# open-mmlab/Amphion

Measured on AMD Instinct MI355X. Metric: audio samples/sec (HiFi-GAN V1 22.05 kHz generator, mel->wav), higher is better.
Workload: dtype f32 (split-f16 MFMA: 3 x v_mfma_f32_32x32x16_f16 per term, f32 accumulate)

## Files before the change

amphion_amd/_lib.py:

```python
from __future__ import annotations

import ctypes
import os
import weakref
from ctypes import POINTER, c_char_p, c_float, c_int, c_int32, c_int64, c_size_t, c_void_p

_HERE = os.path.dirname(os.path.abspath(__file__))
LIB_PATH = os.environ.get("AMP_LIB_PATH") or os.path.join(_HERE, "lib", "libamphion_hip.so")

AMP_MAX_STAGES = 8
AMP_MAX_KERNELS = 8
AMP_MAX_DILATIONS = 8

AMP_ARCH_HIFIGAN, AMP_ARCH_BIGVGAN, AMP_ARCH_HIFIGAN_VITS = 0, 1, 2
AMP_ACT_LRELU, AMP_ACT_SNAKE, AMP_ACT_SNAKEBETA = 0, 1, 2
AMP_PRECISION_F32, AMP_PRECISION_F16X3 = 0, 1
AMP_CONV_OPT_PAD_REFLECT, AMP_CONV_OPT_TANH = 1, 2
AMP_PAD_REPLICATE, AMP_PAD_ZEROS, AMP_PAD_REFLECT = 0, 1, 2
AMP_PW_BIAS, AMP_PW_BIAS_GELU, AMP_PW_SCALE_RES = 0, 1, 2
PRECISIONS = {"f32": AMP_PRECISION_F32, "fp32": AMP_PRECISION_F32, "f16x3": AMP_PRECISION_F16X3}


class AmpError(RuntimeError):

    def __init__(self, status, message):
        super().__init__(f"libamphion_hip error {status}: {message}")
        self.status = status


class amp_gen_desc(ctypes.Structure):
    _fields_ = [
        ("arch", c_int32),
        ("n_in", c_int32),
        ("upsample_initial_channel", c_int32),
        ("n_stages", c_int32),
        ("upsample_rates", c_int32 * AMP_MAX_STAGES),
        ("upsample_kernel_sizes", c_int32 * AMP_MAX_STAGES),
        ("n_kernels", c_int32),
        ("resblock_kernel_sizes", c_int32 * AMP_MAX_KERNELS),
        ("n_dilations", c_int32 * AMP_MAX_KERNELS),
        ("resblock_dilation_sizes", (c_int32 * AMP_MAX_DILATIONS) * AMP_MAX_KERNELS),
        ("resblock_type", c_int32),
        ("activation", c_int32),
        ("snake_logscale", c_int32),
        ("gin_channels", c_int32),
    ]


class amp_mel_desc(ctypes.Structure):
    _fields_ = [
        ("struct_size", ctypes.c_uint32),
        ("n_fft", c_int32),
        ("win_size", c_int32),
        ("hop_size", c_int32),
        ("n_mel", c_int32),
        ("pad_mode", c_int32),
        ("mag_eps", c_float),
        ("log_clip", c_float),
        ("mel_bands_dev", c_void_p),
        ("range_dev", c_void_p),
        ("range_host", c_void_p),
        ("range_reset_dev", c_void_p),
        ("range_seq", c_int32),
    ]

    def __init__(self, *args, **kw):
        super().__init__(ctypes.sizeof(type(self)), *args, **kw)


class amp_dw_desc(ctypes.Structure):
    _fields_ = [
        ("residual_channels", c_int32),
        ("residual_layers", c_int32),
        ("dilation_cycle_length", c_int32),
        ("n_mel", c_int32),
        ("upsample0", c_int32),
        ("upsample1", c_int32),
        ("max_steps", c_int32),
    ]


_SIGNATURES = {
    "amp_version": (c_int, []),
    "amp_last_error": (c_char_p, []),
    "amp_device_count": (c_int, []),
    "amp_set_precision": (c_int, [c_int]),
    "amp_get_precision": (c_int, []),
    "amp_gen_create": (c_int, [POINTER(amp_gen_desc), POINTER(c_void_p)]),
    "amp_gen_set_weight": (c_int, [c_void_p, c_char_p, c_void_p, POINTER(c_int64), c_int]),
    "amp_gen_finalize": (c_int, [c_void_p]),
    "amp_gen_hop": (c_int, [c_void_p]),
    "amp_gen_workspace_bytes": (c_size_t, [c_void_p, c_int, c_int]),
    "amp_set_group_mb": (c_int, [c_int]),
    "amp_set_pair_strips": (c_int, [c_int]),
    "amp_range_check": (c_int, [c_void_p]),
    "amp_gen_range_check": (c_int, [c_void_p, c_void_p]),
    "amp_gen_forward": (c_int, [c_void_p, c_void_p, c_void_p, c_int, c_int, c_void_p, c_void_p, c_size_t, c_void_p]),
    "amp_gen_forward_ragged": (c_int, [c_void_p, c_void_p, c_void_p, c_void_p, c_int, c_int, c_void_p, c_void_p, c_size_t, c_void_p]),
    "amp_gen_set_profiling": (c_int, [c_void_p, c_int]),
    "amp_gen_last_timing_ms": (c_int, [c_void_p, c_int, POINTER(c_float)]),
    "amp_gen_timing_ms": (c_int, [c_void_p, c_int, c_int, POINTER(c_float)]),
    "amp_gen_kernel_name": (c_int, [c_void_p, c_int, c_int, c_char_p, c_size_t]),
    "amp_gen_destroy": (None, [c_void_p]),
    "amp_conv_create": (c_int, [c_int, c_int, c_int, c_int, c_int, c_int, c_int, c_void_p, c_void_p, POINTER(c_void_p)]),
    "amp_conv_out_len": (c_int, [c_void_p, c_int]),
    "amp_conv_forward": (c_int, [c_void_p, c_void_p, c_int, c_int, c_float, c_void_p, c_float, c_void_p, c_void_p]),
    "amp_conv_forward_strided": (c_int, [c_void_p, c_void_p, ctypes.c_longlong, c_int, c_int, c_float, c_void_p, c_float, c_void_p, c_void_p]),
    "amp_conv_forward_ragged": (c_int, [c_void_p, c_void_p, ctypes.c_longlong, c_int, c_int, c_void_p, c_float, c_void_p, c_float, c_void_p, c_void_p]),
    "amp_conv_forward_mrf": (c_int, [c_void_p, c_void_p, c_int, c_int, c_float, c_void_p, c_void_p, c_int, c_float, c_void_p]),
    "amp_apnet_polar": (c_int, [c_void_p, c_void_p, c_void_p, c_size_t, c_void_p, c_void_p, c_void_p, c_void_p]),
    "amp_istft_same": (c_int, [POINTER(amp_mel_desc), c_void_p, c_void_p, c_int, c_int, c_void_p, c_void_p, c_void_p, c_void_p, c_void_p]),
    "amp_istft_same_polar": (c_int, [POINTER(amp_mel_desc), c_void_p, ctypes.c_longlong, c_int, c_int, c_float, c_void_p, c_void_p, c_void_p,
                                     c_void_p, c_void_p]),
    "amp_pw_create": (c_int, [c_int, c_int, c_void_p, c_void_p, POINTER(c_void_p)]),
    "amp_pw_forward": (c_int, [c_void_p, c_void_p, ctypes.c_longlong, c_int, c_int, c_int, c_void_p, c_void_p, c_void_p, c_void_p]),
    "amp_pw_precision": (c_int, [c_void_p]),
    "amp_pw_destroy": (None, [c_void_p]),
    "amp_dw_create": (c_int, [POINTER(amp_dw_desc), POINTER(c_void_p)]),
    "amp_dw_set_weight": (c_int, [c_void_p, c_char_p, c_void_p, ctypes.c_longlong]),
    "amp_dw_finalize": (c_int, [c_void_p]),
    "amp_dw_precision": (c_int, [c_void_p]),
    "amp_dw_set_precision": (c_int, [c_void_p, c_int]),
    "amp_dw_workspace_bytes": (c_size_t, [c_void_p, c_int, c_int]),
    "amp_dw_condition": (c_int, [c_void_p, c_void_p, c_int, c_int, c_void_p, c_void_p, c_size_t, c_void_p]),
    "amp_dw_embed": (c_int, [c_void_p, c_void_p, c_int, c_void_p, c_void_p]),
    "amp_dw_input": (c_int, [c_void_p, c_void_p, c_int, c_int, c_void_p, c_void_p]),
    "amp_dw_layer": (c_int, [c_void_p, c_int, c_void_p, c_void_p, c_void_p, ctypes.c_longlong, c_void_p, c_void_p, c_void_p, c_int, c_int, c_void_p]),
    "amp_dw_tail": (c_int, [c_void_p, c_void_p, c_int, c_int, c_void_p, c_void_p]),
    "amp_dw_forward": (c_int, [c_void_p, c_void_p, c_int, c_void_p, c_int, c_void_p, c_int, c_int, c_void_p, c_void_p, c_size_t, c_void_p]),
    "amp_dw_sample_step": (c_int, [c_void_p, c_void_p, c_int, c_float, c_float, c_float, c_float, c_void_p, c_void_p, c_int, c_int, c_void_p,
                                   c_size_t, c_void_p]),
    "amp_dw_destroy": (None, [c_void_p]),
    "amp_fvq_create": (c_int, [c_int, c_int, c_int, c_int, c_int, POINTER(c_void_p), POINTER(c_void_p), POINTER(c_void_p), POINTER(c_void_p),
                               POINTER(c_void_p), POINTER(c_void_p)]),
    "amp_fvq_encode": (c_int, [c_void_p, c_void_p, c_int, c_int, c_int, c_void_p, c_void_p, c_void_p, c_void_p]),
    "amp_fvq_decode": (c_int, [c_void_p, c_void_p, c_int, c_int, c_int, c_void_p, c_void_p]),
    "amp_fvq_check": (c_int, [c_void_p, c_void_p]),
    "amp_fvq_encode_ex": (c_int, [c_void_p, c_void_p, ctypes.c_longlong, c_void_p, c_int, c_int, c_int, c_void_p, c_void_p, c_void_p, c_void_p,
                                  c_void_p]),
    "amp_fvq_decode_add": (c_int, [c_void_p, c_void_p, c_int, c_int, c_int, c_void_p, c_void_p, c_void_p]),
    "amp_semantic_prepare": (c_int, [c_void_p, c_void_p, c_void_p, c_int, c_int, c_int, c_int, c_void_p, c_void_p]),
    "amp_fvq_destroy": (None, [c_void_p]),
    "amp_codec_unit_create": (c_int, [c_int, c_int, c_void_p, c_void_p, c_void_p, c_void_p, c_void_p, c_void_p, POINTER(c_void_p)]),
    "amp_codec_unit_fused": (c_int, [c_void_p]),
    "amp_set_codec_unit_fusion": (c_int, [c_int]),
    "amp_codec_unit_workspace_bytes": (c_size_t, [c_void_p, c_int, c_int]),
    "amp_codec_unit_forward": (c_int, [c_void_p, c_void_p, c_int, c_int, c_void_p, c_void_p, c_size_t, c_void_p]),
    "amp_codec_unit_destroy": (None, [c_void_p]),
    "amp_aa_unit_create": (c_int, [c_int, c_int, c_void_p, c_void_p, c_void_p, c_void_p, c_void_p, c_void_p, c_void_p, c_void_p, c_int, c_void_p,
                                   c_void_p, POINTER(c_void_p)]),
    "amp_aa_unit_fused": (c_int, [c_void_p]),
    "amp_set_aa_unit_fusion": (c_int, [c_int]),
    "amp_aa_unit_workspace_bytes": (c_size_t, [c_void_p, c_int, c_int]),
    "amp_aa_unit_forward": (c_int, [c_void_p, c_void_p, c_int, c_int, c_void_p, c_void_p, c_size_t, c_void_p]),
    "amp_aa_unit_destroy": (None, [c_void_p]),
    "amp_sconv_create": (c_int, [c_int, c_int, c_int, c_int, c_void_p, c_void_p, POINTER(c_void_p)]),
    "amp_sconv_out_len": (c_int, [c_void_p, c_int]),
    "amp_sconv_workspace_bytes": (c_size_t, [c_void_p, c_int, c_int]),
    "amp_sconv_forward": (c_int, [c_void_p, c_void_p, c_int, c_int, c_void_p, c_void_p, c_size_t, c_void_p, c_void_p]),
    "amp_sconv_destroy": (None, [c_void_p]),
    "amp_tconv_create": (c_int, [c_int, c_int, c_int, c_int, c_int, c_void_p, c_void_p, POINTER(c_void_p)]),
    "amp_tconv_out_len": (c_int, [c_void_p, c_int]),
    "amp_tconv_fused": (c_int, [c_void_p]),
    "amp_set_tconv_fusion": (c_int, [c_int]),
    "amp_tconv_workspace_bytes": (c_size_t, [c_void_p, c_int, c_int]),
    "amp_tconv_forward": (c_int, [c_void_p, c_void_p, c_int, c_int, c_void_p, c_void_p, c_size_t, c_void_p, c_void_p]),
    "amp_tconv_destroy": (None, [c_void_p]),
    "amp_elu_pad": (c_int, [c_void_p, c_int, c_int, c_int, c_int, c_int, c_int, c_float, c_void_p, c_void_p]),
    "amp_lstm_create": (c_int, [c_int, c_int, c_int, c_int, c_int, POINTER(c_void_p), POINTER(c_void_p), POINTER(c_void_p), POINTER(c_void_p),
                                POINTER(c_void_p)]),
    "amp_lstm_workspace_bytes": (c_size_t, [c_void_p, c_int, c_int]),
    "amp_lstm_out_channels": (c_int, [c_void_p]),
    "amp_lstm_forward": (c_int, [c_void_p, c_void_p, c_int, c_int, c_void_p, c_void_p, c_size_t, c_void_p]),
    "amp_lstm_recur": (c_int, [c_void_p, c_int, c_void_p, c_int, c_int, c_void_p, c_void_p, c_void_p, c_void_p]),
    "amp_lstm_destroy": (None, [c_void_p]),
    "amp_evq_create": (c_int, [c_int, c_int, c_int, POINTER(c_void_p), POINTER(c_void_p)]),
    "amp_evq_encode": (c_int, [c_void_p, c_void_p, c_int, c_int, c_int, c_int, c_void_p, c_void_p, c_void_p, c_void_p]),
    "amp_evq_decode": (c_int, [c_void_p, c_void_p, c_int, c_int, c_int, c_int, c_void_p, c_void_p]),
    "amp_evq_check": (c_int, [c_void_p, c_void_p]),
    "amp_evq_destroy": (None, [c_void_p]),
    "amp_dsconv_create": (c_int, [c_int, c_int, c_void_p, c_void_p, POINTER(c_void_p)]),
    "amp_dsconv_out_len": (c_int, [c_void_p, c_int]),
    "amp_dsconv_workspace_bytes": (c_size_t, [c_void_p, c_int, c_int]),
    "amp_dsconv_forward": (c_int, [c_void_p, c_void_p, c_int, c_int, c_int, c_void_p, c_size_t, c_void_p, c_void_p]),
    "amp_dsconv_destroy": (None, [c_void_p]),
    "amp_gelu": (c_int, [c_void_p, ctypes.c_longlong, c_void_p, c_void_p]),
    "amp_layer_norm_c": (c_int, [c_void_p, c_void_p, c_void_p, c_void_p, c_void_p, c_int, c_int, c_int, c_float, c_int, c_void_p, c_void_p]),
    "amp_add_channel_bias": (c_int, [c_void_p, c_void_p, c_int, c_int, c_int, c_void_p]),
    "amp_layer_norm_c_ragged": (c_int, [c_void_p, c_void_p, c_void_p, c_void_p, c_void_p, c_void_p, c_int, c_int, c_int, c_float, c_int, c_void_p, c_void_p]),
    "amp_dds_seam": (c_int, [c_void_p, c_void_p, c_void_p, c_void_p, c_float, c_void_p, c_void_p, c_int, c_int, c_void_p, c_void_p, c_float,
                             c_void_p, c_int, c_int, c_int, c_void_p, c_void_p, c_void_p]),
    "amp_dwconv_layer_norm_c": (c_int, [c_void_p, c_void_p, c_void_p, c_int, c_int, c_void_p, c_void_p, c_void_p, c_int, c_int, c_int, c_float, c_int, c_void_p, c_void_p]),
    "amp_dwconv_layer_norm_c_causal": (c_int, [c_void_p, c_void_p, c_void_p, c_int, c_int, c_void_p, c_void_p, c_void_p, c_int, c_int, c_int, c_float, c_int,
                                               c_void_p, c_void_p]),
    "amp_rel_attention_strided": (c_int, [c_void_p, c_void_p, c_void_p, ctypes.c_longlong, c_void_p, c_void_p, c_void_p, c_int, c_int, c_int, c_int, c_int, c_void_p, c_void_p]),
    "amp_set_rel_attention_tiled": (c_int, [c_int]),
    "amp_set_resblock_streams": (c_int, [c_int]),
    "amp_gen_prepare_streams": (c_int, [c_void_p]),
    "amp_rel_attention": (c_int, [c_void_p, c_void_p, c_void_p, c_void_p, c_void_p, c_void_p, c_int, c_int, c_int, c_int, c_int, c_void_p, c_void_p]),
    "amp_dwconv": (c_int, [c_void_p, c_void_p, c_void_p, c_void_p, c_int, c_int, c_int, c_int, c_int, c_void_p, c_void_p]),
    "amp_spline_flow": (c_int, [c_void_p, c_void_p, c_void_p, c_int, c_int, c_int, c_int, c_float, c_int, c_int, c_int, c_void_p, c_void_p]),
    "amp_spline_flow_proj": (c_int, [c_void_p, c_void_p, c_void_p, c_void_p, c_void_p, c_int, c_int, c_int, c_int, c_int, c_float, c_int, c_int, c_int, c_void_p, c_void_p]),
    "amp_affine_reverse": (c_int, [c_void_p, c_void_p, c_void_p, c_void_p, c_int, c_int, c_int, c_void_p, c_void_p]),
    "amp_embed_tokens": (c_int, [c_void_p, c_void_p, c_void_p, c_int, c_int, c_int, c_int, c_float, c_void_p, c_void_p]),
    "amp_durations": (c_int, [c_void_p, c_void_p, c_int, c_int, c_float, c_void_p, c_void_p, c_void_p, c_void_p]),
    "amp_expand_path": (c_int, [c_void_p, c_void_p, c_void_p, c_void_p, c_int, c_int, c_int, c_int, c_void_p, c_void_p, c_void_p]),
    "amp_expand_path_strided": (c_int, [c_void_p, ctypes.c_longlong, c_void_p, c_void_p, c_void_p, c_int, c_int, c_int, c_int, c_void_p, c_void_p, c_void_p]),
    "amp_gauss_sample": (c_int, [c_void_p, c_void_p, c_void_p, c_size_t, c_float, c_void_p, c_void_p]),
    "amp_snake": (c_int, [c_void_p, c_int, c_int, c_int, c_void_p, c_void_p, c_int, c_void_p, c_void_p]),
    "amp_fir_upsample": (c_int, [c_void_p, c_int, c_int, c_int, c_void_p, c_int, c_int, c_void_p, c_void_p]),
    "amp_fir_filter": (c_int, [c_void_p, c_int, c_int, c_int, c_void_p, c_int, c_int, c_int, c_int, c_int, c_void_p, c_void_p]),
    "amp_wav_to_pcm16": (c_int, [c_void_p, c_int, c_int, ctypes.c_longlong, c_void_p, c_void_p, ctypes.c_longlong, c_void_p]),
    "amp_conv_set_option": (c_int, [c_void_p, c_int, c_int]),
    "amp_pair_forward": (c_int, [c_void_p, c_void_p, c_void_p, c_int, c_int, c_float, c_void_p, c_void_p]),
    "amp_resblock_forward": (c_int, [POINTER(c_void_p), POINTER(c_void_p), c_int, c_void_p, c_int, c_int, c_float, c_void_p, c_void_p]),
    "amp_set_resblock_fusion": (c_int, [c_int]),
    "amp_conv_destroy": (None, [c_void_p]),
    "amp_set_small_conv": (c_int, [c_int]),
    "amp_set_conv_blk": (c_int, [c_int]),
    "amp_set_conv_rg_fast": (c_int, [c_int]),
    "amp_set_pingpong": (c_int, [c_int]),
    "amp_set_conv_blk_narrow": (c_int, [c_int]),
    "amp_ampblock_forward": (c_int, [POINTER(c_void_p), POINTER(c_void_p), c_int, c_void_p, c_void_p, c_int, c_void_p, c_void_p,
                                     c_void_p, c_int, c_int, c_void_p, c_int, c_float, c_void_p]),
    "amp_set_ampblock_fusion": (c_int, [c_int]),
    "amp_conv_create_gated": (c_int, [c_int, c_int, c_int, c_int, c_void_p, c_void_p, POINTER(c_void_p)]),
    "amp_wn_forward": (c_int, [POINTER(c_void_p), POINTER(c_void_p), c_int, c_void_p, c_void_p, ctypes.c_longlong, c_void_p, c_int, c_int,
                               c_void_p, c_void_p, c_void_p]),
    "amp_wn_gate": (c_int, [c_void_p, c_void_p, ctypes.c_longlong, c_void_p, c_int, c_int, c_int, c_void_p]),
    "amp_wn_accumulate": (c_int, [c_void_p, c_void_p, c_void_p, c_void_p, c_int, c_int, c_int, c_int, c_int, c_void_p]),
    "amp_sequence_mask": (c_int, [c_void_p, c_void_p, c_int, c_int, c_int, c_void_p]),
    "amp_coupling_apply": (c_int, [c_void_p, c_void_p, c_void_p, c_int, c_int, c_int, c_int, c_void_p]),
    "amp_flip_channels": (c_int, [c_void_p, c_void_p, c_int, c_int, c_int, c_void_p]),
    "amp_posterior_sample": (c_int, [c_void_p, c_void_p, c_void_p, c_void_p, c_int, c_int, c_int, c_void_p]),
    "amp_antialias_snake": (c_int, [c_void_p, c_int, c_int, c_int, c_void_p, c_void_p, c_int, c_void_p, c_void_p, c_void_p, c_void_p]),
    "amp_istft_forward": (c_int, [POINTER(amp_mel_desc), c_void_p, c_void_p, c_int, c_int, c_void_p, c_void_p, c_void_p, c_void_p, c_void_p]),
    "amp_mel_num_frames": (c_int, [POINTER(amp_mel_desc), c_int]),
    "amp_mel_init": (c_int, []),
    "amp_mel_forward_ragged": (c_int, [POINTER(amp_mel_desc), c_void_p, c_void_p, c_int, c_int, c_void_p, c_void_p, c_void_p, c_void_p, c_void_p, c_void_p, c_void_p]),
    "amp_mel_backward": (c_int, [POINTER(amp_mel_desc), c_void_p, c_int, c_int] + [c_void_p] * 11),
    "amp_mel_forward": (c_int, [POINTER(amp_mel_desc), c_void_p, c_int, c_int, c_void_p, c_void_p, c_void_p, c_void_p, c_void_p, c_void_p, c_void_p]),
}

EXPORTED_SYMBOLS = tuple(_SIGNATURES)

_lib = None


def lib():
    global _lib
    if _lib is None:
        if not os.path.exists(LIB_PATH):
            raise RuntimeError(
                f"{LIB_PATH} not found: build it with `python -m amphion_amd.build` "
                "(the HIP path has no CPU fallback)"
            )
        import torch

        L = ctypes.CDLL(LIB_PATH)
        for name, (res, args) in _SIGNATURES.items():
            fn = getattr(L, name)
            fn.restype = res
            fn.argtypes = args
        _lib = L
    return _lib


def set_precision(name):
    if name not in PRECISIONS:
        raise ValueError(f"precision must be one of {sorted(PRECISIONS)}, got {name!r}")
    check(lib().amp_set_precision(PRECISIONS[name]))


def get_precision():
    return "f32" if lib().amp_get_precision() == AMP_PRECISION_F32 else "f16x3"


def check(status):
    if status < 0:
        raise AmpError(status, lib().amp_last_error().decode("utf-8", "replace"))
    return status


def ptr(t):
    return c_void_p(t.data_ptr()) if t is not None else None


def _destroy(name, address):
    try:
        getattr(lib(), name)(c_void_p(address))
    except Exception:
        pass


def finalizer(owner, destroy, handle):
    return weakref.finalize(owner, _destroy, destroy, handle.value)


AMP_ERR_INVALID = -1
AMP_ERR_UNSUPPORTED = -4
AMP_ERR_RANGE = -6


def range_check(device=None):
    import torch

    dev = torch.device("cuda", torch.cuda.current_device()) if device is None else torch.device(device)
    with torch.cuda.device(dev):
        check(lib().amp_range_check(current_stream_ptr(dev)))


def require_device_tensor(t, name="tensor"):
    import torch

    if not isinstance(t, torch.Tensor):
        raise TypeError(f"{name} must be a torch.Tensor")
    if not t.is_cuda:
        raise RuntimeError(
            f"{name} is on {t.device}: the amphion_amd kernels run on a ROCm (MI355X) device only; "
            "there is no CPU fallback (move the model and its input to 'cuda')"
        )
    if t.dtype != torch.float32:
        raise TypeError(f"{name} must be float32, got {t.dtype}")
    return t.contiguous()


class _NullCtx:
    def __enter__(self):
        return None

    def __exit__(self, *a):
        return False


_NULL_CTX = _NullCtx()


def on_device(device):
    import torch

    idx = device.index if isinstance(device, torch.device) else torch.device(device).index
    if idx is None or idx == torch._C._cuda_getDevice():
        return _NULL_CTX
    return torch.cuda.device(device)


def current_stream_ptr(device):
    import torch

    raw = getattr(torch._C, "_cuda_getCurrentRawStream", None)
    if raw is not None:
        idx = device.index if isinstance(device, torch.device) else torch.device(device).index
        return c_void_p(raw(torch.cuda.current_device() if idx is None else idx))
    return c_void_p(torch.cuda.current_stream(device).cuda_stream)
```

amphion_amd/csrc/amp_host.h:

```cpp
#pragma once
#include <math.h>

#include <vector>

#include "amp_internal.h"

#define AMP_HIP(expr)                                                                  \
    do {                                                                               \
        hipError_t e__ = (expr);                                                       \
        if (e__ != hipSuccess) {                                                       \
            set_error("%s failed: %s (%s:%d)", #expr, hipGetErrorString(e__), __FILE__, __LINE__); \
            return AMP_ERR_HIP;                                                        \
        }                                                                              \
    } while (0)

#define AMP_RC(expr) do { int rc__ = (expr); if (rc__ != AMP_OK) return rc__; } while (0)

struct amp_conv {
    int transposed = 0, cin = 0, cout = 0, k = 0, stride = 1, dilation = 1, padding = 0;
    int M = 0, ntaps = 0, KT = 0, off0 = 0, dstep = 0, halo_left = 0, halo_right = 0, up = 1, up_pad = 0;
    int nchunks = 0;
    int precision = amp::PREC_F32;
    int pad_reflect = 0, tanh_out = 0;
    int out_pad = 0;
    int gated_H = 0;
    int Mpad = 0;
    float wscale = 1.f;
    amp::ConvPlan plan{};
    void* wp_dev = nullptr;
    float* bias_dev = nullptr;
    ~amp_conv() {
        if (wp_dev) (void)hipFree(wp_dev);
        if (bias_dev) (void)hipFree(bias_dev);
    }
};

namespace amp {

int device_upload(const void* host, size_t bytes, void** out);

struct DeviceAllocs {
    std::vector<void*> owned;
    DeviceAllocs() = default;
    DeviceAllocs(const DeviceAllocs&) = delete;
    DeviceAllocs& operator=(const DeviceAllocs&) = delete;
    ~DeviceAllocs() {
        for (void* p : owned) (void)hipFree(p);
    }
    int upload(const void* host, size_t bytes, void** out) {
        if (int rc = device_upload(host, bytes, out); rc != AMP_OK) return rc;
        owned.push_back(*out);
        return AMP_OK;
    }
    template <class T, class P>
    int upload(const std::vector<T>& v, P** out) { return upload(v.data(), v.size() * sizeof(T), (void**)out); }
};

int default_precision();

constexpr int kConvBlkDefault = 3;
constexpr int kConvRgFastDefault = 1;
constexpr int kPingPongDefault = 1;
struct Config {
    int pair_strips = -1;
    int rb_fusion = 1;
    int ampb_fusion = 1;
    int conv_blk = kConvBlkDefault;
    size_t group_bytes = 0;
    int small_conv = 1;
    int conv_rg_fast = 1;
    int pingpong = 1;
    int narrow_blk = 1;
    int rb_streams = -1;
    Config();
};
Config& cfg();

struct RangeGuard {
    unsigned* dev = nullptr;
    unsigned* host = nullptr;
    hipEvent_t ev = nullptr;
    bool pending = false;
};
bool guard_init(RangeGuard& g);
void guard_free(RangeGuard& g);
int range_poll(RangeGuard* g, hipStream_t st);
int range_publish(RangeGuard* g, hipStream_t st);
int range_check_sync(RangeGuard* g, hipStream_t st, const char* who);
struct RangeFlagScope {
    explicit RangeFlagScope(unsigned* word);
    ~RangeFlagScope();
    RangeFlagScope(const RangeFlagScope&) = delete;
    RangeFlagScope& operator=(const RangeFlagScope&) = delete;
};

inline float pow2_weight_scale(float wmax) {
    int e2 = 0;
    if (wmax > 0.f) { (void)frexpf(wmax, &e2); if (ldexpf(1.f, e2 - 1) == wmax) e2 -= 1; }
    return wmax > 0.f ? ldexpf(1.f, 13 - e2) : 1.f;
}

template <class View>
std::vector<_Float16> pack_a_f16x3(int row_blocks, int k16, int taps, size_t pad_entries, float wscale, View view) {
    std::vector<_Float16> wp(((size_t)row_blocks * k16 * taps * 2 + pad_entries) * 64 * 8, (_Float16)0.f);
    for (int mb = 0; mb < row_blocks; ++mb)
        for (int c = 0; c < k16; ++c)
            for (int g = 0; g < taps; ++g)
                for (int lane = 0; lane < 64; ++lane)
                    for (int e = 0; e < 8; ++e) {
                        const float v = view(mb * 32 + (lane & 31), c * 16 + 8 * (lane >> 5) + e, g) * wscale;
                        const _Float16 hi = (_Float16)v;
                        const _Float16 lo = (_Float16)(v - (float)hi);
                        const size_t ent = (((size_t)mb * k16 + c) * taps + g) * 2;
                        wp[((ent + 0) * 64 + lane) * 8 + e] = hi;
                        wp[((ent + 1) * 64 + lane) * 8 + e] = lo;
                    }
    return wp;
}

template <class View>
int pack_matrix_f16x3(const char* who, int rows, int cols, int row_blocks, int k16, View W, std::vector<_Float16>* wp, float* inv_scale) {
    float wmax = 0.f;
    for (int m = 0; m < rows; ++m)
        for (int i = 0; i < cols; ++i) {
            const float w = fabsf(W(m, i));
            if (!(w < 1e30f)) { set_error("%s: non-finite weight", who); return AMP_ERR_INVALID; }
            wmax = fmaxf(wmax, w);
        }
    const float wscale = pow2_weight_scale(wmax);
    *inv_scale = 1.f / (16.f * wscale);
    *wp = pack_a_f16x3(row_blocks, k16, 1, 0, wscale, [&](int m, int i, int) { return (m < rows && i < cols) ? W(m, i) : 0.f; });
    return AMP_OK;
}

int conv_build(amp_conv* c, const float* w, const float* bias);
int conv_run(const amp_conv* c, const float* x, int B, int T, float slope_in, const float* res, float slope_out, float* y, int mode, float div,
             hipStream_t stream, long long xbs = 0, const int* lens = nullptr, int len_mul = 1, ConvArgs* plan_small = nullptr,
             int* plan_ni = nullptr);
int next_rev(const int* lens);

bool pair_supported(const amp_conv* c1, const amp_conv* c2);
int pair_run(const amp_conv* c1, const amp_conv* c2, const float* x, int B, int T, float slope, float* y, int mode, float div,
             hipStream_t stream, const int* lens = nullptr, int len_mul = 1);
bool pair_tile_args(const amp_conv* c1, const amp_conv* c2, const float* x, int B, int T, float slope, float* y, int mode, float div,
                    const int* lens, int len_mul, PairArgs* out);

bool rb_supported(const amp_conv* const* c1, const amp_conv* const* c2, int np, int B, int T);
int rb_split(const amp_conv* const* c1, int np, int B, int T);
int rb_run(const amp_conv* const* c1, const amp_conv* const* c2, int np, const float* x, int B, int T, float slope, float* y, int mode,
           float div, hipStream_t stream, const int* lens = nullptr, int len_mul = 1, int first = 0, int count = -1);

struct ActParams {
    float* a_dev = nullptr;
    float* invb_dev = nullptr;
    float* fu_dev = nullptr;
    float* fd_dev = nullptr;
    float* fu2_dev = nullptr;
};
int act_params_upload(const float* alpha_dev, const float* beta_dev, int C, int logscale, const float* filt_up_host,
                      const float* filt_down_host, float** out);
bool ampb_supported(const amp_conv* const* c1, const amp_conv* const* c2, int np, const ActParams* acts, size_t nacts, int B, int T);
int ampb_run(const amp_conv* const* c1, const amp_conv* const* c2, int np, const ActParams* acts, const float* x, int B, int T, float* y,
             int mode, float div, hipStream_t stream, const int* lens = nullptr, int len_mul = 1);

}
```

amphion_amd/csrc/amp_internal.h:

```cpp
#pragma once
#include <hip/hip_runtime.h>
#include <stdarg.h>
#include <stdint.h>
#include <stdio.h>

#include <atomic>
#include <mutex>
#include <string>
#include <vector>

#include "amphion_hip.h"

namespace amp {

constexpr int KC = 8;
constexpr int KC16 = 16;

enum { PREC_F32 = 0, PREC_F16X3 = 1 };

struct ConvArgs {
    const float* x;
    const void* wp;
    const float* bias;
    const float* res;
    float* y;
    int B, Cin, Tin;
    long long xbs;
    int nchunks;
    int M;
    int Tq;
    int tiles_per_item;
    int rev;
    int row_groups;
    int off0, dstep;
    int halo_left;
    int wd;
    int Cout, Tout;
    int up, up_pad;
    float slope_in, slope_out;
    int mode;
    float div;
    float acc_scale, inv_scale;
    const int* lens;
    int len_mul;
    unsigned* range_flag;
    int pad_reflect;
    int tanh_out;
    int Mpad;
    const float* gate_cond;
    long long gate_cond_bs;
    int wn_H;
    float* wn_x;
    float* wn_out;
    int wn_first, wn_last;
};

struct PairArgs {
    const float* x;
    float* y;
    const void* wp1;
    const float* bias1;
    const void* wp2;
    const float* bias2;
    int B, C, T;
    int tiles_per_item;
    int strip_len;
    int strips_per_item;
    int wide;
    int rev;
    int dil;
    float slope;
    float sc1, isc1, sc2, isc2;
    int mode;
    float div;
    const int* lens;
    int len_mul;
    unsigned* range_flag;
};

struct ConvSmall3Args {
    ConvArgs a[3];
    int nx[3], ny[3];
};
hipError_t launch_conv_small3(const ConvSmall3Args& p, const int ni[3], hipStream_t stream);

struct Pair3Args {
    PairArgs a[3];
    int n[3];
};
hipError_t launch_pair3(const Pair3Args& p, hipStream_t stream);

constexpr int AMP_RB_MAX_PAIRS = 3;
struct RbArgs {
    const float* x;
    float* y;
    const void* wp1[AMP_RB_MAX_PAIRS];
    const float* bias1[AMP_RB_MAX_PAIRS];
    const void* wp2[AMP_RB_MAX_PAIRS];
    const float* bias2[AMP_RB_MAX_PAIRS];
    float sc1[AMP_RB_MAX_PAIRS], isc1[AMP_RB_MAX_PAIRS], sc2[AMP_RB_MAX_PAIRS], isc2[AMP_RB_MAX_PAIRS];
    int dil[AMP_RB_MAX_PAIRS];
    int np;
    int rh;
    int B, C, T;
    int tiles_per_item;
    int rev;
    float slope;
    int mode;
    float div;
    const int* lens;
    int len_mul;
    unsigned* range_flag;
};

constexpr int AMP_AMPB_MAX_STEPS = 6;
struct AmpbArgs {
    const float* x;
    float* y;
    const void* wp[AMP_AMPB_MAX_STEPS];
    const float* bias[AMP_AMPB_MAX_STEPS];
    float sc[AMP_AMPB_MAX_STEPS], isc[AMP_AMPB_MAX_STEPS];
    int dil[AMP_AMPB_MAX_STEPS];
    const float* act_a[AMP_AMPB_MAX_STEPS];
    const float* act_invb[AMP_AMPB_MAX_STEPS];
    const float* act_fu[AMP_AMPB_MAX_STEPS];
    const float* act_fd[AMP_AMPB_MAX_STEPS];
    int ns;
    int rh;
    int B, C, T;
    int tiles_per_item;
    int rev;
    int mode;
    float div;
    const int* lens;
    int len_mul;
    unsigned* range_flag;
};

constexpr int DW_TN = 64;
struct DwLayerArgs {
    const float* x;
    const float* cond;
    const float* dconst;
    long long dconst_bs;
    const float* skip_in;
    float* x_out;
    float* skip_out;
    const uint4* wp1;
    const uint4* wp2;
    const float* w1f;
    const float* w2f;
    const float* bias1;
    const float* bias2;
    int C, n_mel, L, d;
    int K16;
    int tiles_per_item;
    float inv1, inv2;
    unsigned* range_flag;
};
size_t dw_layer_lds_bytes(int C, int n_mel, bool f32);
hipError_t launch_dw_layer(DwLayerArgs a, int B, bool f32, hipStream_t stream);

constexpr int CU_TN = 64;
struct CodecUnitArgs {
    const float* x;
    float* y;
    const uint4* wp1;
    const uint4* wp2;
    const float* bias1;
    const float* bias2;
    const float *alpha1, *invb1, *alpha2, *invb2;
    int C, T, d;
    int tiles_per_item;
    float inv1, inv2;
    unsigned* range_flag;
};
size_t codec_unit_lds_bytes(int C, int d);
hipError_t launch_codec_unit(CodecUnitArgs a, int B, hipStream_t stream);

constexpr int AA_N1 = 64;
constexpr int AA_TN = 54;
struct AaUnitArgs {
    const float* x;
    float* y;
    const uint4* wp1;
    const uint4* wp2;
    const float* bias1;
    const float* bias2;
    const float *a1, *invb1, *a2, *invb2;
    const float* filt;
    int C, T, d;
    int tiles_per_item;
    float inv1, inv2;
    unsigned* range_flag;
};
size_t aa_unit_lds_bytes(int C, int d);
hipError_t launch_aa_unit(AaUnitArgs a, int B, hipStream_t stream);

constexpr int TC_TN = 64;
struct TconvArgs {
    const float* x;
    float* y;
    const uint4* wp;
    const float* bias;
    const float* alpha;
    int cin, cout, s, p;
    int T, Tout;
    int M, NRB;
    int q_first;
    int tiles_per_item;
    float inv;
    unsigned* range_flag;
};
size_t tconv_lds_bytes(int cin);
hipError_t launch_tconv(TconvArgs a, int B, hipStream_t stream);

struct ConvPlan {
    int KT;
    int WM, WN;
    int NI;
    int HALO;
    int NT() const { return 32 * NI * WN; }
    int Mgroup() const { return 32 * WM; }
};

bool choose_plan(int ntaps, int M, int halo_total, int Tq, ConvPlan* plan);

template <int KT> hipError_t launch_conv(const ConvPlan& plan, const ConvArgs& a, hipStream_t stream);
template <int KT> hipError_t launch_conv_f16x3(const ConvPlan& plan, const ConvArgs& a, hipStream_t stream);
template <int KT> int conv_blk_nt(int cm, int halo_total);
template <int KT> hipError_t launch_conv_blk(int cm, int wn, const ConvArgs& a, hipStream_t stream);
constexpr int kSmallConvMaxChunks = 16;
template <int KT> hipError_t launch_conv_small(int ni, int epi, const ConvArgs& a, hipStream_t stream);
template <int KT> int pair_tile(int C, int dil);
template <int KT> hipError_t launch_pair(const PairArgs& a, hipStream_t stream);
template <int KT> int strip_step(int C, int dil, int wide, int* wg_per_cu);
template <int KT> hipError_t launch_strip(const PairArgs& a, hipStream_t stream);
template <int KT> int rb_tile(int C, int max_dil, int wide);
template <int KT> hipError_t launch_rb(const RbArgs& a, int wide, hipStream_t stream);
template <int KT> int ampb_tile(int C, int max_dil, int wide);
template <int KT> hipError_t launch_ampb(const AmpbArgs& a, int wide, hipStream_t stream);

hipError_t launch_conv_post(const float* x, const float* w_dev , const float* bias_dev ,
                            float* y, int B, int Cin, int T, int K, float slope_in, int apply_tanh,
                            const int* lens, int len_mul, hipStream_t stream);

hipError_t launch_act1d(const float* x, float* y, int B, int C, int T, const float* a_dev, const float* invb_dev,
                        const float* filt_up12, const float* filt_dn12, const int* lens, int len_mul,
                        hipStream_t stream, int rev = 0 );

hipError_t launch_add_channel_bias(float* y, const float* cb, int B, int C, int T, hipStream_t stream);
constexpr int AMP_MRF_MAX_PARTS = 3;
struct MrfSumArgs {
    float* y;
    const float* p[AMP_MRF_MAX_PARTS];
    int n;
    float div;
    size_t count;
};
hipError_t launch_mrf_sum(const MrfSumArgs& a, hipStream_t stream);

hipError_t launch_wn_gate(const float* a, const float* cond, long long cond_bs, float* out, int B, int H, int T,
                          hipStream_t stream);
hipError_t launch_wn_accumulate(float* x, float* out, const float* rs, const int* lens, int B, int H, int T, int last,
                                int first, hipStream_t stream);
hipError_t launch_mask(float* x, const int* lens, int B, int C, int T, hipStream_t stream);
hipError_t launch_coupling(float* x, const float* m, const int* lens, int B, int h, int T, int reverse,
                           hipStream_t stream);
hipError_t launch_flip_channels(const float* x, float* y, int B, int C, int T, hipStream_t stream);
hipError_t launch_posterior_sample(const float* stats, const float* eps, const int* lens, float* z, int B, int C, int T,
                                   hipStream_t stream);

hipError_t launch_fir_up(const float* x, float* y, int rows, int T, const float* taps_host, int K, int ratio, int pad,
                         int pad_left, hipStream_t stream);
hipError_t launch_fir_filter(const float* x, float* y, int rows, int T, int Tout, const float* taps_host, int K,
                             int stride, int pad_left, int mode, hipStream_t stream);
hipError_t launch_snake(const float* x, float* y, int B, int C, int T, const float* alpha, const float* beta, int logscale,
                        hipStream_t stream);
hipError_t launch_pcm16(const float* x, short* y, int B, int L, long long x_stride, long long y_stride, const int* lens,
                        hipStream_t stream);
hipError_t launch_apnet_polar(const float* logamp, const float* R, const float* I, size_t n, float* pha, float* rea,
                              float* imag, hipStream_t stream);

hipError_t launch_mel(const amp_mel_desc& d, const float* wav, const int* lens, int B, int L, int F, const float* window,
                      const float* melbasis, float* mel, float* mag, float* re, float* im, hipStream_t stream);

void set_error(const char* fmt, ...);

template <auto Kernel>
inline hipError_t ensure_dynamic_lds(size_t bytes) {
    if (bytes <= 64 * 1024) return hipSuccess;
    static std::atomic<unsigned long long> done{0};
    static std::mutex mu;
    int dev = 0;
    if (hipGetDevice(&dev) != hipSuccess || dev < 0) dev = 0;
    if (dev < 64 && ((done.load(std::memory_order_acquire) >> dev) & 1ull)) return hipSuccess;
    std::lock_guard<std::mutex> lock(mu);
    if (dev < 64 && ((done.load(std::memory_order_acquire) >> dev) & 1ull)) return hipSuccess;
    const hipError_t e = hipFuncSetAttribute(reinterpret_cast<const void*>(Kernel), hipFuncAttributeMaxDynamicSharedMemorySize, (int)bytes);
    if (e != hipSuccess) return e;
    if (dev < 64) done.fetch_or(1ull << dev, std::memory_order_release);
    return hipSuccess;
}

template <auto Kernel, class Args>
inline hipError_t launch_dynamic_lds(unsigned grid, size_t lds, hipStream_t stream, const Args& a) {
    if (hipError_t e = ensure_dynamic_lds<Kernel>(lds); e != hipSuccess) return e;
    hipLaunchKernelGGL(Kernel, dim3(grid), dim3(256), lds, stream, a);
    return hipGetLastError();
}

extern __thread std::string* tl_kernel_log;
bool manifest_on();
void manifest_add(const char* name, unsigned long long workgroups, double gflop, double mb, const char* what);
extern __thread char tl_last_kernel[160];
template <typename... A>
inline void note_kernel(const char* base, A... args) {
    if (!tl_kernel_log && !manifest_on()) return;
    char* buf = tl_last_kernel;
    constexpr int cap = (int)sizeof(tl_last_kernel);
    const int v[] = {static_cast<int>(args)...};
    int n = snprintf(buf, cap, "%s<", base);
    for (size_t i = 0; i < sizeof...(args) && n < cap - 16; ++i)
        n += snprintf(buf + n, cap - n, i ? ", %d" : "%d", v[i]);
    snprintf(buf + n, cap - n, ">");
    if (!tl_kernel_log) return;
    if (tl_kernel_log->find(buf) != std::string::npos) return;
    if (!tl_kernel_log->empty()) *tl_kernel_log += " | ";
    *tl_kernel_log += buf;
}
inline void note_work(unsigned long long workgroups, double gflop, double mb, const char* fmt, ...) __attribute__((format(printf, 4, 5)));
inline void note_work(unsigned long long workgroups, double gflop, double mb, const char* fmt, ...) {
    if (!manifest_on()) return;
    char what[160];
    va_list ap;
    va_start(ap, fmt);
    vsnprintf(what, sizeof(what), fmt, ap);
    va_end(ap);
    manifest_add(tl_last_kernel, workgroups, gflop, mb, what);
}
extern __thread int tl_conv_transposed;
inline void note_conv_work(const ConvArgs& a, int KT, dim3 grid) {
    const bool convt = tl_conv_transposed != 0;
    tl_conv_transposed = 0;
    if (!manifest_on()) return;
    const double gf = 2.0 * a.M * a.Cin * KT * (double)a.Tq * a.B / 1e9;
    const double mb = 4.0 * a.B * ((double)a.Cin * a.Tin + (double)a.Cout * a.Tout * (1 + (a.res ? 1 : 0) + (a.mode ? 1 : 0))) / 1e6;
    note_work((unsigned long long)grid.x * grid.y, gf, mb, "%s %d->%d k=%d d=%d T=%d->%d B=%d%s%s grid=%ux%u", convt ? "ConvT" : "conv", a.Cin,
              a.Cout, a.up > 1 ? KT * a.up : KT, a.dstep, a.Tin, a.Tout, a.B, a.res ? " +res" : "", a.mode ? " +sum" : "", grid.x, grid.y);
}

unsigned* range_flag_for_current_device();

}
```

amphion_amd/csrc/conv_host.hip:

```cpp
#include <string.h>

#include <memory>
#include <type_traits>
#include <vector>

#include "amp_host.h"

namespace amp {

template <int... K> struct Taps { static constexpr int list[] = {K...}; };
using ConvTaps = Taps<1, 2, 3, 5, 7, 11>;
using BlkTaps = Taps<2, 3, 7, 11>;
using SmallTaps = Taps<1, 3, 5, 7, 11>;
using PairTaps = Taps<3, 5, 7, 11>;
using RbTaps = Taps<3, 5, 7, 11>;
using AmpbTaps = Taps<3, 5, 7, 11>;

template <int... K, typename R, typename F>
static R with_taps(Taps<K...>, int k, R dflt, F&& f) {
    R r = dflt;
    (void)((k == K && (r = f(std::integral_constant<int, K>{}), true)) || ...);
    return r;
}

static hipError_t launch_conv(const ConvPlan& p, const ConvArgs& a, hipStream_t s) {
    return with_taps(ConvTaps{}, p.KT, hipErrorInvalidValue, [&](auto K) { return launch_conv<K>(p, a, s); });
}
static hipError_t launch_conv_f16x3(const ConvPlan& p, const ConvArgs& a, hipStream_t s) {
    return with_taps(ConvTaps{}, p.KT, hipErrorInvalidValue, [&](auto K) { return launch_conv_f16x3<K>(p, a, s); });
}
static int conv_blk_nt(int k, int cm, int halo) { return with_taps(BlkTaps{}, k, 0, [&](auto K) { return conv_blk_nt<K>(cm, halo); }); }
static hipError_t launch_conv_blk(int k, int cm, int wn, const ConvArgs& a, hipStream_t s) {
    return with_taps(BlkTaps{}, k, hipErrorInvalidValue, [&](auto K) { return launch_conv_blk<K>(cm, wn, a, s); });
}
static hipError_t launch_conv_small(int k, int ni, int epi, const ConvArgs& a, hipStream_t s) {
    return with_taps(SmallTaps{}, k, hipErrorInvalidValue, [&](auto K) { return launch_conv_small<K>(ni, epi, a, s); });
}
static int pair_tile(int k, int C, int dil) { return with_taps(PairTaps{}, k, 0, [&](auto K) { return pair_tile<K>(C, dil); }); }
static hipError_t launch_pair(int k, const PairArgs& a, hipStream_t s) {
    return with_taps(PairTaps{}, k, hipErrorInvalidValue, [&](auto K) { return launch_pair<K>(a, s); });
}
static int strip_step(int k, int C, int dil, int wide, int* wg) {
    return with_taps(PairTaps{}, k, 0, [&](auto K) { return strip_step<K>(C, dil, wide, wg); });
}
static hipError_t launch_strip(int k, const PairArgs& a, hipStream_t s) {
    return with_taps(PairTaps{}, k, hipErrorInvalidValue, [&](auto K) { return launch_strip<K>(a, s); });
}
static int rb_tile(int k, int C, int max_dil, int wide) { return with_taps(RbTaps{}, k, 0, [&](auto K) { return rb_tile<K>(C, max_dil, wide); }); }
static hipError_t launch_rb(int k, const RbArgs& a, int wide, hipStream_t s) {
    return with_taps(RbTaps{}, k, hipErrorInvalidValue, [&](auto K) { return launch_rb<K>(a, wide, s); });
}
static int ampb_tile(int k, int C, int max_dil, int wide) {
    return with_taps(AmpbTaps{}, k, 0, [&](auto K) { return ampb_tile<K>(C, max_dil, wide); });
}
static hipError_t launch_ampb(int k, const AmpbArgs& a, int wide, hipStream_t s) {
    return with_taps(AmpbTaps{}, k, hipErrorInvalidValue, [&](auto K) { return launch_ampb<K>(a, wide, s); });
}

static int round_up_taps(int ntaps) {
    for (int kt : ConvTaps::list)
        if (kt >= ntaps) return kt;
    return -1;
}

bool choose_plan(int KT, int M, int halo_total, int , ConvPlan* plan) {
    bool ok = false;
    for (int kt : ConvTaps::list) ok |= (kt == KT);
    if (!ok || halo_total > 128) return false;
    plan->KT = KT;
    plan->HALO = halo_total <= 64 ? 64 : 128;
    if (M > 64) { plan->WM = 4; plan->WN = 1; plan->NI = 8; }
    else if (M > 32) { plan->WM = 2; plan->WN = 2; plan->NI = 8; }
    else { plan->WM = 1; plan->WN = 4; plan->NI = 4; }
    return true;
}

struct StripChoice { bool use; int wide; int steps; };
static StripChoice strip_choice(int C, int k) {
    const int mode = cfg().pair_strips;
    if (mode == 0) return {false, 0, 0};
    if (C == 128 && (k == 7 || k == 11)) return {true, 3, 1};
    return {false, 0, 0};
}

static void strip_plan(int B, int T, int n1, int hb, int wg_per_cu, int* strip_len, int* spi_out) {
    const int slots = wg_per_cu * 256;
    long best = -1; int best_spi = 1;
    const int max_spi = (T + n1 - 1) / n1;
    for (int spi = 1; spi <= max_spi; ++spi) {
        const int L = (T + spi - 1) / spi;
        if ((long)(spi - 1) * L >= T) continue;
        const long steps = (L + hb + n1 - 1) / n1;
        const long rounds = ((long)B * spi + slots - 1) / slots;
        const long cost = rounds * (4 * steps + 1);
        if (best < 0 || cost < best) { best = cost; best_spi = spi; }
    }
    *spi_out = best_spi;
    *strip_len = (T + best_spi - 1) / best_spi;
}

static void strip_geometry(int B, int T, int n1, int hb, int wg_per_cu, int steps, bool ragged, int* strip_len, int* spi) {
    strip_plan(B, T, n1, hb, wg_per_cu, strip_len, spi);
    if (steps > 0 && steps * n1 - hb < T) { *strip_len = steps * n1 - hb; *spi = (T + *strip_len - 1) / *strip_len; }
    if (steps == 1 && !ragged && 4 * n1 - hb < T) {
        const int len4 = 4 * n1 - hb, spi4 = (T + len4 - 1) / len4;
        if ((long long)B * spi4 >= 1024) { *strip_len = len4; *spi = spi4; }
    }
}

constexpr long long kSmallGridWorkgroups = 384;

static bool small_conv_enabled() { return cfg().small_conv != 0; }

static int conv_blk_mode() { return cfg().conv_blk; }
static int narrow_blk_mode() { return cfg().narrow_blk; }
constexpr size_t kConvRgFastMaxWeightBytes = 3u << 20;
static bool conv_rg_fast() { return cfg().conv_rg_fast != 0; }
static thread_local unsigned g_launch_parity = 0;
int next_rev(const int* lens) {
    if (!cfg().pingpong || lens) return 0;
    return (int)(g_launch_parity++ & 1u);
}
constexpr long long kConvBlkMinWorkgroups = 512;

int conv_build(amp_conv* c, const float* w, const float* bias) {
    if (c->cin <= 0 || c->cout <= 0 || c->k <= 0 || c->stride <= 0 || c->dilation <= 0) {
        set_error("amp_conv: bad dimensions cin=%d cout=%d k=%d stride=%d dilation=%d", c->cin, c->cout, c->k, c->stride,
                  c->dilation);
        return AMP_ERR_INVALID;
    }
    if (!c->transposed) {
        if (c->stride != 1) { set_error("amp_conv: strided Conv1d is not on the vocoder path"); return AMP_ERR_UNSUPPORTED; }
        c->up = 1; c->up_pad = 0;
        c->M = c->cout;
        c->ntaps = c->k;
        c->off0 = -c->padding;
        c->dstep = c->dilation;
    } else if (c->stride == 1) {
        if (c->dilation != 1) { set_error("amp_conv: dilated ConvTranspose1d unsupported (dilation=%d)", c->dilation); return AMP_ERR_UNSUPPORTED; }
        c->up = 1; c->up_pad = 0;
        c->M = c->cout;
        c->ntaps = c->k;
        c->off0 = -(c->k - 1 - c->padding);
        c->dstep = 1;
    } else {
        if (c->dilation != 1) { set_error("amp_conv: dilated ConvTranspose1d unsupported (dilation=%d)", c->dilation); return AMP_ERR_UNSUPPORTED; }
        c->up = c->stride; c->up_pad = c->padding;
        c->M = c->cout * c->stride;
        c->ntaps = (c->k + c->stride - 1) / c->stride;
        c->off0 = 0;
        c->dstep = -1;
    }
    c->KT = round_up_taps(c->ntaps);
    if (c->KT < 0) { set_error("amp_conv: k=%d at stride=%d is %d taps, unsupported (max 11)", c->k, c->stride, c->ntaps); return AMP_ERR_UNSUPPORTED; }
    const int omin = c->dstep >= 0 ? c->off0 : c->off0 + (c->KT - 1) * c->dstep;
    const int omax = c->dstep >= 0 ? c->off0 + (c->KT - 1) * c->dstep : c->off0;
    c->halo_left = omin < 0 ? -omin : 0;
    c->halo_right = omax > 0 ? omax : 0;
    if (!choose_plan(c->KT, c->M, c->halo_left + c->halo_right, 0, &c->plan)) {
        set_error("amp_conv: receptive field (k=%d, dilation=%d, padding=%d: %d columns) exceeds the 128-column staged halo", c->k, c->dilation,
                  c->padding, c->halo_left + c->halo_right);
        return AMP_ERR_UNSUPPORTED;
    }
    c->precision = default_precision();
    if (c->precision == PREC_F16X3) c->plan.NI = 4;
    const int Mg = c->plan.Mgroup();
    const int Mpad = ((c->M + Mg - 1) / Mg) * Mg;
    c->Mpad = Mpad;
    const int nmb = Mpad / 32;
    const int cin = c->cin, cout = c->cout, k = c->k, up = c->up;
    auto wview = [&](int m, int i, int g) -> float {
        if (m >= c->M || i >= cin || g >= c->ntaps) return 0.f;
        if (!c->transposed) return w[((size_t)m * cin + i) * k + g];
        if (up == 1) return w[((size_t)i * cout + m) * k + (k - 1 - g)];
        const int o = m / up, r = m - o * up;
        const int j = r + g * up;
        return j < k ? w[((size_t)i * cout + o) * k + j] : 0.f;
    };
    if (c->precision == PREC_F32) {
        c->nchunks = (c->cin + KC - 1) / KC;
        const size_t n = ((size_t)nmb * c->nchunks + 1) * c->KT * 64 * 4;
        std::vector<float> wp(n, 0.f);
        for (int mb = 0; mb < nmb; ++mb)
            for (int ch = 0; ch < c->nchunks; ++ch)
                for (int g = 0; g < c->KT; ++g)
                    for (int lane = 0; lane < 64; ++lane)
                        for (int p = 0; p < 4; ++p)
                            wp[((((size_t)mb * c->nchunks + ch) * c->KT + g) * 64 + lane) * 4 + p] =
                                wview(mb * 32 + (lane & 31), ch * KC + 2 * p + (lane >> 5), g);
        AMP_RC(device_upload(wp.data(), n * sizeof(float), &c->wp_dev));
    } else {
        c->nchunks = (c->cin + KC16 - 1) / KC16;
        float wmax = 0.f;
        const size_t nw = (size_t)cin * cout * k;
        for (size_t i = 0; i < nw; ++i) wmax = fmaxf(wmax, fabsf(w[i]));
        if (!(wmax < 1e30f)) { set_error("amp_conv: non-finite weight"); return AMP_ERR_INVALID; }
        c->wscale = pow2_weight_scale(wmax);
        const std::vector<_Float16> wp = pack_a_f16x3(nmb, c->nchunks, c->KT, (size_t)2 * c->KT * 2, c->wscale, wview);
        AMP_RC(device_upload(wp.data(), wp.size() * sizeof(_Float16), &c->wp_dev));
    }
    if (bias) AMP_RC(device_upload(bias, (size_t)cout * sizeof(float), (void**)&c->bias_dev));
    return AMP_OK;
}

static size_t conv_weight_bytes(const amp_conv* c) { return (size_t)c->Mpad * c->nchunks * KC16 * c->KT * 4; }

static int conv_out_len(const amp_conv* c, int T) {
    if (!c->transposed) return T + 2 * c->padding - c->dilation * (c->k - 1);
    return (T - 1) * c->stride - 2 * c->padding + c->k + c->out_pad;
}

static bool small_conv_static_ok(const amp_conv* c) {
    return c->precision == PREC_F16X3 && !c->transposed && !c->pad_reflect && c->plan.WM == 4 &&
           (c->KT == 1 || c->KT == 3 || c->KT == 5 || c->KT == 7 || c->KT == 11) && c->KT == c->ntaps &&
           c->nchunks <= kSmallConvMaxChunks && c->halo_left + c->halo_right <= 64;
}
static bool small_conv_covers(const amp_conv* c) { return small_conv_enabled() && small_conv_static_ok(c); }
static int small_conv_ni(const amp_conv* c) { return (c->halo_left + c->halo_right <= 32) ? 1 : 2; }

int conv_run(const amp_conv* c, const float* x, int B, int T, float slope_in, const float* res, float slope_out,
             float* y, int mode, float div, hipStream_t stream, long long xbs, const int* lens, int len_mul,
             ConvArgs* plan_small, int* plan_ni) {
    if (B <= 0 || T <= 0) { set_error("amp_conv_forward: B=%d T=%d", B, T); return AMP_ERR_INVALID; }
    const int Tout = conv_out_len(c, T);
    if (Tout <= 0) { set_error("amp_conv_forward: input too short (T=%d gives T_out=%d)", T, Tout); return AMP_ERR_INVALID; }
    ConvArgs a{};
    a.x = x; a.wp = c->wp_dev; a.bias = c->bias_dev; a.res = res; a.y = y;
    a.B = B; a.Cin = c->cin; a.Tin = T; a.xbs = xbs > 0 ? xbs : (long long)c->cin * T; a.nchunks = c->nchunks; a.M = c->M;
    a.Tq = c->up > 1 ? T + c->ntaps - 1 : Tout;
    ConvPlan plan = c->plan;
    if (c->precision == PREC_F16X3) {
        const long long wgs = (long long)B * ((a.Tq + plan.NT() - 1) / plan.NT()) * ((c->M + plan.Mgroup() - 1) / plan.Mgroup());
        if (wgs < kSmallGridWorkgroups) plan.NI = 2;
    }
    const int NT = plan.NT();
    a.tiles_per_item = (a.Tq + NT - 1) / NT;
    a.off0 = c->off0; a.dstep = c->dstep; a.halo_left = c->halo_left;
    a.wd = NT + c->halo_left + c->halo_right;
    a.Cout = c->cout; a.Tout = Tout; a.up = c->up; a.up_pad = c->up_pad;
    a.slope_in = slope_in; a.slope_out = slope_out; a.mode = mode; a.div = div;
    a.lens = lens; a.len_mul = len_mul;
    a.pad_reflect = c->pad_reflect; a.tanh_out = c->tanh_out;
    a.range_flag = c->precision == PREC_F16X3 ? range_flag_for_current_device() : nullptr;
    a.rev = c->precision == PREC_F16X3 ? next_rev(lens) : 0;
    if (c->pad_reflect && (c->halo_left >= T || c->halo_right >= T)) {
        set_error("amp_conv_forward: reflection padding %d needs more than %d input samples", c->halo_left > c->halo_right ? c->halo_left : c->halo_right, T);
        return AMP_ERR_INVALID;
    }
    if (c->gated_H) { set_error("amp_conv_forward: a gated conv (amp_conv_create_gated) only runs inside amp_wn_forward"); return AMP_ERR_STATE; }
    if (c->precision == PREC_F16X3 && slope_in > 1.f) {
        set_error("amp_conv_forward: leaky_relu slope %g > 1 on the input is outside the f16x3 kernels (use AMP_PRECISION_F32)", (double)slope_in);
        return AMP_ERR_UNSUPPORTED;
    }
    tl_conv_transposed = c->transposed;
    if (c->precision == PREC_F32) {
        if (plan_small) return AMP_ERR_UNSUPPORTED;
        a.acc_scale = a.inv_scale = 1.f;
        AMP_HIP(launch_conv(plan, a, stream));
    } else {
        a.acc_scale = 16.f * c->wscale;
        a.inv_scale = 1.f / a.acc_scale;
        const long long wgs_half = (long long)B * ((a.Tq + 63) / 64) * ((c->M + plan.Mgroup() - 1) / plan.Mgroup());
        int blk_cm = 0, blk_nt = 0, blk_wn = 1;
        const bool blk_kt = c->KT == 2 || c->KT == 3 || (conv_blk_mode() == 3 && (c->KT == 7 || c->KT == 11));
        if (c->M % 256 == 0) blk_wn = 1;
        else if (c->M % 128 == 0 && c->KT != 2 && (narrow_blk_mode() >= 2 || (narrow_blk_mode() == 1 && c->KT >= 7))) blk_wn = 2;
        else blk_wn = 0;
        if (conv_blk_mode() > 0 && plan.NI == 4 && blk_wn > 0 && blk_kt && !c->tanh_out && !c->pad_reflect) {
            int cm = (conv_blk_mode() >= 2 && c->KT == 2 && c->nchunks % 2 == 0) ? 2 : 1;
            const int halo = c->halo_left + c->halo_right;
            const int nt = blk_wn * conv_blk_nt(c->KT, cm, halo);
            if (nt > 0 && (long long)B * ((a.Tq + nt - 1) / nt) * (c->M / (256 / blk_wn)) >= kConvBlkMinWorkgroups) { blk_cm = cm; blk_nt = nt; }
        }
        if (plan_small && !(blk_cm == 0 && plan.NI == 2 && small_conv_covers(c) && (c->KT <= 5 || wgs_half <= 128))) return AMP_ERR_UNSUPPORTED;
        if (blk_cm > 0) {
            const int rows = 256 / blk_wn;
            a.tiles_per_item = (a.Tq + blk_nt - 1) / blk_nt;
            a.wd = blk_nt + c->halo_left + c->halo_right;
            a.row_groups = (conv_rg_fast() && c->M / rows > 1 && conv_weight_bytes(c) <= kConvRgFastMaxWeightBytes) ? c->M / rows : 0;
            AMP_HIP(launch_conv_blk(c->KT, blk_cm, blk_wn, a, stream));
        } else if (plan.NI == 2 && small_conv_covers(c) && (c->KT <= 5 || wgs_half <= 128)) {
            const int ni = small_conv_ni(c);
            a.Mpad = c->Mpad;
            a.tiles_per_item = (a.Tq + 32 * ni - 1) / (32 * ni);
            a.wd = 32 * ni + c->halo_left + c->halo_right;
            if (plan_small) { *plan_small = a; *plan_ni = ni; return AMP_OK; }
            AMP_HIP(launch_conv_small(c->KT, ni, 0, a, stream));
        } else {
            const int nrg = (c->M + plan.Mgroup() - 1) / plan.Mgroup();
            a.row_groups = (conv_rg_fast() && nrg > 1 && conv_weight_bytes(c) <= kConvRgFastMaxWeightBytes) ? nrg : 0;
            AMP_HIP(launch_conv_f16x3(plan, a, stream));
        }
    }
    return AMP_OK;
}

bool pair_supported(const amp_conv* c1, const amp_conv* c2) {
    if (c1->precision != PREC_F16X3 || c2->precision != PREC_F16X3) return false;
    if (c1->pad_reflect || c2->pad_reflect || c1->tanh_out || c2->tanh_out) return false;
    if (c1->transposed || c2->transposed || c1->cin != c1->cout || c2->cin != c2->cout || c1->cin != c2->cin) return false;
    if (c1->k != c2->k || c2->dilation != 1 || c1->k != c1->KT) return false;
    if (c1->padding != (c1->k - 1) / 2 * c1->dilation || c2->padding != (c2->k - 1) / 2) return false;
    if (!c1->bias_dev || !c2->bias_dev) return false;
    const StripChoice sc = strip_choice(c1->cin, c1->k);
    if (sc.use && strip_step(c1->k, c1->cin, c1->dilation, sc.wide, nullptr) > 0) return true;
    return pair_tile(c1->k, c1->cin, c1->dilation) > 0;
}

int pair_run(const amp_conv* c1, const amp_conv* c2, const float* x, int B, int T, float slope, float* y,
                    int mode, float div, hipStream_t stream, const int* lens, int len_mul) {
    if (x == y) { set_error("pair_run: x and y must not alias"); return AMP_ERR_INVALID; }
    if (slope > 1.f) { set_error("pair_run: leaky_relu slope %g > 1 is outside the fused pair kernels", (double)slope); return AMP_ERR_UNSUPPORTED; }
    PairArgs a{};
    a.x = x; a.y = y;
    a.wp1 = c1->wp_dev; a.bias1 = c1->bias_dev; a.wp2 = c2->wp_dev; a.bias2 = c2->bias_dev;
    a.B = B; a.C = c1->cin; a.T = T;
    a.dil = c1->dilation;
    a.slope = slope;
    a.sc1 = 16.f * c1->wscale; a.isc1 = 1.f / a.sc1;
    a.sc2 = 16.f * c2->wscale; a.isc2 = 1.f / a.sc2;
    a.mode = mode; a.div = div;
    a.lens = lens; a.len_mul = len_mul;
    a.range_flag = range_flag_for_current_device();
    a.rev = next_rev(lens);
    int wg = 2;
    const StripChoice sc = strip_choice(c1->cin, c1->k);
    const int n1 = sc.use ? strip_step(c1->k, c1->cin, c1->dilation, sc.wide, &wg) : 0;
    if (n1 > 0) {
        a.wide = sc.wide;
        strip_geometry(B, T, n1, c1->k - 1, wg, sc.steps, lens != nullptr, &a.strip_len, &a.strips_per_item);
        if (cfg().pair_strips == -1 && sc.wide >= 2 && (long long)B * a.strips_per_item < 512 && pair_tile(c1->k, c1->cin, c1->dilation) > 0) {
            const int NT = pair_tile(c1->k, c1->cin, c1->dilation);
            a.tiles_per_item = (T + NT - 1) / NT;
            AMP_HIP(launch_pair(c1->k, a, stream));
            return AMP_OK;
        }
        AMP_HIP(launch_strip(c1->k, a, stream));
        return AMP_OK;
    }
    const int NT = pair_tile(c1->k, c1->cin, c1->dilation);
    a.tiles_per_item = (T + NT - 1) / NT;
    AMP_HIP(launch_pair(c1->k, a, stream));
    return AMP_OK;
}

bool pair_tile_args(const amp_conv* c1, const amp_conv* c2, const float* x, int B, int T, float slope, float* y, int mode,
                           float div, const int* lens, int len_mul, PairArgs* out) {
    if (x == y || slope > 1.f || !pair_supported(c1, c2)) return false;
    PairArgs a{};
    a.x = x; a.y = y;
    a.wp1 = c1->wp_dev; a.bias1 = c1->bias_dev; a.wp2 = c2->wp_dev; a.bias2 = c2->bias_dev;
    a.B = B; a.C = c1->cin; a.T = T;
    a.dil = c1->dilation;
    a.slope = slope;
    a.sc1 = 16.f * c1->wscale; a.isc1 = 1.f / a.sc1;
    a.sc2 = 16.f * c2->wscale; a.isc2 = 1.f / a.sc2;
    a.mode = mode; a.div = div;
    a.lens = lens; a.len_mul = len_mul;
    a.range_flag = range_flag_for_current_device();
    a.rev = 0;
    int wg = 2;
    const StripChoice sc = strip_choice(c1->cin, c1->k);
    const int n1 = sc.use ? strip_step(c1->k, c1->cin, c1->dilation, sc.wide, &wg) : 0;
    if (n1 > 0) {
        int strip_len = 0, strips_per_item = 0;
        strip_geometry(B, T, n1, c1->k - 1, wg, sc.steps, lens != nullptr, &strip_len, &strips_per_item);
        if (!(cfg().pair_strips == -1 && sc.wide >= 2 && (long long)B * strips_per_item < 512)) return false;
    }
    const int NT = pair_tile(c1->k, c1->cin, c1->dilation);
    if (NT <= 0) return false;
    a.tiles_per_item = (T + NT - 1) / NT;
    *out = a;
    return true;
}

static int rb_fusion_mode() { return cfg().rb_fusion; }
static int rb_form(int C, int k) {
    const int m = rb_fusion_mode();
    if (m == 0) return -1;
    if (m == 3) return (C == 32 || (C == 64 && k <= 5)) ? 0 : 1;
    if (m == 2) return 1;
    if (C == 32) return k >= 11 ? 1 : 0;
    if (C == 64) return k <= 5 ? 0 : 1;
    if (C == 128) return 1;
    return -1;
}
constexpr long long kRbMinWorkgroups = 256;

bool rb_supported(const amp_conv* const* c1, const amp_conv* const* c2, int np, int B, int T) {
    if (np < 1 || np > AMP_RB_MAX_PAIRS) return false;
    int max_dil = 1, rh = 0;
    for (int p = 0; p < np; ++p) {
        if (!c1[p] || !c2[p] || !pair_supported(c1[p], c2[p])) return false;
        if (c1[p]->cin != c1[0]->cin || c1[p]->k != c1[0]->k) return false;
        max_dil = c1[p]->dilation > max_dil ? c1[p]->dilation : max_dil;
        rh += (c1[p]->k - 1) / 2 * (c1[p]->dilation + 1);
    }
    const int form = rb_form(c1[0]->cin, c1[0]->k);
    if (form < 0) return false;
    const int W = rb_tile(c1[0]->k, c1[0]->cin, max_dil, form);
    if (W <= 0 || W - 2 * rh < W / 2) return false;
    const int NT = W - 2 * rh;
    if (rb_fusion_mode() == 1 && (long long)B * ((T + NT - 1) / NT) < kRbMinWorkgroups) return false;
    return true;
}

int rb_split(const amp_conv* const* c1, int np, int B, int T) {
    if (np != 3 || rb_fusion_mode() != 1) return 0;
    int max_dil = 1, rh = 0;
    for (int p = 0; p < np; ++p) {
        max_dil = c1[p]->dilation > max_dil ? c1[p]->dilation : max_dil;
        rh += (c1[p]->k - 1) / 2 * (c1[p]->dilation + 1);
    }
    const int W = rb_tile(c1[0]->k, c1[0]->cin, max_dil, rb_form(c1[0]->cin, c1[0]->k));
    const int NT = W - 2 * rh;
    if (W <= 0 || 5 * NT >= 4 * W) return 0;
    if ((long long)B * ((T + NT - 1) / NT) < 1024) return 0;
    return 2;
}

int rb_run(const amp_conv* const* c1, const amp_conv* const* c2, int np, const float* x, int B, int T, float slope, float* y, int mode,
           float div, hipStream_t stream, const int* lens, int len_mul, int first, int count) {
    if (x == y) { set_error("rb_run: x and y must not alias"); return AMP_ERR_INVALID; }
    if (slope > 1.f) { set_error("rb_run: leaky_relu slope %g > 1 is outside the fused kernels", (double)slope); return AMP_ERR_UNSUPPORTED; }
    RbArgs a{};
    a.x = x; a.y = y;
    a.np = count < 0 ? np - first : count;
    c1 += first;
    c2 += first;
    int max_dil = 1;
    for (int p = 0; p < a.np; ++p) {
        a.wp1[p] = c1[p]->wp_dev; a.bias1[p] = c1[p]->bias_dev; a.wp2[p] = c2[p]->wp_dev; a.bias2[p] = c2[p]->bias_dev;
        a.sc1[p] = 16.f * c1[p]->wscale; a.isc1[p] = 1.f / a.sc1[p];
        a.sc2[p] = 16.f * c2[p]->wscale; a.isc2[p] = 1.f / a.sc2[p];
        a.dil[p] = c1[p]->dilation;
        a.rh += (c1[p]->k - 1) / 2 * (c1[p]->dilation + 1);
        max_dil = c1[p]->dilation > max_dil ? c1[p]->dilation : max_dil;
    }
    for (int p = a.np; p < AMP_RB_MAX_PAIRS; ++p) {
        a.wp1[p] = a.wp1[0]; a.bias1[p] = a.bias1[0]; a.wp2[p] = a.wp2[0]; a.bias2[p] = a.bias2[0]; a.dil[p] = 1;
    }
    a.B = B; a.C = c1[0]->cin; a.T = T;
    const int form = rb_form(a.C, c1[0]->k);
    const int W = rb_tile(c1[0]->k, a.C, max_dil, form);
    const int NT = W - 2 * a.rh;
    a.tiles_per_item = (T + NT - 1) / NT;
    a.slope = slope; a.mode = mode; a.div = div;
    a.lens = lens; a.len_mul = len_mul;
    a.range_flag = range_flag_for_current_device();
    a.rev = next_rev(lens);
    AMP_HIP(launch_rb(c1[0]->k, a, form, stream));
    return AMP_OK;
}

static int ampb_fusion_mode() { return cfg().ampb_fusion; }
static int ampb_form(int C, int k) {
    const int m = ampb_fusion_mode();
    if (m == 0) return -1;
    if (m == 3) return C == 32 ? 0 : 1;
    if (m == 2) return 1;
    if (C == 32) return k >= 11 ? 1 : 0;
    if (C == 64) return k <= 3 ? 1 : -1;
    return -1;
}
constexpr long long kAmpbMinWorkgroups = 256;

static int ampb_halo(const amp_conv* const* c1, int np) {
    int rh = 0;
    for (int p = 0; p < np; ++p) rh += 10 + (c1[p]->k - 1) / 2 * (c1[p]->dilation + 1);
    return (rh + 3) & ~3;
}

bool ampb_supported(const amp_conv* const* c1, const amp_conv* const* c2, int np, const ActParams* acts, size_t nacts, int B, int T) {
    if (np < 1 || 2 * np > AMP_AMPB_MAX_STEPS || nacts != (size_t)(2 * np)) return false;
    for (size_t i = 0; i < nacts; ++i)
        if (!acts[i].fu2_dev) return false;
    if ((T & 3) != 0) return false;
    int max_dil = 1;
    for (int p = 0; p < np; ++p) {
        const amp_conv *a = c1[p], *b = c2[p];
        if (!a || !b || a->precision != PREC_F16X3 || b->precision != PREC_F16X3) return false;
        if (a->pad_reflect || b->pad_reflect || a->tanh_out || b->tanh_out || a->transposed || b->transposed) return false;
        if (a->cin != a->cout || b->cin != b->cout || a->cin != b->cin || a->cin != c1[0]->cin) return false;
        if (a->k != c1[0]->k || b->k != a->k || b->dilation != 1 || a->k != a->KT) return false;
        if (a->padding != (a->k - 1) / 2 * a->dilation || b->padding != (b->k - 1) / 2) return false;
        if (!a->bias_dev || !b->bias_dev) return false;
        max_dil = a->dilation > max_dil ? a->dilation : max_dil;
    }
    const int form = ampb_form(c1[0]->cin, c1[0]->k);
    if (form < 0) return false;
    const int W = ampb_tile(c1[0]->k, c1[0]->cin, max_dil, form);
    const int rh = ampb_halo(c1, np);
    if (W <= 0 || W - 2 * rh < W / 2) return false;
    const int NT = W - 2 * rh;
    if (ampb_fusion_mode() == 1 && (long long)B * ((T + NT - 1) / NT) < kAmpbMinWorkgroups) return false;
    return true;
}

int ampb_run(const amp_conv* const* c1, const amp_conv* const* c2, int np, const ActParams* acts, const float* x, int B, int T,
                    float* y, int mode, float div, hipStream_t stream, const int* lens, int len_mul) {
    if (x == y) { set_error("ampb_run: x and y must not alias"); return AMP_ERR_INVALID; }
    AmpbArgs a{};
    a.x = x; a.y = y;
    a.ns = 2 * np;
    int max_dil = 1;
    for (int s = 0; s < AMP_AMPB_MAX_STEPS; ++s) {
        const int sv = s < a.ns ? s : 0;
        const amp_conv* c = (sv & 1) ? c2[sv >> 1] : c1[sv >> 1];
        a.wp[s] = c->wp_dev; a.bias[s] = c->bias_dev;
        a.sc[s] = 16.f * c->wscale; a.isc[s] = 1.f / a.sc[s];
        a.dil[s] = c->dilation;
        a.act_a[s] = acts[sv].a_dev; a.act_invb[s] = acts[sv].invb_dev; a.act_fu[s] = acts[sv].fu2_dev; a.act_fd[s] = acts[sv].fd_dev;
        max_dil = c->dilation > max_dil ? c->dilation : max_dil;
    }
    a.rh = ampb_halo(c1, np);
    a.B = B; a.C = c1[0]->cin; a.T = T;
    const int form = ampb_form(a.C, c1[0]->k);
    const int W = ampb_tile(c1[0]->k, a.C, max_dil, form);
    const int NT = W - 2 * a.rh;
    a.tiles_per_item = (T + NT - 1) / NT;
    a.mode = mode; a.div = div;
    a.lens = lens; a.len_mul = len_mul;
    a.range_flag = range_flag_for_current_device();
    a.rev = next_rev(lens);
    AMP_HIP(launch_ampb(c1[0]->k, a, form, stream));
    return AMP_OK;
}

int act_params_upload(const float* alpha_dev, const float* beta_dev, int C, int logscale, const float* filt_up_host,
                             const float* filt_down_host, float** out) {
    std::vector<float> al(C), be(C), a(C), ib(C);
    AMP_HIP(hipMemcpy(al.data(), alpha_dev, C * sizeof(float), hipMemcpyDeviceToHost));
    if (beta_dev) AMP_HIP(hipMemcpy(be.data(), beta_dev, C * sizeof(float), hipMemcpyDeviceToHost));
    for (int i = 0; i < C; ++i) {
        float av = al[i], bv = beta_dev ? be[i] : al[i];
        if (logscale) { av = expf(av); bv = expf(bv); }
        a[i] = av;
        ib[i] = 1.0f / (bv + 0.000000001f);
    }
    float* scratch = nullptr;
    AMP_HIP(hipMalloc((void**)&scratch, (2 * (size_t)C + 36) * sizeof(float)));
    float fu2[12];
    for (int i = 0; i < 12; ++i) fu2[i] = 2.f * filt_up_host[i];
    hipError_t e = hipMemcpy(scratch, a.data(), C * sizeof(float), hipMemcpyHostToDevice);
    if (e == hipSuccess) e = hipMemcpy(scratch + C, ib.data(), C * sizeof(float), hipMemcpyHostToDevice);
    if (e == hipSuccess) e = hipMemcpy(scratch + 2 * C, filt_up_host, 12 * sizeof(float), hipMemcpyHostToDevice);
    if (e == hipSuccess) e = hipMemcpy(scratch + 2 * C + 12, filt_down_host, 12 * sizeof(float), hipMemcpyHostToDevice);
    if (e == hipSuccess) e = hipMemcpy(scratch + 2 * C + 24, fu2, 12 * sizeof(float), hipMemcpyHostToDevice);
    if (e != hipSuccess) { (void)hipFree(scratch); set_error("act_params_upload: %s", hipGetErrorString(e)); return AMP_ERR_HIP; }
    *out = scratch;
    return AMP_OK;
}

}

using namespace amp;

extern "C" {

int amp_conv_create(int transposed, int cin, int cout, int k, int stride, int dilation, int padding,
                    const float* weight_host, const float* bias_host, amp_conv** out) {
    if (!weight_host || !out) { set_error("amp_conv_create: null argument"); return AMP_ERR_INVALID; }
    if (amp_device_count() <= 0) { set_error("amp_conv_create: no HIP device visible (the HIP path has no CPU fallback)"); return AMP_ERR_HIP; }
    auto c = std::make_unique<amp_conv>();
    c->transposed = transposed; c->cin = cin; c->cout = cout; c->k = k; c->stride = stride; c->dilation = dilation; c->padding = padding;
    int rc = conv_build(c.get(), weight_host, bias_host);
    if (rc != AMP_OK) return rc;
    *out = c.release();
    return AMP_OK;
}

int amp_conv_create_gated(int hidden, int k, int dilation, int padding, const float* weight_host, const float* bias_host,
                          amp_conv** out) {
    if (!weight_host || !out) { set_error("amp_conv_create_gated: null argument"); return AMP_ERR_INVALID; }
    if (amp_device_count() <= 0) { set_error("amp_conv_create_gated: no HIP device visible (the HIP path has no CPU fallback)"); return AMP_ERR_HIP; }
    if (hidden <= 0 || hidden % 32 != 0) { set_error("amp_conv_create_gated: hidden=%d must be a multiple of 32", hidden); return AMP_ERR_UNSUPPORTED; }
    if (default_precision() != PREC_F16X3) { set_error("amp_conv_create_gated: the fused WN layer exists for the f16x3 arithmetic only"); return AMP_ERR_UNSUPPORTED; }
    const int H = hidden, M = 2 * H;
    const size_t rowlen = (size_t)H * k;
    std::vector<float> wperm((size_t)M * rowlen), bperm((size_t)M, 0.f);
    for (int p = 0; p < M; ++p) {
        const int mb = p >> 5, rho = p & 31;
        const int i = rho & 3, hi = (rho >> 2) & 1, jj = rho >> 3, s = jj & 1, u = jj >> 1;
        const int orow = s * H + 16 * mb + i + 4 * hi + 8 * u;
        memcpy(&wperm[(size_t)p * rowlen], &weight_host[(size_t)orow * rowlen], rowlen * sizeof(float));
        if (bias_host) bperm[p] = bias_host[orow];
    }
    auto c = std::make_unique<amp_conv>();
    c->transposed = 0; c->cin = H; c->cout = M; c->k = k; c->stride = 1; c->dilation = dilation; c->padding = padding;
    int rc = conv_build(c.get(), wperm.data(), bperm.data());
    if (rc != AMP_OK) return rc;
    if (!small_conv_static_ok(c.get()) || conv_out_len(c.get(), 64) != 64) {
        set_error("amp_conv_create_gated: H=%d k=%d dilation=%d padding=%d is outside the fused WN kernel (k in {1,3,5}, H <= 256, 'same' padding, (k-1)*dilation <= 64)", H, k, dilation, padding);
        return AMP_ERR_UNSUPPORTED;
    }
    c->gated_H = H;
    *out = c.release();
    return AMP_OK;
}

static void small_args(const amp_conv* c, const float* x, int B, int T, const int* lens, int ni, ConvArgs* a) {
    *a = ConvArgs{};
    a->x = x; a->wp = c->wp_dev; a->bias = c->bias_dev;
    a->B = B; a->Cin = c->cin; a->Tin = T; a->xbs = (long long)c->cin * T; a->nchunks = c->nchunks; a->M = c->M; a->Mpad = c->Mpad;
    a->Tq = T; a->tiles_per_item = (T + 32 * ni - 1) / (32 * ni);
    a->off0 = c->off0; a->dstep = c->dstep; a->halo_left = c->halo_left; a->wd = 32 * ni + c->halo_left + c->halo_right;
    a->Cout = c->cout; a->Tout = T; a->up = 1; a->up_pad = 0;
    a->slope_in = 1.f; a->slope_out = 1.f; a->mode = 0; a->div = 1.f;
    a->lens = lens; a->len_mul = 1;
    a->acc_scale = 16.f * c->wscale; a->inv_scale = 1.f / a->acc_scale;
    a->range_flag = range_flag_for_current_device();
}

int amp_wn_forward(const amp_conv* const* in_layers, const amp_conv* const* res_skip_layers, int n_layers, float* x_dev,
                   const float* cond_dev, long long cond_batch_stride, const int32_t* lens_dev, int B, int T,
                   float* acts_ws_dev, float* out_dev, void* stream_) {
    if (!in_layers || !res_skip_layers || n_layers <= 0 || !x_dev || !acts_ws_dev || !out_dev || B <= 0 || T <= 0) {
        set_error("amp_wn_forward: bad argument");
        return AMP_ERR_INVALID;
    }
    hipStream_t stream = (hipStream_t)stream_;
    const int H = in_layers[0] ? in_layers[0]->gated_H : 0;
    for (int i = 0; i < n_layers; ++i) {
        const amp_conv* ci = in_layers[i];
        const amp_conv* cr = res_skip_layers[i];
        if (!ci || !cr) { set_error("amp_wn_forward: null layer %d", i); return AMP_ERR_INVALID; }
        const int rs_out = i < n_layers - 1 ? 2 * H : H;
        if (!ci->gated_H || ci->gated_H != H || cr->k != 1 || cr->cin != H || cr->cout != rs_out || cr->gated_H ||
            !small_conv_static_ok(cr) || cr->tanh_out || ci->tanh_out || !cr->bias_dev || !ci->bias_dev) {
            set_error("amp_wn_forward: layer %d is not an (amp_conv_create_gated in-layer, 1x1 %d -> %d res_skip) pair", i, H, rs_out);
            return AMP_ERR_INVALID;
        }
    }
    for (int i = 0; i < n_layers; ++i) {
        ConvArgs a;
        const int ni_in = small_conv_ni(in_layers[i]), ni_rs = small_conv_ni(res_skip_layers[i]);
        small_args(in_layers[i], x_dev, B, T, lens_dev, ni_in, &a);
        a.y = acts_ws_dev; a.wn_H = H;
        a.gate_cond = cond_dev ? cond_dev + (size_t)i * 2 * H : nullptr;
        a.gate_cond_bs = cond_batch_stride;
        AMP_HIP(launch_conv_small(in_layers[i]->KT, ni_in, 1, a, stream));
        small_args(res_skip_layers[i], acts_ws_dev, B, T, nullptr, ni_rs, &a);
        a.lens = lens_dev;
        a.wn_H = H; a.wn_x = x_dev; a.wn_out = out_dev; a.wn_first = i == 0; a.wn_last = i == n_layers - 1;
        AMP_HIP(launch_conv_small(1, ni_rs, 2, a, stream));
    }
    return AMP_OK;
}

int amp_conv_out_len(const amp_conv* c, int T) { return c ? conv_out_len(c, T) : 0; }

int amp_conv_forward(const amp_conv* c, const float* x_dev, int B, int T, float slope_in, const float* res_dev,
                     float slope_out, float* y_dev, void* stream) {
    if (!c || !x_dev || !y_dev) { set_error("amp_conv_forward: null argument"); return AMP_ERR_INVALID; }
    if (x_dev == y_dev) { set_error("amp_conv_forward: x and y must not alias (the conv reads a halo)"); return AMP_ERR_INVALID; }
    return conv_run(c, x_dev, B, T, slope_in, res_dev, slope_out, y_dev, 0, 1.f, (hipStream_t)stream);
}

int amp_conv_forward_strided(const amp_conv* c, const float* x_dev, long long x_batch_stride, int B, int T,
                             float slope_in, const float* res_dev, float slope_out, float* y_dev, void* stream) {
    if (!c || !x_dev || !y_dev) { set_error("amp_conv_forward_strided: null argument"); return AMP_ERR_INVALID; }
    if (x_batch_stride < (long long)c->cin * T) { set_error("amp_conv_forward_strided: batch stride %lld < cin*T", x_batch_stride); return AMP_ERR_INVALID; }
    return conv_run(c, x_dev, B, T, slope_in, res_dev, slope_out, y_dev, 0, 1.f, (hipStream_t)stream, x_batch_stride);
}

int amp_conv_forward_ragged(const amp_conv* c, const float* x_dev, long long x_batch_stride, int B, int T, const int32_t* lens_dev,
                            float slope_in, const float* res_dev, float slope_out, float* y_dev, void* stream) {
    if (!c || !x_dev || !y_dev) { set_error("amp_conv_forward_ragged: null argument"); return AMP_ERR_INVALID; }
    if (x_dev == y_dev) { set_error("amp_conv_forward_ragged: x and y must not alias (the conv reads a halo)"); return AMP_ERR_INVALID; }
    if (x_batch_stride != 0 && x_batch_stride < (long long)c->cin * T) { set_error("amp_conv_forward_ragged: batch stride %lld < cin*T", x_batch_stride); return AMP_ERR_INVALID; }
    if (lens_dev && (c->transposed || c->pad_reflect || conv_out_len(c, T) != T)) {
        set_error("amp_conv_forward_ragged: valid lengths need a 'same' zero-padded Conv1d (output length == input length)");
        return AMP_ERR_UNSUPPORTED;
    }
    return conv_run(c, x_dev, B, T, slope_in, res_dev, slope_out, y_dev, 0, 1.f, (hipStream_t)stream, x_batch_stride, lens_dev);
}

int amp_pair_forward(const amp_conv* c1, const amp_conv* c2, const float* x_dev, int B, int T, float slope,
                     float* y_dev, void* stream) {
    if (!c1 || !c2 || !x_dev || !y_dev) { set_error("amp_pair_forward: null argument"); return AMP_ERR_INVALID; }
    if (B <= 0 || T <= 0) { set_error("amp_pair_forward: B=%d T=%d", B, T); return AMP_ERR_INVALID; }
    if (!pair_supported(c1, c2)) {
        set_error("amp_pair_forward: pair (C=%d k=%d dilation=%d) is not covered by the fused kernel", c1->cin, c1->k, c1->dilation);
        return AMP_ERR_UNSUPPORTED;
    }
    return pair_run(c1, c2, x_dev, B, T, slope, y_dev, 0, 1.f, (hipStream_t)stream);
}

int amp_resblock_forward(const amp_conv* const* c1, const amp_conv* const* c2, int n_pairs, const float* x_dev, int B, int T,
                         float slope, float* y_dev, void* stream) {
    if (!c1 || !c2 || !x_dev || !y_dev) { set_error("amp_resblock_forward: null argument"); return AMP_ERR_INVALID; }
    if (B <= 0 || T <= 0 || n_pairs < 1 || n_pairs > AMP_RB_MAX_PAIRS) { set_error("amp_resblock_forward: B=%d T=%d n_pairs=%d", B, T, n_pairs); return AMP_ERR_INVALID; }
    for (int p = 0; p < n_pairs; ++p) if (!c1[p] || !c2[p]) { set_error("amp_resblock_forward: null conv handle"); return AMP_ERR_INVALID; }
    if (!rb_supported(c1, c2, n_pairs, B, T)) {
        set_error("amp_resblock_forward: block (C=%d k=%d, %d pairs, B=%d T=%d) is not covered by the whole-resblock kernel under the "
                  "current amp_set_resblock_fusion mode", c1[0]->cin, c1[0]->k, n_pairs, B, T);
        return AMP_ERR_UNSUPPORTED;
    }
    return rb_run(c1, c2, n_pairs, x_dev, B, T, slope, y_dev, 0, 1.f, (hipStream_t)stream);
}

int amp_ampblock_forward(const amp_conv* const* c1, const amp_conv* const* c2, int n_pairs, const float* alpha_dev,
                         const float* beta_dev, int logscale, const float* filt_up_host, const float* filt_down_host,
                         const float* x_dev, int B, int T, float* y_dev, int mode, float div, void* stream) {
    if (!c1 || !c2 || !alpha_dev || !filt_up_host || !filt_down_host || !x_dev || !y_dev) { set_error("amp_ampblock_forward: null argument"); return AMP_ERR_INVALID; }
    if (B <= 0 || T <= 0 || n_pairs < 1 || 2 * n_pairs > AMP_AMPB_MAX_STEPS || mode < 0 || mode > 2) {
        set_error("amp_ampblock_forward: B=%d T=%d n_pairs=%d mode=%d", B, T, n_pairs, mode);
        return AMP_ERR_INVALID;
    }
    if (x_dev == y_dev) { set_error("amp_ampblock_forward: x and y must not alias (tiles read each other's halo)"); return AMP_ERR_INVALID; }
    for (int p = 0; p < n_pairs; ++p) if (!c1[p] || !c2[p]) { set_error("amp_ampblock_forward: null conv handle"); return AMP_ERR_INVALID; }
    const int C = c1[0]->cin, na = 2 * n_pairs;
    float* scratch[AMP_AMPB_MAX_STEPS] = {};
    ActParams acts[AMP_AMPB_MAX_STEPS];
    int rc = AMP_OK;
    for (int i = 0; i < na && rc == AMP_OK; ++i) {
        rc = act_params_upload(alpha_dev + (size_t)i * C, beta_dev ? beta_dev + (size_t)i * C : nullptr, C, logscale, filt_up_host, filt_down_host, &scratch[i]);
        if (rc == AMP_OK) { acts[i].a_dev = scratch[i]; acts[i].invb_dev = scratch[i] + C; acts[i].fu_dev = scratch[i] + 2 * C; acts[i].fd_dev = scratch[i] + 2 * C + 12; acts[i].fu2_dev = scratch[i] + 2 * C + 24; }
    }
    if (rc == AMP_OK && !ampb_supported(c1, c2, n_pairs, acts, (size_t)na, B, T)) {
        set_error("amp_ampblock_forward: block (C=%d k=%d, %d pairs, B=%d T=%d) is not covered by the whole-AMPBlock kernel under the "
                  "current amp_set_ampblock_fusion mode (run the convs and activations one by one: the same bits)", c1[0]->cin, c1[0]->k, n_pairs, B, T);
        rc = AMP_ERR_UNSUPPORTED;
    }
    if (rc == AMP_OK) rc = ampb_run(c1, c2, n_pairs, acts, x_dev, B, T, y_dev, mode, div, (hipStream_t)stream);
    hipError_t e = hipStreamSynchronize((hipStream_t)stream);
    for (int i = 0; i < na; ++i) if (scratch[i]) (void)hipFree(scratch[i]);
    if (rc == AMP_OK && e != hipSuccess) { set_error("amp_ampblock_forward: %s", hipGetErrorString(e)); return AMP_ERR_HIP; }
    return rc;
}

int amp_conv_forward_mrf(const amp_conv* c, const float* x_dev, int B, int T, float slope_in, const float* res_dev,
                         float* y_dev, int mode, float div, void* stream) {
    if (!c || !x_dev || !y_dev) { set_error("amp_conv_forward_mrf: null argument"); return AMP_ERR_INVALID; }
    if (x_dev == y_dev) { set_error("amp_conv_forward_mrf: x and y must not alias (the conv reads a halo)"); return AMP_ERR_INVALID; }
    if (mode < 0 || mode > 2 || (mode == 2 && !(div > 0.f))) { set_error("amp_conv_forward_mrf: mode=%d div=%g", mode, (double)div); return AMP_ERR_INVALID; }
    return conv_run(c, x_dev, B, T, slope_in, res_dev, 1.f, y_dev, mode, div, (hipStream_t)stream);
}

int amp_conv_set_option(amp_conv* c, int option, int value) {
    if (!c) { set_error("amp_conv_set_option: null handle"); return AMP_ERR_INVALID; }
    if (option == AMP_CONV_OPT_PAD_REFLECT) {
        if (value && c->transposed) { set_error("amp_conv_set_option: reflection padding on a transposed conv"); return AMP_ERR_UNSUPPORTED; }
        c->pad_reflect = value != 0;
    } else if (option == AMP_CONV_OPT_TANH) {
        if (value && c->transposed) { set_error("amp_conv_set_option: tanh on a transposed conv"); return AMP_ERR_UNSUPPORTED; }
        c->tanh_out = value != 0;
    } else {
        set_error("amp_conv_set_option: unknown option %d", option);
        return AMP_ERR_INVALID;
    }
    return AMP_OK;
}

void amp_conv_destroy(amp_conv* c) { delete c; }

}
```

amphion_amd/csrc/generator.hip:

```cpp
#include <math.h>
#include <stdio.h>

#include <map>
#include <memory>
#include <mutex>
#include <string>
#include <vector>

#include "amp_host.h"

using namespace amp;

struct HostTensor {
    std::vector<int64_t> shape;
    std::vector<float> data;
    size_t numel() const { size_t n = 1; for (auto s : shape) n *= (size_t)s; return n; }
};

struct ResBlock {
    int k = 0;
    std::vector<int> dil;
    std::vector<std::unique_ptr<amp_conv>> c1, c2;
    std::vector<ActParams> acts;
};
// ... 122 lines not shown

int amp_gen_set_weight(amp_gen* g, const char* ref_key, const float* data_host, const int64_t* shape, int ndim) {
    if (!g || !ref_key || !data_host || (!shape && ndim > 0)) { set_error("amp_gen_set_weight: null argument"); return AMP_ERR_INVALID; }
    if (g->finalized) { set_error("amp_gen_set_weight: handle already finalized"); return AMP_ERR_STATE; }
    std::string key(ref_key);
    if (key.rfind("module.", 0) == 0) key = key.substr(7);
    auto it = g->expected.find(key);
    if (it == g->expected.end()) { set_error("amp_gen_set_weight: unexpected key '%s'", ref_key); return AMP_ERR_INVALID; }
    HostTensor t;
    t.shape.assign(shape, shape + ndim);
    if (t.shape != it->second) {
        std::string got, want;
        for (auto s : t.shape) got += std::to_string(s) + ",";
        for (auto s : it->second) want += std::to_string(s) + ",";
        set_error("amp_gen_set_weight: '%s' has shape (%s) expected (%s)", ref_key, got.c_str(), want.c_str());
        return AMP_ERR_INVALID;
    }
    hipPointerAttribute_t attr{};
    const bool on_device = hipPointerGetAttributes(&attr, data_host) == hipSuccess && attr.type == hipMemoryTypeDevice;
    if (!on_device) (void)hipGetLastError();
    if (on_device) {
        t.data.resize(t.numel());
        AMP_HIP(hipMemcpy(t.data.data(), data_host, t.numel() * sizeof(float), hipMemcpyDeviceToHost));
    } else {
        t.data.assign(data_host, data_host + t.numel());
    }
    g->w[key] = std::move(t);
    return AMP_OK;
}

}

static bool get_folded(amp_gen* g, const std::string& p, std::vector<float>* wout, const float** bias, bool need_bias) {
    auto itw = g->w.find(p + ".weight");
    if (itw != g->w.end()) {
        *wout = itw->second.data;
    } else {
        auto ig = g->w.find(p + ".weight_g"), iv = g->w.find(p + ".weight_v");
        if (ig == g->w.end() || iv == g->w.end()) { set_error("amp_gen_finalize: missing weight for '%s'", p.c_str()); return false; }
        const HostTensor& V = iv->second;
        const size_t d0 = (size_t)V.shape[0], inner = V.numel() / d0;
        wout->resize(V.numel());
        for (size_t r = 0; r < d0; ++r) {
            double ss = 0.0;
            for (size_t i = 0; i < inner; ++i) { const double v = V.data[r * inner + i]; ss += v * v; }
            const float nrm = (float)sqrt(ss);
            const float sc = ig->second.data[r] / nrm;
            for (size_t i = 0; i < inner; ++i) (*wout)[r * inner + i] = V.data[r * inner + i] * sc;
        }
    }
    *bias = nullptr;
    auto ib = g->w.find(p + ".bias");
    if (ib != g->w.end()) *bias = ib->second.data.data();
    else if (need_bias) { set_error("amp_gen_finalize: missing '%s.bias'", p.c_str()); return false; }
    return true;
}

static int upload(amp_gen* g, const float* src, size_t n, float** dst) {
    AMP_RC(device_upload(src, n * sizeof(float), (void**)dst));
    g->dev_allocs.push_back(*dst);
    return AMP_OK;
}

static int build_act(amp_gen* g, const std::string& p, int c, ActParams* out) {
    auto ia = g->w.find(p + ".act.alpha");
    if (ia == g->w.end()) { set_error("amp_gen_finalize: missing '%s.act.alpha'", p.c_str()); return AMP_ERR_MISSING_WEIGHT; }
    const std::vector<float>* beta = nullptr;
    if (g->d.activation == AMP_ACT_SNAKEBETA) {
        auto ib = g->w.find(p + ".act.beta");
        if (ib == g->w.end()) { set_error("amp_gen_finalize: missing '%s.act.beta'", p.c_str()); return AMP_ERR_MISSING_WEIGHT; }
        beta = &ib->second.data;
    }
    auto iu = g->w.find(p + ".upsample.filter"), idn = g->w.find(p + ".downsample.lowpass.filter");
    if (iu == g->w.end() || idn == g->w.end()) { set_error("amp_gen_finalize: missing anti-aliasing filter buffers of '%s'", p.c_str()); return AMP_ERR_MISSING_WEIGHT; }
    std::vector<float> a(c), ib(c);
    for (int i = 0; i < c; ++i) {
        float al = ia->second.data[i];
        float be = beta ? (*beta)[i] : al;
        if (g->d.snake_logscale) { al = expf(al); be = expf(be); }
        a[i] = al;
        ib[i] = 1.0f / (be + 0.000000001f);
    }
    int rc;
    if ((rc = upload(g, a.data(), c, &out->a_dev)) != AMP_OK) return rc;
    if ((rc = upload(g, ib.data(), c, &out->invb_dev)) != AMP_OK) return rc;
    if ((rc = upload(g, iu->second.data.data(), 12, &out->fu_dev)) != AMP_OK) return rc;
    if ((rc = upload(g, idn->second.data.data(), 12, &out->fd_dev)) != AMP_OK) return rc;
    float fu2[12];
    for (int i = 0; i < 12; ++i) fu2[i] = 2.f * iu->second.data[i];
    if ((rc = upload(g, fu2, 12, &out->fu2_dev)) != AMP_OK) return rc;
    return AMP_OK;
}

static int make_conv(amp_gen* g, const std::string& p, bool transposed, int cin, int cout, int k, int stride, int dil,
                     int pad, bool need_bias, std::unique_ptr<amp_conv>* out) {
    std::vector<float> w;
    const float* bias = nullptr;
    if (!get_folded(g, p, &w, &bias, need_bias)) return AMP_ERR_MISSING_WEIGHT;
    auto c = std::make_unique<amp_conv>();
    c->transposed = transposed; c->cin = cin; c->cout = cout; c->k = k; c->stride = stride; c->dilation = dil; c->padding = pad;
    int rc = conv_build(c.get(), w.data(), bias);
    if (rc != AMP_OK) return rc;
    *out = std::move(c);
    return AMP_OK;
}

extern "C" {

int amp_gen_finalize(amp_gen* g) {
    if (!g) { set_error("amp_gen_finalize: null handle"); return AMP_ERR_INVALID; }
    if (g->finalized) return AMP_OK;
    if (amp_device_count() <= 0) { set_error("amp_gen_finalize: no HIP device visible (the HIP path has no CPU fallback)"); return AMP_ERR_HIP; }
    const amp_gen_desc& d = g->d;
    const bool vits = d.arch == AMP_ARCH_HIFIGAN_VITS;
    const int c0 = d.upsample_initial_channel;
    int rc;
    if ((rc = make_conv(g, "conv_pre", false, d.n_in, c0, 7, 1, 1, 3, true, &g->conv_pre)) != AMP_OK) return rc;
    if (vits && d.gin_channels > 0)
        if ((rc = make_conv(g, "cond", false, d.gin_channels, c0, 1, 1, 1, 0, true, &g->cond)) != AMP_OK) return rc;
    int ch = c0;
    for (int i = 0; i < d.n_stages; ++i) {
        const int u = d.upsample_rates[i], k = d.upsample_kernel_sizes[i];
        const int cin = c0 >> i, cout = c0 >> (i + 1);
        std::unique_ptr<amp_conv> up;
        if ((rc = make_conv(g, ups_key(g, i), true, cin, cout, k, u, 1, (k - u) / 2, true, &up)) != AMP_OK) return rc;
        g->ups.push_back(std::move(up));
        ch = cout;
        for (int j = 0; j < d.n_kernels; ++j) {
            ResBlock rb;
            rb.k = d.resblock_kernel_sizes[j];
            const std::string pre = "resblocks." + std::to_string(i * d.n_kernels + j);
            for (int p = 0; p < d.n_dilations[j]; ++p) {
                const int dl = d.resblock_dilation_sizes[j][p];
                rb.dil.push_back(dl);
                std::unique_ptr<amp_conv> a, b;
                const int pad1 = (rb.k * dl - dl) / 2;
                if (d.resblock_type == 1) {
                    if ((rc = make_conv(g, pre + ".convs1." + std::to_string(p), false, cout, cout, rb.k, 1, dl, pad1, true, &a)) != AMP_OK) return rc;
                    if ((rc = make_conv(g, pre + ".convs2." + std::to_string(p), false, cout, cout, rb.k, 1, 1, (rb.k - 1) / 2, true, &b)) != AMP_OK) return rc;
                    rb.c1.push_back(std::move(a));
                    rb.c2.push_back(std::move(b));
                } else {
                    if ((rc = make_conv(g, pre + ".convs." + std::to_string(p), false, cout, cout, rb.k, 1, dl, pad1, true, &a)) != AMP_OK) return rc;
                    rb.c1.push_back(std::move(a));
                }
            }
            if (d.arch == AMP_ARCH_BIGVGAN) {
                const int nact = d.resblock_type == 1 ? 2 * d.n_dilations[j] : d.n_dilations[j];
                rb.acts.resize(nact);
                for (int m = 0; m < nact; ++m)
                    if ((rc = build_act(g, pre + ".activations." + std::to_string(m), cout, &rb.acts[m])) != AMP_OK) return rc;
            }
            g->rbs.push_back(std::move(rb));
        }
    }
    if (d.arch == AMP_ARCH_BIGVGAN)
        if ((rc = build_act(g, "activation_post", ch, &g->act_post)) != AMP_OK) return rc;
    {
        std::vector<float> w;
        const float* bias = nullptr;
        if (!get_folded(g, "conv_post", &w, &bias, !vits)) return AMP_ERR_MISSING_WEIGHT;
        g->post_cin = ch;
        if ((rc = upload(g, w.data(), w.size(), &g->post_w_dev)) != AMP_OK) return rc;
        if (bias) if ((rc = upload(g, bias, 1, &g->post_b_dev)) != AMP_OK) return rc;
    }
    if (!guard_init(g->guard)) { set_error("amp_gen_finalize: cannot allocate the range-guard word"); return AMP_ERR_HIP; }
    g->w.clear();
    g->finalized = true;
    return AMP_OK;
}

int amp_gen_hop(const amp_gen* g) { return g ? g->hop : 0; }

static size_t gen_buf_elems(const amp_gen* g, int B, int T) {
    size_t mx = (size_t)B * g->d.upsample_initial_channel * T;
    int t = T;
    for (int i = 0; i < g->d.n_stages; ++i) {
        t *= g->d.upsample_rates[i];
        const size_t e = (size_t)B * g->ch[i] * t;
        if (e > mx) mx = e;
    }
    return (mx + 63) & ~(size_t)63;
}

static int gen_num_bufs(const amp_gen* g) { return g->d.arch == AMP_ARCH_BIGVGAN ? 6 : 5; }

constexpr long long kRbHorizontalMaxFrames = 1024;
constexpr long long kRbStreamsMaxFrames = 4096;
static int gen_side_bufs(const amp_gen* g) { return (g->d.n_kernels - 1) * (g->d.arch == AMP_ARCH_BIGVGAN ? 4 : 3); }
static bool gen_streams_wanted(const amp_gen* g, int B, int T) {
    if (g->d.n_kernels < 2) return false;
    const int m = cfg().rb_streams;
    return m == 1 || (m < 0 && (long long)B * T <= kRbStreamsMaxFrames);
}

static size_t group_target_bytes() { return cfg().group_bytes; }

static int gen_group_items(const amp_gen* g, int B, int T) {
    const size_t target = group_target_bytes();
    if (target == 0) return B;
    const size_t per_item = gen_buf_elems(g, 1, T) * sizeof(float) * (size_t)(gen_num_bufs(g) - 1);
    size_t n = target / (per_item ? per_item : 1);
    if (n < 1) n = 1;
    return n < (size_t)B ? (int)n : B;
}

size_t amp_gen_workspace_bytes(const amp_gen* g, int B, int T) {
    if (!g || B <= 0 || T <= 0) return 0;
    const int G = gen_group_items(g, B, T);
    const int nb = gen_num_bufs(g) + ((G == B && gen_streams_wanted(g, B, T)) ? gen_side_bufs(g) : 0);
    return gen_buf_elems(g, G, T) * sizeof(float) * nb + (size_t)G * g->d.upsample_initial_channel * sizeof(float) + 256;
}

int amp_gen_set_profiling(amp_gen* g, int slots) {
    if (!g || slots < 0 || slots > 4096) { set_error("amp_gen_set_profiling: bad argument"); return AMP_ERR_INVALID; }
    for (auto& p : g->prof) {
        if (p.ev_begin) (void)hipEventDestroy(p.ev_begin);
        if (p.ev_end) (void)hipEventDestroy(p.ev_end);
        for (auto e : p.ev_mrf) (void)hipEventDestroy(e);
        for (auto e : p.ev_rb) (void)hipEventDestroy(e);
    }
    g->prof.clear();
    g->prof.resize((size_t)slots);
    g->prof_count = 0;
    for (auto& p : g->prof) {
        AMP_HIP(hipEventCreate(&p.ev_begin));
        AMP_HIP(hipEventCreate(&p.ev_end));
    }
    return AMP_OK;
}

int amp_gen_timing_ms(amp_gen* g, int back, int which, float* ms_out) {
    if (!g || !ms_out) { set_error("amp_gen_timing_ms: null argument"); return AMP_ERR_INVALID; }
    if (g->prof.empty() || back < 0 || (size_t)back >= g->prof.size() || (size_t)back >= g->prof_count) {
        set_error("amp_gen_timing_ms: no profiled forward %d back (slots=%zu, recorded=%zu)", back, g->prof.size(), g->prof_count);
        return AMP_ERR_STATE;
    }
    const amp_gen::ProfSlot& p = g->prof[(g->prof_count - 1 - (size_t)back) % g->prof.size()];
    if (!p.valid) { set_error("amp_gen_timing_ms: slot not recorded"); return AMP_ERR_STATE; }
    AMP_HIP(hipEventSynchronize(p.ev_end));
    if (which == 0) {
        AMP_HIP(hipEventElapsedTime(ms_out, p.ev_begin, p.ev_end));
    } else if (which >= 1 && which < 2 + g->d.n_stages) {
        float tot = 0.f;
        for (int gi = 0; gi < p.ev_groups; ++gi)
            for (int i = 0; i < g->d.n_stages; ++i) {
                if (which >= 2 && i != which - 2) continue;
                float ms = 0.f;
                const size_t e = 2 * ((size_t)g->d.n_stages * gi + i);
                AMP_HIP(hipEventElapsedTime(&ms, p.ev_mrf[e], p.ev_mrf[e + 1]));
                tot += ms;
            }
        *ms_out = tot;
    } else if (which >= 100 && which < 100 + 16 * g->d.n_stages && (which - 100) % 16 < g->d.n_kernels) {
        const int i = (which - 100) / 16, j = (which - 100) % 16, nk = g->d.n_kernels;
        float tot = 0.f;
        for (int gi = 0; gi < p.ev_groups; ++gi) {
            float ms = 0.f;
            const size_t e = (size_t)g->d.n_stages * (nk + 1) * gi + (size_t)i * (nk + 1) + j;
            AMP_HIP(hipEventElapsedTime(&ms, p.ev_rb[e], p.ev_rb[e + 1]));
            tot += ms;
        }
        *ms_out = tot;
    } else {
        set_error("amp_gen_timing_ms: which=%d", which);
        return AMP_ERR_INVALID;
    }
    return AMP_OK;
}

int amp_gen_last_timing_ms(amp_gen* g, int which, float* ms_out) { return amp_gen_timing_ms(g, 0, which, ms_out); }

int amp_gen_kernel_name(amp_gen* g, int back, int which, char* buf, size_t n) {
    if (!g || !buf || n == 0) { set_error("amp_gen_kernel_name: null argument"); return AMP_ERR_INVALID; }
    if (g->prof.empty() || back < 0 || (size_t)back >= g->prof.size() || (size_t)back >= g->prof_count) {
        set_error("amp_gen_kernel_name: no profiled forward %d back (slots=%zu, recorded=%zu)", back, g->prof.size(), g->prof_count);
        return AMP_ERR_STATE;
    }
    const amp_gen::ProfSlot& p = g->prof[(g->prof_count - 1 - (size_t)back) % g->prof.size()];
    const int i = (which - 100) / 16, j = (which - 100) % 16;
    if (which < 100 || i >= g->d.n_stages || j >= g->d.n_kernels || (size_t)(i * g->d.n_kernels + j) >= p.rb_kernels.size()) {
        set_error("amp_gen_kernel_name: which=%d", which);
        return AMP_ERR_INVALID;
    }
    snprintf(buf, n, "%s", p.rb_kernels[(size_t)i * g->d.n_kernels + j].c_str());
    return AMP_OK;
}

constexpr float kLreluSlope = 0.1f;

struct Stage {
    amp_gen* g;
    int i;
    int B, t, C, lm;
    const int* lens;
    hipStream_t st;
    bool conc;
    const float* U;
    float* XS;
    float *R, *TMP, *ACT;
    float* SIDE;
    int side_per;
    size_t be;
    const ResBlock& rb(int j) const { return g->rbs[(size_t)i * g->d.n_kernels + j]; }
};

constexpr int kMaxFusedPairs = AMP_AMPB_MAX_STEPS / 2 > AMP_RB_MAX_PAIRS ? AMP_AMPB_MAX_STEPS / 2 : AMP_RB_MAX_PAIRS;
struct RbPtrs {
    const amp_conv *c1[kMaxFusedPairs], *c2[kMaxFusedPairs];
    int n = 0;
    explicit RbPtrs(const ResBlock& rb) {
        if (rb.c1.size() > (size_t)kMaxFusedPairs || rb.c2.size() != rb.c1.size()) return;
        n = (int)rb.c1.size();
        for (int p = 0; p < n; ++p) { c1[p] = rb.c1[p].get(); c2[p] = rb.c2[p].get(); }
    }
};

static int accumulate_mode(int j, int nk) { return j == 0 ? 0 : (j == nk - 1 ? 2 : 1); }

struct RbBufs { float *R, *TMP, *XS, *ACT; };
static RbBufs rb_bufs(const Stage& s, int j, bool own) {
    if (!own || j == 0) return {s.R, s.TMP, s.XS, s.ACT};
    float* SB = s.SIDE + (size_t)(j - 1) * s.side_per * s.be;
    return {SB, SB + s.be, SB + 2 * s.be, s.ACT ? SB + 3 * s.be : nullptr};
}

static int launch_stage_mrf_sum(const Stage& s, const hipEvent_t* evs) {
    const int nk = s.g->d.n_kernels;
    MrfSumArgs ma{};
    ma.y = s.XS; ma.n = nk - 1; ma.div = (float)nk; ma.count = (size_t)s.B * s.C * s.t;
    for (int j = 1; j < nk; ++j) {
        if (evs) AMP_HIP(hipStreamWaitEvent(s.st, evs[1 + j], 0));
        ma.p[j - 1] = rb_bufs(s, j, true).XS;
    }
    AMP_HIP(launch_mrf_sum(ma, s.st));
    return AMP_OK;
}

static bool horizontal_slots(const Stage& s, int slot_of[3]) {
    slot_of[0] = slot_of[1] = slot_of[2] = -1;
    for (int j = 0; j < 3; ++j) {
        const int k = s.rb(j).c1[0]->k;
        const int sl = k == 11 ? 0 : k == 7 ? 1 : k == 3 ? 2 : -1;
        if (sl < 0 || slot_of[sl] >= 0) return false;
        slot_of[sl] = j;
    }
    return true;
}

static int try_stage_pair3(const Stage& s, const int slot_of[3], bool* ran) {
    *ran = false;
    const int nk = s.g->d.n_kernels;
    const size_t nd = s.rb(0).dil.size();
    std::vector<Pair3Args> plan(nd);
    for (int sl = 0; sl < 3; ++sl) {
        const int j = slot_of[sl];
        const ResBlock& rb = s.rb(j);
        if (rb.dil.size() != nd) return AMP_OK;
        const RbBufs b = rb_bufs(s, j, true);
        const float* cur = s.U;
        for (size_t p = 0; p < nd; ++p) {
            float* dst = p + 1 == nd ? b.XS : (cur == b.R ? b.TMP : b.R);
            if (!pair_tile_args(rb.c1[p].get(), rb.c2[p].get(), cur, s.B, s.t, kLreluSlope, dst, 0, (float)nk, s.lens, s.lm, &plan[p].a[sl]))
                return AMP_OK;
            plan[p].n[sl] = s.B * plan[p].a[sl].tiles_per_item;
            cur = dst;
        }
    }
    for (const Pair3Args& p : plan) AMP_HIP(launch_pair3(p, s.st));
    AMP_RC(launch_stage_mrf_sum(s, nullptr));
    *ran = true;
    return AMP_OK;
}

static int try_stage_small3(const Stage& s, const int slot_of[3], bool* ran) {
    *ran = false;
    const int nk = s.g->d.n_kernels;
    for (int j = 0; j < 3; ++j)
        if (pair_supported(s.rb(j).c1[0].get(), s.rb(j).c2[0].get())) return AMP_OK;
    const size_t nd = s.rb(0).dil.size();
    struct Step { ConvSmall3Args p; int ni[3]; };
    std::vector<Step> steps;
    const float* cur[3] = {s.U, s.U, s.U};
    RbBufs b[3];
    for (int j = 0; j < 3; ++j) b[j] = rb_bufs(s, j, true);
    auto plan3 = [&](bool second, size_t p) -> bool {
        Step sp{};
        for (int sl = 0; sl < 3; ++sl) {
            const int j = slot_of[sl];
            const amp_conv* c = second ? s.rb(j).c2[p].get() : s.rb(j).c1[p].get();
            const int rc = second ? conv_run(c, b[j].TMP, s.B, s.t, 1.f, cur[j], 1.f, b[j].R, 0, 1.f, s.st, 0, s.lens, s.lm, &sp.p.a[sl], &sp.ni[sl])
                                  : conv_run(c, cur[j], s.B, s.t, kLreluSlope, nullptr, kLreluSlope, b[j].TMP, 0, 1.f, s.st, 0, s.lens, s.lm, &sp.p.a[sl], &sp.ni[sl]);
            if (rc != AMP_OK) return false;
            sp.p.nx[sl] = s.B * sp.p.a[sl].tiles_per_item;
            sp.p.ny[sl] = (sp.p.a[sl].M + 127) / 128;
        }
        if (sp.ni[1] != 1 || sp.ni[2] != 1) return false;
        steps.push_back(sp);
        return true;
    };
    bool ok = true;
    for (size_t p = 0; ok && p < nd; ++p) {
        for (int j = 0; j < 3 && ok; ++j) ok = s.rb(j).dil.size() == nd;
        ok = ok && plan3(false, p);
        if (ok && p + 1 < nd) {
            ok = plan3(true, p);
            for (int j = 0; j < 3; ++j) cur[j] = b[j].R;
        }
    }
    for (int j = 0; ok && j < 3; ++j) {
        ConvArgs unused_a; int unused_ni;
        ok = conv_run(s.rb(j).c2[nd - 1].get(), b[j].TMP, s.B, s.t, 1.f, cur[j], 1.f, s.XS, accumulate_mode(j, nk), (float)nk, s.st, 0, s.lens,
                      s.lm, &unused_a, &unused_ni) == AMP_OK;
    }
    if (!ok) return AMP_OK;
    for (const Step& sp : steps) AMP_HIP(launch_conv_small3(sp.p, sp.ni, s.st));
    for (int j = 0; j < 3; ++j)
        AMP_RC(conv_run(s.rb(j).c2[nd - 1].get(), b[j].TMP, s.B, s.t, 1.f, cur[j], 1.f, s.XS, accumulate_mode(j, nk), (float)nk, s.st, 0, s.lens, s.lm));
    *ran = true;
    return AMP_OK;
}

static int wait_before_last(hipEvent_t wait, hipStream_t sj) {
    if (wait) AMP_HIP(hipStreamWaitEvent(sj, wait, 0));
    return AMP_OK;
}

static int run_resblock1(const Stage& s, const ResBlock& rb, const RbBufs& b, int mode_last, hipEvent_t wait, hipStream_t sj) {
    const int B = s.B, t = s.t;
    const float nk = (float)s.g->d.n_kernels;
    const int nd = (int)rb.dil.size();
    RbPtrs q(rb);
    if (q.n && rb_supported(q.c1, q.c2, nd, B, t)) {
        const int sp = rb_split(q.c1, nd, B, t);
        if (sp > 0) AMP_RC(rb_run(q.c1, q.c2, nd, s.U, B, t, kLreluSlope, b.R, 0, 1.f, sj, s.lens, s.lm, 0, sp));
        AMP_RC(wait_before_last(wait, sj));
        return rb_run(q.c1, q.c2, nd, sp > 0 ? b.R : s.U, B, t, kLreluSlope, b.XS, mode_last, nk, sj, s.lens, s.lm, sp, -1);
    }
    const float* cur = s.U;
    for (int p = 0; p < nd; ++p) {
        const bool last = p == nd - 1;
        const amp_conv *c1 = rb.c1[p].get(), *c2 = rb.c2[p].get();
        if (pair_supported(c1, c2)) {
            float* dst = last ? b.XS : (cur == b.R ? b.TMP : b.R);
            if (last) AMP_RC(wait_before_last(wait, sj));
            AMP_RC(pair_run(c1, c2, cur, B, t, kLreluSlope, dst, last ? mode_last : 0, nk, sj, s.lens, s.lm));
            cur = dst;
            continue;
        }
        if (cur == b.TMP) {
            AMP_HIP(hipMemcpyAsync(b.R, b.TMP, (size_t)B * s.C * t * sizeof(float), hipMemcpyDeviceToDevice, sj));
            cur = b.R;
        }
        AMP_RC(conv_run(c1, cur, B, t, kLreluSlope, nullptr, kLreluSlope, b.TMP, 0, 1.f, sj, 0, s.lens, s.lm));
        if (!last) { AMP_RC(conv_run(c2, b.TMP, B, t, 1.f, cur, 1.f, b.R, 0, 1.f, sj, 0, s.lens, s.lm)); cur = b.R; }
        else { AMP_RC(wait_before_last(wait, sj)); AMP_RC(conv_run(c2, b.TMP, B, t, 1.f, cur, 1.f, b.XS, mode_last, nk, sj, 0, s.lens, s.lm)); }
    }
    return AMP_OK;
}

static int run_ampblock1(const Stage& s, const ResBlock& rb, const RbBufs& b, int mode_last, hipEvent_t wait, hipStream_t sj) {
    const int B = s.B, t = s.t, nd = (int)rb.dil.size();
    const float nk = (float)s.g->d.n_kernels;
    RbPtrs q(rb);
    if (q.n && ampb_supported(q.c1, q.c2, nd, rb.acts.data(), rb.acts.size(), B, t)) {
        AMP_RC(wait_before_last(wait, sj));
        return ampb_run(q.c1, q.c2, nd, rb.acts.data(), s.U, B, t, b.XS, mode_last, nk, sj, s.lens, s.lm);
    }
    const float* cur = s.U;
    for (int p = 0; p < nd; ++p) {
        const ActParams& a1 = rb.acts[2 * p];
        const ActParams& a2 = rb.acts[2 * p + 1];
        AMP_HIP(launch_act1d(cur, b.ACT, B, s.C, t, a1.a_dev, a1.invb_dev, a1.fu_dev, a1.fd_dev, s.lens, s.lm, sj, next_rev(s.lens)));
        AMP_RC(conv_run(rb.c1[p].get(), b.ACT, B, t, 1.f, nullptr, 1.f, b.TMP, 0, 1.f, sj, 0, s.lens, s.lm));
        AMP_HIP(launch_act1d(b.TMP, b.ACT, B, s.C, t, a2.a_dev, a2.invb_dev, a2.fu_dev, a2.fd_dev, s.lens, s.lm, sj, next_rev(s.lens)));
        if (p < nd - 1) { AMP_RC(conv_run(rb.c2[p].get(), b.ACT, B, t, 1.f, cur, 1.f, b.R, 0, 1.f, sj, 0, s.lens, s.lm)); cur = b.R; }
        else { AMP_RC(wait_before_last(wait, sj)); AMP_RC(conv_run(rb.c2[p].get(), b.ACT, B, t, 1.f, cur, 1.f, b.XS, mode_last, nk, sj, 0, s.lens, s.lm)); }
    }
    return AMP_OK;
}

static int run_resblock2(const Stage& s, const ResBlock& rb, const RbBufs& b, int mode_last, hipEvent_t wait, hipStream_t sj) {
    const bool big = s.g->d.arch == AMP_ARCH_BIGVGAN;
    const int B = s.B, t = s.t, nd = (int)rb.dil.size();
    const float* cur = s.U;
    for (int p = 0; p < nd; ++p) {
        const float* in = cur;
        float sl = kLreluSlope;
        if (big) {
            const ActParams& a1 = rb.acts[p];
            AMP_HIP(launch_act1d(cur, b.ACT, B, s.C, t, a1.a_dev, a1.invb_dev, a1.fu_dev, a1.fd_dev, s.lens, s.lm, sj, next_rev(s.lens)));
            in = b.ACT;
            sl = 1.f;
        }
        if (p < nd - 1) {
            float* dst = (in == cur && cur == b.R) ? b.TMP : b.R;
            AMP_RC(conv_run(rb.c1[p].get(), in, B, t, sl, cur, 1.f, dst, 0, 1.f, sj, 0, s.lens, s.lm));
            cur = dst;
        } else {
            AMP_RC(wait_before_last(wait, sj));
            AMP_RC(conv_run(rb.c1[p].get(), in, B, t, sl, cur, 1.f, b.XS, mode_last, (float)s.g->d.n_kernels, sj, 0, s.lens, s.lm));
        }
    }
    return AMP_OK;
}

static bool stage_sums_separately(const Stage& s) {
    const amp_gen_desc& d = s.g->d;
    if (!s.conc || d.resblock_type != 1 || d.arch == AMP_ARCH_BIGVGAN || d.n_kernels - 1 > AMP_MRF_MAX_PARTS) return false;
    for (int j = 0; j < d.n_kernels; ++j) {
        const ResBlock& rb = s.rb(j);
        const size_t last = rb.dil.size() - 1;
        RbPtrs q(rb);
        if (!(q.n && rb_supported(q.c1, q.c2, q.n, s.B, s.t)) && !pair_supported(rb.c1[last].get(), rb.c2[last].get())) return false;
    }
    return true;
}

struct KernelLogScope {
    explicit KernelLogScope(std::string* p) { tl_kernel_log = p; if (p) p->clear(); }
    ~KernelLogScope() { tl_kernel_log = nullptr; }
};

static int run_stage_resblocks(const Stage& s, hipEvent_t* ev_rb, std::vector<std::string>* rb_names) {
    amp_gen* g = s.g;
    const int nk = g->d.n_kernels;
    const size_t ev0 = (size_t)s.i * (nk + 1);
    hipEvent_t* evs = s.conc ? &g->ev_side[ev0] : nullptr;
    const bool sum_stage = stage_sums_separately(s);
    if (s.conc) {
        AMP_HIP(hipEventRecord(evs[0], s.st));
        for (int j = 1; j < nk; ++j) AMP_HIP(hipStreamWaitEvent(g->side[j - 1], evs[0], 0));
    }
    for (int j = 0; j < nk; ++j) {
        const hipStream_t sj = (s.conc && j > 0) ? g->side[j - 1] : s.st;
        RbBufs b = rb_bufs(s, j, s.conc);
        if (!sum_stage) b.XS = s.XS;
        const hipEvent_t wait = (s.conc && !sum_stage && j > 0) ? evs[j] : nullptr;
        const int mode_last = sum_stage ? 0 : accumulate_mode(j, nk);
        if (ev_rb) AMP_HIP(hipEventRecord(ev_rb[ev0 + j], sj));
        {
            KernelLogScope log_scope(rb_names ? &(*rb_names)[(size_t)s.i * nk + j] : nullptr);
            const ResBlock& rb = s.rb(j);
            if (g->d.resblock_type != 1) AMP_RC(run_resblock2(s, rb, b, mode_last, wait, sj));
            else if (g->d.arch == AMP_ARCH_BIGVGAN) AMP_RC(run_ampblock1(s, rb, b, mode_last, wait, sj));
            else AMP_RC(run_resblock1(s, rb, b, mode_last, wait, sj));
        }
        if (s.conc) AMP_HIP(hipEventRecord(evs[1 + j], sj));
    }
    if (s.conc && !sum_stage) AMP_HIP(hipStreamWaitEvent(s.st, evs[nk], 0));
    if (sum_stage) AMP_RC(launch_stage_mrf_sum(s, evs));
    if (ev_rb) AMP_HIP(hipEventRecord(ev_rb[ev0 + nk], s.st));
    return AMP_OK;
}

static int gen_forward_group(amp_gen* g, const float* mel_dev, const float* cond_dev, const int* lens, int B, int T,
                             float* wav_dev, float* base, size_t be, hipStream_t st,
                             hipEvent_t* ev_mrf , hipEvent_t* ev_rb ,
                             std::vector<std::string>* rb_names = nullptr ,
                             bool conc = false ) {
    const amp_gen_desc& d = g->d;
    const bool big = d.arch == AMP_ARCH_BIGVGAN;
    float* X = base;
    float* XS = base + be;
    float* U = base + 2 * be;
    Stage s{};
    s.g = g; s.B = B; s.lens = lens; s.st = st; s.conc = conc; s.U = U;
    s.R = base + 3 * be;
    s.TMP = base + 4 * be;
    s.ACT = big ? base + 5 * be : nullptr;
    s.SIDE = base + (size_t)gen_num_bufs(g) * be;
    s.side_per = big ? 4 : 3;
    s.be = be;
    float* CB = base + (size_t)(gen_num_bufs(g) + (conc ? gen_side_bufs(g) : 0)) * be;

    AMP_RC(conv_run(g->conv_pre.get(), mel_dev, B, T, 1.f, nullptr, 1.f, X, 0, 1.f, st, 0, lens, 1));
    if (cond_dev) {
        AMP_RC(conv_run(g->cond.get(), cond_dev, B, 1, 1.f, nullptr, 1.f, CB, 0, 1.f, st));
        AMP_HIP(launch_add_channel_bias(X, CB, B, d.upsample_initial_channel, T, st));
    }
    const bool horizontal = conc && (long long)B * T <= kRbHorizontalMaxFrames && d.resblock_type == 1 && !big && d.n_kernels == 3;
    int t = T;
    int lm = 1;
    for (int i = 0; i < d.n_stages; ++i) {
        AMP_RC(conv_run(g->ups[i].get(), X, B, t, big ? 1.f : kLreluSlope, nullptr, 1.f, U, 0, 1.f, st, 0, lens, lm));
        t *= d.upsample_rates[i];
        lm *= d.upsample_rates[i];
        if (ev_mrf) AMP_HIP(hipEventRecord(ev_mrf[2 * i], st));
        s.i = i; s.t = t; s.C = g->ch[i]; s.lm = lm; s.XS = XS;
        bool ran = false;
        int slot_of[3];
        if (horizontal && horizontal_slots(s, slot_of)) {
            AMP_RC(try_stage_pair3(s, slot_of, &ran));
            if (!ran) AMP_RC(try_stage_small3(s, slot_of, &ran));
        }
        if (!ran) AMP_RC(run_stage_resblocks(s, ev_rb, rb_names));
        if (ev_mrf) AMP_HIP(hipEventRecord(ev_mrf[2 * i + 1], st));
        float* tmp = X; X = XS; XS = tmp;
    }
    if (big) {
        AMP_HIP(launch_act1d(X, s.ACT, B, g->post_cin, t, g->act_post.a_dev, g->act_post.invb_dev, g->act_post.fu_dev, g->act_post.fd_dev, lens, lm, st, next_rev(lens)));
        AMP_HIP(launch_conv_post(s.ACT, g->post_w_dev, g->post_b_dev, wav_dev, B, g->post_cin, t, 7, 1.f, 1, lens, lm, st));
    } else {
        AMP_HIP(launch_conv_post(X, g->post_w_dev, g->post_b_dev, wav_dev, B, g->post_cin, t, 7, 0.01f, 1, lens, lm, st));
    }
    return AMP_OK;
}

static bool gen_ensure_side(amp_gen* g, hipStream_t st) {
    const size_t ns = (size_t)g->d.n_kernels - 1, ne = (size_t)g->d.n_stages * (g->d.n_kernels + 1);
    if (g->side.size() == ns && g->ev_side.size() == ne) return true;
    hipStreamCaptureStatus cs = hipStreamCaptureStatusNone;
    if (hipStreamIsCapturing(st, &cs) != hipSuccess || cs != hipStreamCaptureStatusNone) { (void)hipGetLastError(); return false; }
    while (g->side.size() < ns) {
        hipStream_t s_ = nullptr;
        if (hipStreamCreateWithFlags(&s_, hipStreamNonBlocking) != hipSuccess) { (void)hipGetLastError(); return false; }
        g->side.push_back(s_);
    }
    while (g->ev_side.size() < ne) {
        hipEvent_t e = nullptr;
        if (hipEventCreateWithFlags(&e, hipEventDisableTiming) != hipSuccess) { (void)hipGetLastError(); return false; }
        g->ev_side.push_back(e);
    }
    return true;
}

int amp_gen_prepare_streams(amp_gen* g) {
    if (!g || !g->finalized) { set_error("amp_gen_prepare_streams: null or unfinalized handle"); return AMP_ERR_STATE; }
    if (g->d.n_kernels < 2) return AMP_OK;
    if (!gen_ensure_side(g, nullptr)) { set_error("amp_gen_prepare_streams: could not create the side streams"); return AMP_ERR_HIP; }
    return AMP_OK;
}

int amp_gen_forward(amp_gen* g, const float* mel_dev, const float* cond_dev, int B, int T, float* wav_dev,
                    void* workspace_dev, size_t workspace_bytes, void* stream_) {
    return amp_gen_forward_ragged(g, mel_dev, cond_dev, nullptr, B, T, wav_dev, workspace_dev, workspace_bytes, stream_);
}

int amp_gen_forward_ragged(amp_gen* g, const float* mel_dev, const float* cond_dev, const int32_t* lens_dev, int B, int T,
                           float* wav_dev, void* workspace_dev, size_t workspace_bytes, void* stream_) {
    if (!g || !mel_dev || !wav_dev || !workspace_dev) { set_error("amp_gen_forward: null argument"); return AMP_ERR_INVALID; }
    if (!g->finalized) { set_error("amp_gen_forward: call amp_gen_finalize first"); return AMP_ERR_STATE; }
    if (B <= 0 || T <= 0) { set_error("amp_gen_forward: B=%d T=%d", B, T); return AMP_ERR_INVALID; }
    if (workspace_bytes < amp_gen_workspace_bytes(g, B, T)) { set_error("amp_gen_forward: workspace too small (%zu < %zu)", workspace_bytes, amp_gen_workspace_bytes(g, B, T)); return AMP_ERR_INVALID; }
    if (cond_dev && !g->cond) { set_error("amp_gen_forward: cond given but gin_channels == 0"); return AMP_ERR_INVALID; }
    hipStream_t st = (hipStream_t)stream_;
    std::lock_guard<std::mutex> launch_lock(g->launch_mu);
    AMP_RC(range_poll(&g->guard, st));
    RangeFlagScope flag_scope(g->guard.dev);
    const amp_gen_desc& d = g->d;
    const int G = gen_group_items(g, B, T);
    const int ngroups = (B + G - 1) / G;
    const size_t be = gen_buf_elems(g, G, T);
    const size_t L = (size_t)T * g->hop;
    amp_gen::ProfSlot* ps = g->prof.empty() ? nullptr : &g->prof[g->prof_count % g->prof.size()];
    const bool conc = ngroups == 1 && !ps && gen_streams_wanted(g, B, T) && gen_ensure_side(g, st);
    if (ps) {
        const size_t need = 2 * (size_t)d.n_stages * ngroups;
        while (ps->ev_mrf.size() < need) {
            hipEvent_t e;
            AMP_HIP(hipEventCreate(&e));
            ps->ev_mrf.push_back(e);
        }
        const size_t need_rb = (size_t)d.n_stages * (d.n_kernels + 1) * ngroups;
        while (ps->ev_rb.size() < need_rb) {
            hipEvent_t e;
            AMP_HIP(hipEventCreate(&e));
            ps->ev_rb.push_back(e);
        }
        ps->ev_groups = ngroups;
        ps->rb_kernels.assign((size_t)d.n_stages * d.n_kernels, std::string());
        AMP_HIP(hipEventRecord(ps->ev_begin, st));
    }
    for (int gi = 0; gi < ngroups; ++gi) {
        const int b0 = gi * G;
        const int Bg = (B - b0) < G ? (B - b0) : G;
        AMP_RC(gen_forward_group(g, mel_dev + (size_t)b0 * d.n_in * T,
                                 cond_dev ? cond_dev + (size_t)b0 * d.gin_channels : nullptr,
                                 lens_dev ? lens_dev + b0 : nullptr, Bg, T,
                                 wav_dev + (size_t)b0 * L, (float*)workspace_dev, be, st,
                                 ps ? ps->ev_mrf.data() + 2 * (size_t)d.n_stages * gi : nullptr,
                                 ps ? ps->ev_rb.data() + (size_t)d.n_stages * (d.n_kernels + 1) * gi : nullptr,
                                 (ps && gi == 0) ? &ps->rb_kernels : nullptr, conc));
    }
    if (ps) { AMP_HIP(hipEventRecord(ps->ev_end, st)); ps->valid = true; ++g->prof_count; }
    AMP_RC(range_publish(&g->guard, st));
    return AMP_OK;
}

int amp_gen_range_check(amp_gen* g, void* stream_) {
    if (!g) { set_error("amp_gen_range_check: null handle"); return AMP_ERR_INVALID; }
    return range_check_sync(&g->guard, (hipStream_t)stream_, "amp_gen_range_check");
}

void amp_gen_destroy(amp_gen* g) { delete g; }

}
```

amphion_amd/csrc/rb_f16x3.hip:

```cpp
#include "f16x3_device.h"

#ifndef AMP_KT
#error "compile with -DAMP_KT=<taps>"
#endif

namespace amp {


template <int KT, int WM, int WN, int NI, int RING = 0, int RB_G = 32>
__global__ __launch_bounds__(64 * WM * WN, 2) void rb_f16x3_kernel(const RbArgs a) {
    static_assert(RING == 0 || RING < KT, "a ring shorter than one chunk");
    constexpr int NTHR = 64 * WM * WN;
    constexpr int W = 32 * NI * WN;
    constexpr int WL = W + 2 * RB_G;
    constexpr int H2 = (KT - 1) / 2;
    constexpr int NCH = 2 * WM;
    constexpr int CHS = 4 * WL;
    constexpr int C = 32 * WM;
    static_assert(NI % 2 == 0, "B fragments are read in halves");
    extern __shared__ __attribute__((aligned(16))) uint4 smem4[];

    const int tid = threadIdx.x;
    const int lane = tid & 63;
    const int wave = __builtin_amdgcn_readfirstlane(tid >> 6);
    const int wm = wave / WN, wn = wave % WN;
    const int hi = lane >> 5, l31 = lane & 31;
    const int nbx = gridDim.x;
    int bx = tile_order(blockIdx.x, nbx, a.lens != nullptr, a.rev);
    const int item = bx / a.tiles_per_item;
    const int tile = bx - item * a.tiles_per_item;
    const int T = a.T;
    const int RH = a.rh;
    const int NT = W - 2 * RH;
    const int O0 = tile * NT;
    int Tv = T;
    if (a.lens) { const int l = a.lens[item] * a.len_mul; Tv = l < Tv ? l : Tv; }
    if (O0 >= Tv) return;
    const int q0 = O0 - RH;

    for (int i = tid; i < NCH * 4 * 2 * RB_G; i += NTHR) {
        const int row = i / (2 * RB_G), g = i - row * (2 * RB_G);
        smem4[row * WL + (g < RB_G ? g : W + g)] = make_uint4(0u, 0u, 0u, 0u);
    }

    const int colw = wn * (32 * NI) + l31;
    int qcl[NI];
    bool qok[NI];
#pragma unroll
    for (int t = 0; t < NI; ++t) {
        const int q = q0 + colw + 32 * t;
        qok[t] = (q >= 0) && (q < Tv);
        qcl[t] = q < 0 ? 0 : (q < T ? q : T - 1);
    }
    const float* xr = a.x + (size_t)item * C * T + (size_t)(32 * wm + 16 * hi) * T;
    f32x16 rv[NI];
#pragma unroll
    for (int t = 0; t < NI; ++t)
#pragma unroll
        for (int r = 0; r < 16; ++r) rv[t][r] = xr[(size_t)r * T + qcl[t]];

    constexpr size_t MBS = (size_t)NCH * (KT * 128);
    constexpr int NA = RING > 0 ? RING : KT;
    Frag a_h[NA], a_l[NA];
    const int wlane = (lane & 32) | (16 * ((lane >> 2) & 1) + 4 * ((lane >> 3) & 3) + (lane & 3));
    {
        const uint4* w0 = static_cast<const uint4*>(a.wp1[0]) + (size_t)wm * MBS + wlane;
#pragma unroll
        for (int g = 0; g < NA; ++g) {
            a_h[g].u = w0[g * 128];
            a_l[g].u = w0[g * 128 + 64];
        }
    }
    AMP_PIN_VMEM();

    float range_max = 0.f;
    const float kpos = 16.f, kneg = 16.f * a.slope;
    auto stage_x = [&]() __attribute__((always_inline)) {
#pragma unroll
        for (int t = 0; t < NI; ++t) {
            const int col = RB_G + colw + 32 * t;
            const bool ok = qok[t];
            const int o4 = (2 * wm + hi) * CHS + col;
#pragma unroll
            for (int o = 0; o < 2; ++o) {
                struct { uint2 u; } fh0, fl0, fh1, fl1;
                stage4_f16(ok ? rv[t][8 * o + 0] : 0.f, ok ? rv[t][8 * o + 1] : 0.f, ok ? rv[t][8 * o + 2] : 0.f,
                           ok ? rv[t][8 * o + 3] : 0.f, kpos, kneg, range_max, fh0.u, fl0.u);
                stage4_f16(ok ? rv[t][8 * o + 4] : 0.f, ok ? rv[t][8 * o + 5] : 0.f, ok ? rv[t][8 * o + 6] : 0.f,
                           ok ? rv[t][8 * o + 7] : 0.f, kpos, kneg, range_max, fh1.u, fl1.u);
                smem4[o4 + o * WL] = make_uint4(fh0.u.x, fh0.u.y, fh1.u.x, fh1.u.y);
                smem4[o4 + o * WL + 2 * WL] = make_uint4(fl0.u.x, fl0.u.y, fl1.u.x, fl1.u.y);
            }
        }
    };

    f32x16 acc[NI];
    auto conv = [&](const void* wp, const float* bias, float sc, int d, const void* wp_next) __attribute__((always_inline)) {
#pragma unroll
        for (int r = 0; r < 16; ++r) {
            const float bv = bias[32 * wm + 16 * hi + r] * sc;
#pragma unroll
            for (int t = 0; t < NI; ++t) acc[t][r] = bv;
        }
        const uint4* wa = static_cast<const uint4*>(wp) + (size_t)wm * MBS + wlane;
        const uint4* wn0 = static_cast<const uint4*>(wp_next) + (size_t)wm * MBS + wlane;
        const int rd = hi * WL + RB_G + colw - H2 * d;
#pragma unroll 1
        for (int c = 0; c < NCH; ++c) {
            const uint4* wcur = wa + (size_t)c * (KT * 128);
            const uint4* wan = (c + 1) < NCH ? wa + (size_t)(c + 1) * (KT * 128) : wn0;
            const uint4* base = smem4 + c * CHS + rd;
#pragma unroll
            for (int g = 0; g < KT; ++g) {
                const int v = RING > 0 ? g % NA : g;
                const uint4* bg = base + g * d;
                constexpr int NB = NI / 2;
#pragma unroll
                for (int th = 0; th < 2; ++th) {
                    Frag bh[NB], bl[NB];
#pragma unroll
                    for (int t = 0; t < NB; ++t) {
                        bh[t].u = bg[32 * (th * NB + t)];
                        bl[t].u = bg[2 * WL + 32 * (th * NB + t)];
                    }
                    mfma3<NB>(acc + th * NB, a_h[v], a_l[v], bh, bl);
                }
                {
                    const bool same = RING > 0 && g + RING < KT;
                    const uint4* src = same ? wcur + (size_t)(g + RING) * 128 : wan + (size_t)v * 128;
                    a_h[v].u = src[0];
                    a_l[v].u = src[64];
                }
                AMP_PIN_VMEM();
            }
        }
    };

    stage_x();
    __syncthreads();

    const int np = a.np;
#pragma unroll 1
    for (int p = 0; p < AMP_RB_MAX_PAIRS; ++p) {
        if (p < np) {
            const bool last = (p + 1 == np);
            conv(a.wp1[p], a.bias1[p], a.sc1[p], a.dil[p], a.wp2[p]);
            __syncthreads();
            {
                const float i1 = a.isc1[p];
                const float slope = a.slope;
#pragma unroll
                for (int t = 0; t < NI; ++t) {
                    const int o4 = (2 * wm + hi) * CHS + RB_G + colw + 32 * t;
#pragma unroll
                    for (int o = 0; o < 2; ++o) {
                        struct { uint2 u; } fh0, fl0, fh1, fl1;
                        seam4_f16(acc[t][8 * o + 0], acc[t][8 * o + 1], acc[t][8 * o + 2], acc[t][8 * o + 3], i1, slope, qok[t], range_max, fh0.u, fl0.u);
                        seam4_f16(acc[t][8 * o + 4], acc[t][8 * o + 5], acc[t][8 * o + 6], acc[t][8 * o + 7], i1, slope, qok[t], range_max, fh1.u, fl1.u);
                        smem4[o4 + o * WL] = make_uint4(fh0.u.x, fh0.u.y, fh1.u.x, fh1.u.y);
                        smem4[o4 + o * WL + 2 * WL] = make_uint4(fl0.u.x, fl0.u.y, fl1.u.x, fl1.u.y);
                    }
                }
            }
            __syncthreads();
            conv(a.wp2[p], a.bias2[p], a.sc2[p], 1, last ? a.wp2[p] : a.wp1[p + 1 < AMP_RB_MAX_PAIRS ? p + 1 : p]);
            {
                const float i2 = a.isc2[p];
#pragma unroll
                for (int t = 0; t < NI; ++t)
#pragma unroll
                    for (int r = 0; r < 16; ++r) rv[t][r] = __builtin_fmaf(acc[t][r], i2, rv[t][r]);
            }
            if (!last) {
                __syncthreads();
                stage_x();
                __syncthreads();
            }
        }
    }

    {
        const int mode = a.mode;
        float* yr = a.y + (size_t)item * C * T + (size_t)(32 * wm + 16 * hi) * T;
        if (mode != 0) {
#pragma unroll
            for (int t = 0; t < NI; ++t)
#pragma unroll
                for (int r = 0; r < 16; ++r) acc[t][r] = yr[(size_t)r * T + qcl[t]];
#pragma unroll
            for (int t = 0; t < NI; ++t) rv[t] += acc[t];
            if (mode == 2) {
#pragma unroll
                for (int t = 0; t < NI; ++t)
#pragma unroll
                    for (int r = 0; r < 16; ++r) rv[t][r] = rv[t][r] / a.div;
            }
        }
#pragma unroll
        for (int t = 0; t < NI; ++t) {
            const int col = colw + 32 * t;
            const int q = q0 + col;
            if (col >= RH && col < W - RH && q < T) {
#pragma unroll
                for (int r = 0; r < 16; ++r) yr[(size_t)r * T + qcl[t]] = rv[t][r];
            }
        }
    }
    if (a.range_flag && __any(range_max > 65504.f) && lane == 0) atomicOr(a.range_flag, 1u);
}

template <int KT, int WM, int WN, int NI, int RING = 0, int RB_G = 32>
static hipError_t launch_rb_one(const RbArgs& a, hipStream_t stream) {
    constexpr int W = 32 * NI * WN;
    const size_t lds = (size_t)2 * WM * 4 * (W + 2 * RB_G) * sizeof(uint4);
    if (hipError_t e = ensure_dynamic_lds<&rb_f16x3_kernel<KT, WM, WN, NI, RING, RB_G>>(lds); e != hipSuccess) return e;
    dim3 grid((unsigned)(a.B * a.tiles_per_item));
    note_kernel("rb_f16x3_kernel", KT, WM, WN, NI, RING, RB_G);
    note_work(grid.x, a.np * 2 * 2.0 * a.C * a.C * KT * (double)a.T * a.B / 1e9, 4.0 * a.B * (double)a.C * a.T * (2 + (a.mode ? 1 : 0)) / 1e6,
              "whole ResBlock C=%d k=%d T=%d B=%d: %d convs%s", a.C, KT, a.T, a.B, 2 * a.np, a.mode ? " +sum" : "");
    hipLaunchKernelGGL((rb_f16x3_kernel<KT, WM, WN, NI, RING, RB_G>), grid, dim3(64 * WM * WN), lds, stream, a);
    return hipGetLastError();
}

template <int KT>
int rb_tile(int C, int max_dil, int wide) {
    const int reach = (KT - 1) / 2 * max_dil;
    if (reach > 32) return 0;
    if (C == 32) return wide ? 1024 : 512;
    if (C == 64) return wide ? 512 : ((KT <= 5 && reach <= 16) ? 256 : 0);
    if (C == 128) return (wide && KT <= 5 && reach <= 16) ? 256 : 0;
    return 0;
}

template <int KT>
hipError_t launch_rb(const RbArgs& a, int wide, hipStream_t stream) {
    constexpr int RING = KT >= 7 ? 4 : 0;
    if (a.C == 32) return wide ? launch_rb_one<KT, 1, 8, 4, RING>(a, stream) : launch_rb_one<KT, 1, 4, 4, RING>(a, stream);
    if (a.C == 64 && wide) return launch_rb_one<KT, 2, 4, 4, RING>(a, stream);
    if constexpr (KT <= 5) {
        if (a.C == 64 && !wide) return launch_rb_one<KT, 2, 2, 4, 0, 16>(a, stream);
    }
    if constexpr (KT <= 5) {
        if (a.C == 128 && wide) return launch_rb_one<KT, 4, 2, 4, 0, 16>(a, stream);
    }

    return hipErrorInvalidValue;
}

template int rb_tile<AMP_KT>(int, int, int);
template hipError_t launch_rb<AMP_KT>(const RbArgs&, int, hipStream_t);

}
```

amphion_amd/csrc/runtime.hip:

```cpp
#include <stdarg.h>
#include <stdio.h>
#include <stdlib.h>
#include <string.h>

#include <mutex>
#include <string>

#include "amp_host.h"

namespace amp {

static thread_local char g_err[512] = "";

void set_error(const char* fmt, ...) {
    va_list ap;
    va_start(ap, fmt);
    vsnprintf(g_err, sizeof(g_err), fmt, ap);
    va_end(ap);
}

static RangeGuard g_guard[64];
__thread std::string* tl_kernel_log = nullptr;
__thread char tl_last_kernel[160] = "";
__thread int tl_conv_transposed = 0;
static FILE* manifest_file() {
    static FILE* f = [] {
        const char* p = getenv("AMP_LAUNCH_MANIFEST");
        return (p && *p) ? fopen(p, "a") : nullptr;
    }();
    return f;
}
bool manifest_on() {
    static const bool on = manifest_file() != nullptr;
    return on;
}
void manifest_add(const char* name, unsigned long long workgroups, double gflop, double mb, const char* what) {
    static std::mutex mu;
    std::lock_guard<std::mutex> lk(mu);
    FILE* f = manifest_file();
    if (!f) return;
    fprintf(f, "%s\t%llu\t%.6f\t%.6f\t%s\n", name, workgroups, gflop, mb, what);
    fflush(f);
    tl_last_kernel[0] = '\0';
}
static thread_local unsigned* tl_range_flag = nullptr;
RangeFlagScope::RangeFlagScope(unsigned* word) { tl_range_flag = word; }
RangeFlagScope::~RangeFlagScope() { tl_range_flag = nullptr; }

bool guard_init(RangeGuard& g) {
    if (g.dev) return true;
    if (hipMalloc(&g.dev, sizeof(unsigned)) != hipSuccess) { g.dev = nullptr; return false; }
    if (hipMemset(g.dev, 0, sizeof(unsigned)) != hipSuccess || hipHostMalloc(&g.host, sizeof(unsigned)) != hipSuccess ||
        hipEventCreateWithFlags(&g.ev, hipEventDisableTiming) != hipSuccess) {
        (void)hipFree(g.dev);
        g.dev = nullptr;
        return false;
    }
    *g.host = 0;
    return true;
}

void guard_free(RangeGuard& g) {
    if (g.dev) (void)hipFree(g.dev);
    if (g.host) (void)hipHostFree(g.host);
    if (g.ev) (void)hipEventDestroy(g.ev);
    g = RangeGuard{};
}

static RangeGuard* guard_for_current_device() {
    int dev = 0;
    if (hipGetDevice(&dev) != hipSuccess || dev < 0 || dev >= 64) return nullptr;
    return guard_init(g_guard[dev]) ? &g_guard[dev] : nullptr;
}

unsigned* range_flag_for_current_device() {
    if (tl_range_flag) return tl_range_flag;
    RangeGuard* g = guard_for_current_device();
    return g ? g->dev : nullptr;
}

static bool stream_is_capturing(hipStream_t st) {
    hipStreamCaptureStatus cs = hipStreamCaptureStatusNone;
    return hipStreamIsCapturing(st, &cs) == hipSuccess && cs != hipStreamCaptureStatusNone;
}

static const char kRangeMsg[] =
    "an activation left the split-f16 operand range of the f16x3 kernels (|x| > 4094 or infinite) in a previous "
    "launch: its output is not the fp32 reference's; re-run with amp_set_precision(AMP_PRECISION_F32)";

int range_poll(RangeGuard* g, hipStream_t st) {
    if (!g || !g->dev || !g->pending || stream_is_capturing(st)) return AMP_OK;
    if (hipEventQuery(g->ev) != hipSuccess) return AMP_OK;
    g->pending = false;
    if (*g->host == 0) return AMP_OK;
    *g->host = 0;
    AMP_HIP(hipMemsetAsync(g->dev, 0, sizeof(unsigned), st));
    set_error("%s", kRangeMsg);
    return AMP_ERR_RANGE;
}

int range_publish(RangeGuard* g, hipStream_t st) {
    if (!g || !g->dev || stream_is_capturing(st)) return AMP_OK;
    AMP_HIP(hipMemcpyAsync(g->host, g->dev, sizeof(unsigned), hipMemcpyDeviceToHost, st));
    AMP_HIP(hipEventRecord(g->ev, st));
    g->pending = true;
    return AMP_OK;
}

int range_check_sync(RangeGuard* g, hipStream_t st, const char* who) {
    if (!g || !g->dev) return AMP_OK;
    if (stream_is_capturing(st)) { set_error("%s: the stream is capturing", who); return AMP_ERR_STATE; }
    AMP_HIP(hipMemcpyAsync(g->host, g->dev, sizeof(unsigned), hipMemcpyDeviceToHost, st));
    AMP_HIP(hipStreamSynchronize(st));
    g->pending = false;
    const unsigned v = *g->host;
    *g->host = 0;
    if (v == 0) return AMP_OK;
    AMP_HIP(hipMemsetAsync(g->dev, 0, sizeof(unsigned), st));
    set_error("%s", kRangeMsg);
    return AMP_ERR_RANGE;
}

static int g_precision = -1;
int default_precision() {
    if (g_precision < 0) {
        const char* e = getenv("AMP_PRECISION");
        g_precision = (e && (!strcmp(e, "f32") || !strcmp(e, "fp32"))) ? PREC_F32 : PREC_F16X3;
    }
    return g_precision;
}

Config::Config() {
    auto num = [](const char* name, int lo, int hi, int dflt) {
        const char* e = getenv(name);
        if (!e || !*e) return dflt;
        const int v = atoi(e);
        return (v < lo || v > hi) ? dflt : v;
    };
    rb_fusion = num("AMP_RB_FUSION", 0, 3, 1);
    ampb_fusion = num("AMP_AMPB_FUSION", 0, 3, 1);
    rb_streams = num("AMP_RB_STREAMS", -1, 1, -1);
    static const char* const kRemoved[][2] = {
        {"AMP_GROUP_MB", "amp_set_group_mb(megabytes)"}, {"AMP_PAIR_STRIP", "amp_set_pair_strips(mode)"}, {"AMP_CONV_BLK", "amp_set_conv_blk(mode)"},
        {"AMP_FUSE_PAIRS", "nothing (the fused pairs are the only form)"}, {"AMP_RB_SUM_FRAMES", "nothing"},
        {"AMP_RB_HORIZONTAL", "amp_set_resblock_streams(mode)"}, {"AMP_RB_HORIZONTAL_FRAMES", "amp_set_resblock_streams(mode)"}};
    for (const auto& r : kRemoved) {
        const char* e = getenv(r[0]);
        if (e && *e) fprintf(stderr, "libamphion_hip: the environment variable %s=%s is no longer read (removed in ABI 142); use %s\n", r[0], e, r[1]);
    }
}
Config& cfg() { static Config c; return c; }

int device_upload(const void* host, size_t bytes, void** out) {
    void* p = nullptr;
    AMP_HIP(hipMalloc(&p, bytes));
    const hipError_t e = hipMemcpy(p, host, bytes, hipMemcpyHostToDevice);
    if (e != hipSuccess) {
        (void)hipFree(p);
        set_error("hipMemcpy of %zu bytes to the device failed: %s", bytes, hipGetErrorString(e));
        return AMP_ERR_HIP;
    }
    *out = p;
    return AMP_OK;
}

}

using namespace amp;

extern "C" {

int amp_version(void) { return 150; }
const char* amp_last_error(void) { return g_err; }

int amp_set_precision(int precision) {
    if (precision != AMP_PRECISION_F32 && precision != AMP_PRECISION_F16X3) {
        set_error("amp_set_precision: unknown precision %d", precision);
        return AMP_ERR_INVALID;
    }
    g_precision = precision;
    return AMP_OK;
}

int amp_get_precision(void) { return default_precision(); }

int amp_device_count(void) {
    int n = 0;
    if (hipGetDeviceCount(&n) != hipSuccess) return 0;
    return n;
}

int amp_set_pair_strips(int on) {
    if (on < -1 || on > 0) { set_error("amp_set_pair_strips: %d (-1 the policy, 0 the per-tile kernel everywhere; the four-wave strips of mode 1 left in ABI 142)", on); return AMP_ERR_INVALID; }
    cfg().pair_strips = on;
    return AMP_OK;
}

int amp_set_group_mb(int megabytes) {
    if (megabytes < 0) { set_error("amp_set_group_mb: %d", megabytes); return AMP_ERR_INVALID; }
    cfg().group_bytes = (size_t)megabytes << 20;
    return AMP_OK;
}

int amp_set_resblock_streams(int mode) {
    if (mode < -1 || mode > 1) { set_error("amp_set_resblock_streams: mode=%d", mode); return AMP_ERR_INVALID; }
    cfg().rb_streams = mode;
    return AMP_OK;
}

int amp_set_small_conv(int on) {
    cfg().small_conv = on ? 1 : 0;
    return AMP_OK;
}

int amp_set_pingpong(int on) {
    cfg().pingpong = on < 0 ? kPingPongDefault : (on ? 1 : 0);
    return AMP_OK;
}

int amp_set_conv_rg_fast(int on) {
    cfg().conv_rg_fast = on < 0 ? kConvRgFastDefault : (on ? 1 : 0);
    return AMP_OK;
}

int amp_set_conv_blk_narrow(int on) {
    if (on < -1 || on > 2) { set_error("amp_set_conv_blk_narrow: %d (0 off, 1 policy: 128-row convs with k >= 7, 2 every 128-row conv, -1 default)", on); return AMP_ERR_INVALID; }
    cfg().narrow_blk = on < 0 ? 1 : on;
    return AMP_OK;
}

int amp_set_conv_blk(int mode) {
    if (mode < -1 || mode > 3) { set_error("amp_set_conv_blk: mode %d (0 off, 1 | 2 chunks per staging round, 3 = 2 + k = 7 / 11, -1 default)", mode); return AMP_ERR_INVALID; }
    cfg().conv_blk = mode < 0 ? kConvBlkDefault : mode;
    return AMP_OK;
}

int amp_set_resblock_fusion(int mode) {
    if (mode < -1 || mode > 3) { set_error("amp_set_resblock_fusion: mode=%d", mode); return AMP_ERR_INVALID; }
    cfg().rb_fusion = mode < 0 ? 1 : mode;
    return AMP_OK;
}

int amp_set_ampblock_fusion(int mode) {
    if (mode < -1 || mode > 3) { set_error("amp_set_ampblock_fusion: mode=%d", mode); return AMP_ERR_INVALID; }
    cfg().ampb_fusion = mode < 0 ? 1 : mode;
    return AMP_OK;
}

int amp_range_check(void* stream_) {
    return range_check_sync(guard_for_current_device(), (hipStream_t)stream_, "amp_range_check");
}

}
```

include/amphion_hip.h:

```cpp
#ifndef AMPHION_HIP_H
#define AMPHION_HIP_H

#include <stddef.h>
#include <stdint.h>

#ifdef __cplusplus
extern "C" {
#endif

typedef enum amp_status {
    AMP_OK = 0,
    AMP_ERR_INVALID = -1,
    AMP_ERR_MISSING_WEIGHT = -2,
    AMP_ERR_HIP = -3,
    AMP_ERR_UNSUPPORTED = -4,
    AMP_ERR_STATE = -5,
    AMP_ERR_RANGE = -6
} amp_status;

typedef enum amp_arch {
    AMP_ARCH_HIFIGAN = 0,
    AMP_ARCH_BIGVGAN = 1,
    AMP_ARCH_HIFIGAN_VITS = 2
} amp_arch;

typedef enum amp_activation {
    AMP_ACT_LRELU = 0,
    AMP_ACT_SNAKE = 1,
    AMP_ACT_SNAKEBETA = 2
} amp_activation;

typedef enum amp_precision {
    AMP_PRECISION_F32 = 0,
    AMP_PRECISION_F16X3 = 1
} amp_precision;

#define AMP_MAX_STAGES 8
#define AMP_MAX_KERNELS 8
#define AMP_MAX_DILATIONS 8

typedef struct amp_gen_desc {
    int32_t arch;
    int32_t n_in;
    int32_t upsample_initial_channel;
    int32_t n_stages;
    int32_t upsample_rates[AMP_MAX_STAGES];
    int32_t upsample_kernel_sizes[AMP_MAX_STAGES];
    int32_t n_kernels;
    int32_t resblock_kernel_sizes[AMP_MAX_KERNELS];
    int32_t n_dilations[AMP_MAX_KERNELS];
    int32_t resblock_dilation_sizes[AMP_MAX_KERNELS][AMP_MAX_DILATIONS];
    int32_t resblock_type;
    int32_t activation;
    int32_t snake_logscale;
    int32_t gin_channels;
} amp_gen_desc;

typedef struct amp_gen amp_gen;

int amp_version(void);
const char* amp_last_error(void);
int amp_device_count(void);

int amp_set_precision(int precision );
int amp_get_precision(void);


int amp_gen_create(const amp_gen_desc* desc, amp_gen** out);

int amp_gen_set_weight(amp_gen* g, const char* ref_key, const float* data_host, const int64_t* shape, int ndim);

int amp_gen_finalize(amp_gen* g);

int amp_gen_hop(const amp_gen* g);
size_t amp_gen_workspace_bytes(const amp_gen* g, int B, int T);

int amp_set_group_mb(int megabytes);

int amp_range_check(void* stream);
int amp_gen_range_check(amp_gen* g, void* stream);

int amp_set_pair_strips(int on);

int amp_gen_forward(amp_gen* g, const float* mel_dev, const float* cond_dev, int B, int T, float* wav_dev,
                    void* workspace_dev, size_t workspace_bytes, void* stream);

int amp_gen_forward_ragged(amp_gen* g, const float* mel_dev, const float* cond_dev, const int32_t* lens_dev, int B,
                           int T, float* wav_dev, void* workspace_dev, size_t workspace_bytes, void* stream);

int amp_gen_set_profiling(amp_gen* g, int slots);
int amp_gen_timing_ms(amp_gen* g, int back, int which, float* ms_out);
int amp_gen_last_timing_ms(amp_gen* g, int which, float* ms_out);
int amp_gen_kernel_name(amp_gen* g, int back, int which, char* buf, size_t n);

void amp_gen_destroy(amp_gen* g);


typedef struct amp_conv amp_conv;

int amp_conv_create(int transposed, int cin, int cout, int k, int stride, int dilation, int padding,
                    const float* weight_host, const float* bias_host, amp_conv** out);
int amp_conv_out_len(const amp_conv* c, int T);
int amp_conv_forward(const amp_conv* c, const float* x_dev, int B, int T, float slope_in, const float* res_dev,
                     float slope_out, float* y_dev, void* stream);
int amp_conv_forward_strided(const amp_conv* c, const float* x_dev, long long x_batch_stride, int B, int T,
                             float slope_in, const float* res_dev, float slope_out, float* y_dev, void* stream);
int amp_conv_forward_ragged(const amp_conv* c, const float* x_dev, long long x_batch_stride, int B, int T, const int32_t* lens_dev,
                            float slope_in, const float* res_dev, float slope_out, float* y_dev, void* stream);
int amp_conv_forward_mrf(const amp_conv* c, const float* x_dev, int B, int T, float slope_in, const float* res_dev,
                         float* y_dev, int mode, float div, void* stream);

int amp_apnet_polar(const float* logamp_dev, const float* r_dev, const float* i_dev, size_t n, float* pha_dev,
                    float* rea_dev, float* imag_dev, void* stream);

#define AMP_FIR_MAX_TAPS 64
int amp_fir_upsample(const float* x_dev, int B, int C, int T, const float* filt_host, int K, int ratio, float* y_dev,
                     void* stream);
typedef enum amp_pad_mode { AMP_PAD_REPLICATE = 0, AMP_PAD_ZEROS = 1, AMP_PAD_REFLECT = 2 } amp_pad_mode;
int amp_fir_filter(const float* x_dev, int B, int C, int T, const float* filt_host, int K, int stride, int pad_left,
                   int pad_right, int pad_mode, float* y_dev, void* stream);

int amp_layer_norm_c(const float* x_dev, const float* res_dev, const float* gamma_dev, const float* beta_dev,
                     const float* post_dev, int B, int C, int T, float eps, int gelu, float* y_dev, void* stream);
int amp_layer_norm_c_ragged(const float* x_dev, const float* res_dev, const float* gamma_dev, const float* beta_dev,
                            const float* post_dev, const int* lens_dev, int B, int C, int T, float eps, int gelu, float* y_dev,
                            void* stream);
int amp_dwconv_layer_norm_c(const float* x_dev, const float* dw_weight_dev, const float* dw_bias_dev, int K, int dilation,
                            const float* gamma_dev, const float* beta_dev, const int* lens_dev, int B, int C, int T, float eps,
                            int gelu, float* y_dev, void* stream);
int amp_dwconv_layer_norm_c_causal(const float* x_dev, const float* dw_weight_dev, const float* dw_bias_dev, int K, int dilation,
                                   const float* gamma_dev, const float* beta_dev, const int* lens_dev, int B, int C, int T, float eps,
                                   int gelu, float* y_dev, void* stream);
int amp_dds_seam(const float* y_dev, const float* x_dev, const float* gamma2_dev, const float* beta2_dev, float eps2,
                 const float* dw_weight_dev, const float* dw_bias_dev, int K, int dilation, const float* gamma1_dev, const float* beta1_dev,
                 float eps1, const int* lens_dev, int B, int C, int T, float* x_out_dev, float* z_out_dev, void* stream);
int amp_add_channel_bias(float* x_dev, const float* cb_dev, int B, int C, int T, void* stream);
int amp_rel_attention(const float* q_dev, const float* k_dev, const float* v_dev, const float* emb_k_dev,
                      const float* emb_v_dev, const int* lens_dev, int B, int H, int dk, int T, int window, float* out_dev,
                      void* stream);
int amp_rel_attention_strided(const float* q_dev, const float* k_dev, const float* v_dev, long long qkv_batch_stride,
                              const float* emb_k_dev, const float* emb_v_dev, const int* lens_dev, int B, int H, int dk, int T,
                              int window, float* out_dev, void* stream);
int amp_set_rel_attention_tiled(int on);
int amp_dwconv(const float* x_dev, const float* w_dev, const float* bias_dev, const int* lens_dev, int B, int C, int T, int K,
               int dilation, float* y_dev, void* stream);
int amp_spline_flow(const float* z_dev, const float* h_dev, const int* lens_dev, int B, int T, int num_bins,
                    int filter_channels, float tail_bound, int inverse, int flip_in, int flip_out, float* z_out_dev,
                    void* stream);
int amp_spline_flow_proj(const float* z_dev, const float* hc_dev, const float* proj_w_dev, const float* proj_b_dev, const int* lens_dev,
                         int B, int C, int T, int num_bins, int filter_channels, float tail_bound, int inverse, int flip_in, int flip_out,
                         float* z_out_dev, void* stream);
int amp_affine_reverse(const float* x_dev, const float* m_dev, const float* logs_dev, const int* lens_dev, int B, int C, int T,
                       float* y_dev, void* stream);
int amp_embed_tokens(const long long* tokens_dev, const float* weight_dev, const int* lens_dev, int B, int T, int hidden,
                     int n_vocab, float scale, float* y_dev, void* stream);
int amp_durations(const float* logw_dev, const int* lens_dev, int B, int T, float length_scale, float* w_ceil_dev, int* cum_dev,
                  int* ylen_dev, void* stream);
int amp_expand_path(const float* src_dev, const int* cum_dev, const int* xlens_dev, const int* ylens_dev, int B, int D, int Tx,
                    int Ty, float* out_dev, float* attn_dev, void* stream);
int amp_expand_path_strided(const float* src_dev, long long src_batch_stride, const int* cum_dev, const int* xlens_dev,
                            const int* ylens_dev, int B, int D, int Tx, int Ty, float* out_dev, float* attn_dev, void* stream);
int amp_gauss_sample(const float* m_dev, const float* logs_dev, const float* noise_dev, size_t n, float noise_scale,
                     float* out_dev, void* stream);

int amp_snake(const float* x_dev, int B, int C, int T, const float* alpha_dev, const float* beta_dev, int logscale,
              float* y_dev, void* stream);

int amp_wav_to_pcm16(const float* wav_dev, int B, int L, long long wav_stride, const int* lens_dev, int16_t* pcm_dev,
                     long long pcm_stride, void* stream);

typedef enum amp_conv_option { AMP_CONV_OPT_PAD_REFLECT = 1, AMP_CONV_OPT_TANH = 2 } amp_conv_option;
int amp_conv_set_option(amp_conv* c, int option, int value);

int amp_pair_forward(const amp_conv* c1, const amp_conv* c2, const float* x_dev, int B, int T, float slope,
                     float* y_dev, void* stream);

int amp_resblock_forward(const amp_conv* const* c1, const amp_conv* const* c2, int n_pairs, const float* x_dev, int B, int T,
                         float slope, float* y_dev, void* stream);
int amp_set_resblock_fusion(int mode);
int amp_set_resblock_streams(int mode);
int amp_gen_prepare_streams(amp_gen* g);

int amp_ampblock_forward(const amp_conv* const* c1, const amp_conv* const* c2, int n_pairs, const float* alpha_dev,
                         const float* beta_dev, int logscale, const float* filt_up_host, const float* filt_down_host,
                         const float* x_dev, int B, int T, float* y_dev, int mode, float div, void* stream);
int amp_set_ampblock_fusion(int mode);

void amp_conv_destroy(amp_conv* c);

int amp_set_small_conv(int on);

int amp_set_conv_blk(int mode);
int amp_set_conv_blk_narrow(int on);

int amp_set_conv_rg_fast(int on);

int amp_set_pingpong(int on);


int amp_conv_create_gated(int hidden, int k, int dilation, int padding, const float* weight_host, const float* bias_host,
                          amp_conv** out);

int amp_wn_forward(const amp_conv* const* in_layers, const amp_conv* const* res_skip_layers, int n_layers, float* x_dev,
                   const float* cond_dev, long long cond_batch_stride, const int32_t* lens_dev, int B, int T,
                   float* acts_ws_dev, float* out_dev, void* stream);


int amp_wn_gate(const float* a_dev, const float* cond_dev, long long cond_batch_stride, float* out_dev, int B, int H,
                int T, void* stream);
int amp_wn_accumulate(float* x_dev, float* out_dev, const float* rs_dev, const int32_t* lens_dev, int B, int H, int T,
                      int first, int last, void* stream);
int amp_sequence_mask(float* x_dev, const int32_t* lens_dev, int B, int C, int T, void* stream);
int amp_coupling_apply(float* x_dev, const float* m_dev, const int32_t* lens_dev, int B, int half_channels, int T,
                       int reverse, void* stream);
int amp_flip_channels(const float* x_dev, float* y_dev, int B, int C, int T, void* stream);
int amp_posterior_sample(const float* stats_dev, const float* eps_dev, const int32_t* lens_dev, float* z_dev, int B,
                         int C, int T, void* stream);

int amp_antialias_snake(const float* x_dev, int B, int C, int T, const float* alpha_dev, const float* beta_dev,
                        int logscale, const float* filt_up_host, const float* filt_down_host, float* y_dev,
                        void* stream);

typedef struct amp_mel_desc {
    uint32_t struct_size;
    int32_t n_fft;
    int32_t win_size;
    int32_t hop_size;
    int32_t n_mel;
    int32_t pad_mode;
    float mag_eps;
    float log_clip;
    const int32_t* mel_bands_dev;
    int32_t* range_dev;
    int32_t* range_host;
    int32_t* range_reset_dev;
    int32_t range_seq;
} amp_mel_desc;

int amp_mel_init(void);
int amp_mel_num_frames(const amp_mel_desc* d, int L);
int amp_mel_forward(const amp_mel_desc* d, const float* wav_dev, int B, int L, const float* window_dev,
                    const float* melbasis_dev, float* mel_dev, float* mag_dev, float* re_dev, float* im_dev,
                    void* stream);

int amp_mel_forward_ragged(const amp_mel_desc* d, const float* wav_dev, const int32_t* lens_dev, int B, int L,
                           const float* window_dev, const float* melbasis_dev, float* mel_dev, float* mag_dev,
                           float* re_dev, float* im_dev, void* stream);

int amp_mel_backward(const amp_mel_desc* d, const int32_t* lens_dev, int B, int L, const float* window_dev,
                     const float* melbasis_dev, const float* mel_linear_dev, const float* mag_dev, const float* re_dev,
                     const float* im_dev, const float* grad_logmel_dev, float* spec_ws_dev, float* frames_ws_dev,
                     float* grad_wav_dev, void* stream);

int amp_istft_forward(const amp_mel_desc* d, const float* mag_dev, const float* phase_dev, int B, int F,
                      const float* window_dev, const float* wss_dev, float* frames_ws_dev, float* wav_dev, void* stream);

int amp_istft_same(const amp_mel_desc* d, const float* re_dev, const float* im_dev, int B, int F, const float* window_dev,
                   const float* envelope_dev, float* frames_ws_dev, float* wav_dev, void* stream);

int amp_istft_same_polar(const amp_mel_desc* d, const float* head_dev, long long head_batch_stride, int B, int F, float mag_clip,
                         const float* window_dev, const float* envelope_dev, float* frames_ws_dev, float* wav_dev, void* stream);

typedef struct amp_pw amp_pw;
typedef enum amp_pw_epilogue { AMP_PW_BIAS = 0, AMP_PW_BIAS_GELU = 1, AMP_PW_SCALE_RES = 2 } amp_pw_epilogue;
int amp_pw_create(int cin, int cout, const float* weight_host, const float* bias_host, amp_pw** out);
int amp_pw_forward(const amp_pw* p, const float* x_dev, long long x_batch_stride, int B, int T, int epilogue,
                   const float* gamma_dev, const float* res_dev, float* y_dev, void* stream);
int amp_pw_precision(const amp_pw* p);
void amp_pw_destroy(amp_pw* p);

typedef struct amp_dw amp_dw;
typedef struct amp_dw_desc {
    int32_t residual_channels;
    int32_t residual_layers;
    int32_t dilation_cycle_length;
    int32_t n_mel;
    int32_t upsample0, upsample1;
    int32_t max_steps;
} amp_dw_desc;
int amp_dw_create(const amp_dw_desc* desc, amp_dw** out);
int amp_dw_set_weight(amp_dw* h, const char* key, const float* data_host, long long count);
int amp_dw_finalize(amp_dw* h);
int amp_dw_precision(const amp_dw* h);
int amp_dw_set_precision(amp_dw* h, int precision);
size_t amp_dw_workspace_bytes(const amp_dw* h, int B, int F);
int amp_dw_condition(const amp_dw* h, const float* mel_dev, int B, int F, float* cond_dev, void* ws_dev, size_t ws_bytes, void* stream);
int amp_dw_embed(const amp_dw* h, const float* steps_dev, int n_steps, float* dconst_dev, void* stream);
int amp_dw_input(const amp_dw* h, const float* audio_dev, int B, int L, float* x_dev, void* stream);
int amp_dw_layer(const amp_dw* h, int layer, const float* x_dev, const float* cond_dev, const float* dconst_dev, long long dconst_batch_stride,
                 const float* skip_in_dev, float* x_out_dev, float* skip_out_dev, int B, int L, void* stream);
int amp_dw_tail(const amp_dw* h, const float* skip_dev, int B, int L, float* eps_dev, void* stream);
int amp_dw_forward(const amp_dw* h, const float* audio_dev, int L, const float* steps_dev, int n_steps, const float* cond_dev, int B, int F,
                   float* eps_dev, void* ws_dev, size_t ws_bytes, void* stream);
int amp_dw_sample_step(const amp_dw* h, float* audio_dev, int L, float step, float c1, float c2, float sigma, const float* noise_dev,
                       const float* cond_dev, int B, int F, void* ws_dev, size_t ws_bytes, void* stream);
void amp_dw_destroy(amp_dw* h);


typedef struct amp_fvq amp_fvq;
int amp_fvq_create(int input_dim, int codebook_dim, int codebook_size, int num_quantizers, int use_l2_normalize,
                   const float* const* in_w_host, const float* const* in_b_host, const float* const* codebook_host,
                   const float* const* out_w_host, const float* const* out_b_host, amp_fvq** out);
int amp_fvq_encode(const amp_fvq* h, const float* z_dev, int B, int T, int n_quantizers, long long* codes_dev, float* zq_dev, float* all_zq_dev,
                   void* stream);
int amp_fvq_decode(const amp_fvq* h, const long long* codes_dev, int n_quantizers, int B, int T, float* out_dev, void* stream);
int amp_fvq_check(amp_fvq* h, void* stream);
void amp_fvq_destroy(amp_fvq* h);
int amp_fvq_encode_ex(const amp_fvq* h, const float* z_dev, long long z_row_stride, const float* sub_dev, int B, int T, int n_quantizers,
                      long long* codes_dev, float* zq_dev, float* all_zq_dev, float* latents_dev, void* stream);
int amp_fvq_decode_add(const amp_fvq* h, const long long* codes_dev, int n_quantizers, int B, int T, const float* add_dev, float* out_dev,
                       void* stream);

int amp_semantic_prepare(const float* hidden_dev, const float* mean_dev, const float* std_dev, int B, int T, int C, int factor, float* out_dev,
                         void* stream);

typedef struct amp_codec_unit amp_codec_unit;
int amp_codec_unit_create(int channels, int dilation, const float* alpha1_host, const float* w1_host, const float* b1_host, const float* alpha2_host,
                          const float* w2_host, const float* b2_host, amp_codec_unit** out);
int amp_codec_unit_fused(const amp_codec_unit* h);
int amp_set_codec_unit_fusion(int mode);
size_t amp_codec_unit_workspace_bytes(const amp_codec_unit* h, int B, int T);
int amp_codec_unit_forward(const amp_codec_unit* h, const float* x_dev, int B, int T, float* y_dev, void* ws_dev, size_t ws_bytes, void* stream);
void amp_codec_unit_destroy(amp_codec_unit* h);

typedef struct amp_sconv amp_sconv;
int amp_sconv_create(int cin, int cout, int stride, int padding, const float* weight_host, const float* bias_host, amp_sconv** out);
int amp_sconv_out_len(const amp_sconv* h, int T);
size_t amp_sconv_workspace_bytes(const amp_sconv* h, int B, int T);
int amp_sconv_forward(const amp_sconv* h, const float* x_dev, int B, int T, const float* alpha_dev, void* ws_dev, size_t ws_bytes, float* y_dev,
                      void* stream);
void amp_sconv_destroy(amp_sconv* h);

typedef struct amp_tconv amp_tconv;
int amp_tconv_create(int cin, int cout, int stride, int padding, int output_padding, const float* weight_host, const float* bias_host,
                     amp_tconv** out);
int amp_tconv_out_len(const amp_tconv* h, int T);
int amp_tconv_fused(const amp_tconv* h);
int amp_set_tconv_fusion(int mode);
size_t amp_tconv_workspace_bytes(const amp_tconv* h, int B, int T);
int amp_tconv_forward(const amp_tconv* h, const float* x_dev, int B, int T, const float* alpha_dev, void* ws_dev, size_t ws_bytes, float* y_dev,
                      void* stream);
void amp_tconv_destroy(amp_tconv* h);

typedef struct amp_aa_unit amp_aa_unit;
int amp_aa_unit_create(int channels, int dilation, const float* alpha1_host, const float* beta1_host, const float* w1_host, const float* b1_host,
                       const float* alpha2_host, const float* beta2_host, const float* w2_host, const float* b2_host, int logscale,
                       const float* filt_up12_host, const float* filt_down12_host, amp_aa_unit** out);
int amp_aa_unit_fused(const amp_aa_unit* h);
int amp_set_aa_unit_fusion(int mode);
size_t amp_aa_unit_workspace_bytes(const amp_aa_unit* h, int B, int T);
int amp_aa_unit_forward(const amp_aa_unit* h, const float* x_dev, int B, int T, float* y_dev, void* ws_dev, size_t ws_bytes, void* stream);
void amp_aa_unit_destroy(amp_aa_unit* h);


int amp_elu_pad(const float* x_dev, int B, int C, int T, int pad_left, int pad_right, int elu, float alpha, float* y_dev, void* stream);

typedef struct amp_lstm amp_lstm;
int amp_lstm_create(int input_size, int hidden, int num_layers, int bidirectional, int skip, const float* const* w_ih_host,
                    const float* const* w_hh_host, const float* const* b_ih_host, const float* const* b_hh_host, amp_lstm** out);
size_t amp_lstm_workspace_bytes(const amp_lstm* h, int B, int T);
int amp_lstm_out_channels(const amp_lstm* h);
int amp_lstm_forward(const amp_lstm* h, const float* x_dev, int B, int T, float* y_dev, void* ws_dev, size_t ws_bytes, void* stream);
int amp_lstm_recur(const amp_lstm* h, int layer, const float* gx_dev, int B, int T, const float* skip_dev, float* y_dev, void* ws_dev, void* stream);
void amp_lstm_destroy(amp_lstm* h);

typedef struct amp_evq amp_evq;
int amp_evq_create(int dim, int codebook_size, int num_quantizers, const float* const* codebook_host, amp_evq** out);
int amp_evq_encode(const amp_evq* h, const float* z_dev, int B, int T, int st, int n_q, long long* codes_dev, float* zq_dev, float* all_zq_dev,
                   void* stream);
int amp_evq_decode(const amp_evq* h, const long long* codes_dev, int n, int st, int B, int T, float* out_dev, void* stream);
int amp_evq_check(amp_evq* h, void* stream);
void amp_evq_destroy(amp_evq* h);


typedef struct amp_dsconv amp_dsconv;
int amp_dsconv_create(int cin, int cout, const float* weight_host, const float* bias_host, amp_dsconv** out);
int amp_dsconv_out_len(const amp_dsconv* h, int T);
size_t amp_dsconv_workspace_bytes(const amp_dsconv* h, int B, int T);
int amp_dsconv_forward(const amp_dsconv* h, const float* x_dev, int B, int T, int gelu, void* ws_dev, size_t ws_bytes, float* y_dev, void* stream);
void amp_dsconv_destroy(amp_dsconv* h);

int amp_gelu(const float* x_dev, long long n, float* y_dev, void* stream);

#ifdef __cplusplus
}
#endif
#endif
```

Before: 145.9 million.

## Fold next stage's ConvTranspose1d upsample into the final resblock kernel

Adds a FOLD variant of the whole-resblock f16x3 kernel that, after the last resblock launch (mode 2, sum/div), restages the averaged output in shared memory and runs the next stage's stride-2 k=4 transposed conv directly, writing the upsampled tensor. The generator uses this when stage fold is on (on by default) for non-concurrent HiFi-GAN type-1 stages. The intent is to save a separate upsample kernel launch and the global write and read of the resblock output between stages. In exchange, tiles overlap by one more column, the folded kernel does extra MFMA work per tile and uses more registers, and the resblock output is no longer written to y on that path.

```diff
diff --git a/amphion_amd/_lib.py b/amphion_amd/_lib.py
--- a/amphion_amd/_lib.py
+++ b/amphion_amd/_lib.py
@@ -215,6 +215,9 @@
     "amp_pair_forward": (c_int, [c_void_p, c_void_p, c_void_p, c_int, c_int, c_float, c_void_p, c_void_p]),
     "amp_resblock_forward": (c_int, [POINTER(c_void_p), POINTER(c_void_p), c_int, c_void_p, c_int, c_int, c_float, c_void_p, c_void_p]),
     "amp_set_resblock_fusion": (c_int, [c_int]),
+    "amp_resblock_upsample_forward": (c_int, [POINTER(c_void_p), POINTER(c_void_p), c_int, c_void_p, c_int, c_int, c_float, c_void_p, c_int, c_float,
+                                              c_void_p, c_void_p, c_void_p]),
+    "amp_set_stage_fold": (c_int, [c_int]),
     "amp_conv_destroy": (None, [c_void_p]),
     "amp_set_small_conv": (c_int, [c_int]),
     "amp_set_conv_blk": (c_int, [c_int]),
diff --git a/amphion_amd/csrc/amp_host.h b/amphion_amd/csrc/amp_host.h
--- a/amphion_amd/csrc/amp_host.h
+++ b/amphion_amd/csrc/amp_host.h
@@ -61,6 +61,7 @@
 constexpr int kConvBlkDefault = 3;
 constexpr int kConvRgFastDefault = 1;
 constexpr int kPingPongDefault = 1;
+constexpr int kStageFoldDefault = 1;
 struct Config {
     int pair_strips = -1;
     int rb_fusion = 1;
@@ -71,6 +72,7 @@
     int conv_rg_fast = 1;
     int pingpong = 1;
     int narrow_blk = 1;
+    int stage_fold = -1;
     int rb_streams = -1;
     Config();
 };
@@ -148,7 +150,10 @@
 bool rb_supported(const amp_conv* const* c1, const amp_conv* const* c2, int np, int B, int T);
 int rb_split(const amp_conv* const* c1, int np, int B, int T);
 int rb_run(const amp_conv* const* c1, const amp_conv* const* c2, int np, const float* x, int B, int T, float slope, float* y, int mode,
-           float div, hipStream_t stream, const int* lens = nullptr, int len_mul = 1, int first = 0, int count = -1);
+           float div, hipStream_t stream, const int* lens = nullptr, int len_mul = 1, int first = 0, int count = -1,
+           const amp_conv* next_up = nullptr, float* u_out = nullptr);
+bool rb_fold_supported(const amp_conv* const* c1, const amp_conv* const* c2, int np, int first, int mode, const amp_conv* up);
+bool stage_fold_on();
 
 struct ActParams {
     float* a_dev = nullptr;
diff --git a/amphion_amd/csrc/amp_internal.h b/amphion_amd/csrc/amp_internal.h
--- a/amphion_amd/csrc/amp_internal.h
+++ b/amphion_amd/csrc/amp_internal.h
@@ -111,6 +111,10 @@
     const int* lens;
     int len_mul;
     unsigned* range_flag;
+    const void* up_wp;
+    const float* up_bias;
+    float up_sc, up_isc;
+    float* up_out;
 };
 
 constexpr int AMP_AMPB_MAX_STEPS = 6;
@@ -238,6 +242,7 @@
 template <int KT> hipError_t launch_strip(const PairArgs& a, hipStream_t stream);
 template <int KT> int rb_tile(int C, int max_dil, int wide);
 template <int KT> hipError_t launch_rb(const RbArgs& a, int wide, hipStream_t stream);
+template <int KT> bool rb_has_up(int C, int wide);
 template <int KT> int ampb_tile(int C, int max_dil, int wide);
 template <int KT> hipError_t launch_ampb(const AmpbArgs& a, int wide, hipStream_t stream);
 
diff --git a/amphion_amd/csrc/conv_host.hip b/amphion_amd/csrc/conv_host.hip
--- a/amphion_amd/csrc/conv_host.hip
+++ b/amphion_amd/csrc/conv_host.hip
@@ -50,6 +50,7 @@
 static hipError_t launch_rb(int k, const RbArgs& a, int wide, hipStream_t s) {
     return with_taps(RbTaps{}, k, hipErrorInvalidValue, [&](auto K) { return launch_rb<K>(a, wide, s); });
 }
+static bool rb_has_up(int k, int C, int wide) { return with_taps(RbTaps{}, k, false, [&](auto K) { return rb_has_up<K>(C, wide); }); }
 static int ampb_tile(int k, int C, int max_dil, int wide) {
     return with_taps(AmpbTaps{}, k, 0, [&](auto K) { return ampb_tile<K>(C, max_dil, wide); });
 }
@@ -419,9 +420,28 @@
     return 2;
 }
 
+bool rb_fold_supported(const amp_conv* const* c1, const amp_conv* const* c2, int np, int first, int mode, const amp_conv* up) {
+    if (!up || first < 0 || first >= np || mode != 2) return false;
+    if (up->precision != PREC_F16X3 || !up->transposed || up->stride != 2 || up->ntaps != 2 || up->KT != 2 || up->k != 4 || up->padding != 1 ||
+        up->out_pad != 0 || up->dilation != 1 || !up->bias_dev || up->pad_reflect || up->tanh_out || up->gated_H) return false;
+    for (int p = first; p < np; ++p) {
+        if (!c1[p] || !c2[p] || !pair_supported(c1[p], c2[p]) || c1[p]->cin != c1[first]->cin || c1[p]->k != c1[first]->k) return false;
+    }
+    const int C = c1[first]->cin, k = c1[first]->k;
+    if (up->cin != C || up->cout * 2 != C) return false;
+    const int form = rb_form(C, k);
+    return form >= 0 && rb_has_up(k, C, form);
+}
+bool stage_fold_on() { return (cfg().stage_fold < 0 ? kStageFoldDefault : cfg().stage_fold) != 0; }
+
 int rb_run(const amp_conv* const* c1, const amp_conv* const* c2, int np, const float* x, int B, int T, float slope, float* y, int mode,
-           float div, hipStream_t stream, const int* lens, int len_mul, int first, int count) {
+           float div, hipStream_t stream, const int* lens, int len_mul, int first, int count, const amp_conv* next_up, float* u_out) {
     if (x == y) { set_error("rb_run: x and y must not alias"); return AMP_ERR_INVALID; }
+    if (next_up) {
+        if (!u_out || u_out == x || u_out == y) { set_error("rb_run: the folded ConvTranspose1d's output must alias neither x nor y"); return AMP_ERR_INVALID; }
+        if (count >= 0 && first + count != np) { set_error("rb_run: only the resblock's final launch takes the next ConvTranspose1d"); return AMP_ERR_INVALID; }
+        if (!rb_fold_supported(c1, c2, np, first, mode, next_up)) { set_error("rb_run: this launch has no closing ConvTranspose1d phase"); return AMP_ERR_UNSUPPORTED; }
+    }
     if (slope > 1.f) { set_error("rb_run: leaky_relu slope %g > 1 is outside the fused kernels", (double)slope); return AMP_ERR_UNSUPPORTED; }
     RbArgs a{};
     a.x = x; a.y = y;
@@ -445,6 +465,13 @@
     const int W = rb_tile(c1[0]->k, a.C, max_dil, form);
     const int NT = W - 2 * a.rh;
     a.tiles_per_item = (T + NT - 1) / NT;
+    if (next_up) {
+        if (NT - 1 < 1) { set_error("rb_run: tile too narrow for the closing phase"); return AMP_ERR_UNSUPPORTED; }
+        a.tiles_per_item = (T + 1 + NT - 2) / (NT - 1);
+        a.up_wp = next_up->wp_dev; a.up_bias = next_up->bias_dev;
+        a.up_sc = 16.f * next_up->wscale; a.up_isc = 1.f / a.up_sc;
+        a.up_out = u_out;
+    }
     a.slope = slope; a.mode = mode; a.div = div;
     a.lens = lens; a.len_mul = len_mul;
     a.range_flag = range_flag_for_current_device();
@@ -700,6 +727,22 @@
     return rb_run(c1, c2, n_pairs, x_dev, B, T, slope, y_dev, 0, 1.f, (hipStream_t)stream);
 }
 
+int amp_resblock_upsample_forward(const amp_conv* const* c1, const amp_conv* const* c2, int n_pairs, const float* x_dev, int B, int T,
+                                  float slope, float* y_dev, int mode, float div, const amp_conv* up, float* u_dev, void* stream) {
+    if (!c1 || !c2 || !x_dev || !y_dev || (up && !u_dev)) { set_error("amp_resblock_upsample_forward: null argument"); return AMP_ERR_INVALID; }
+    if (B <= 0 || T <= 0 || n_pairs < 1 || n_pairs > AMP_RB_MAX_PAIRS || mode < 0 || mode > 2) {
+        set_error("amp_resblock_upsample_forward: B=%d T=%d n_pairs=%d mode=%d", B, T, n_pairs, mode);
+        return AMP_ERR_INVALID;
+    }
+    for (int p = 0; p < n_pairs; ++p) if (!c1[p] || !c2[p]) { set_error("amp_resblock_upsample_forward: null conv handle"); return AMP_ERR_INVALID; }
+    if (!rb_supported(c1, c2, n_pairs, B, T) || (up && !rb_fold_supported(c1, c2, n_pairs, 0, mode, up))) {
+        set_error("amp_resblock_upsample_forward: block (C=%d k=%d, %d pairs, B=%d T=%d, mode %d%s) is not covered by the whole-resblock kernel "
+                  "under the current amp_set_resblock_fusion mode", c1[0]->cin, c1[0]->k, n_pairs, B, T, mode, up ? ", closing ConvTranspose1d" : "");
+        return AMP_ERR_UNSUPPORTED;
+    }
+    return rb_run(c1, c2, n_pairs, x_dev, B, T, slope, y_dev, mode, div, (hipStream_t)stream, nullptr, 1, 0, -1, up, u_dev);
+}
+
 int amp_ampblock_forward(const amp_conv* const* c1, const amp_conv* const* c2, int n_pairs, const float* alpha_dev,
                          const float* beta_dev, int logscale, const float* filt_up_host, const float* filt_down_host,
                          const float* x_dev, int B, int T, float* y_dev, int mode, float div, void* stream) {
diff --git a/amphion_amd/csrc/generator.hip b/amphion_amd/csrc/generator.hip
--- a/amphion_amd/csrc/generator.hip
+++ b/amphion_amd/csrc/generator.hip
@@ -448,6 +448,8 @@
     float* SIDE;
     int side_per;
     size_t be;
+    const amp_conv* next_up = nullptr;
+    float** u_next = nullptr;
     const ResBlock& rb(int j) const { return g->rbs[(size_t)i * g->d.n_kernels + j]; }
 };
 
@@ -581,7 +583,11 @@
         const int sp = rb_split(q.c1, nd, B, t);
         if (sp > 0) AMP_RC(rb_run(q.c1, q.c2, nd, s.U, B, t, kLreluSlope, b.R, 0, 1.f, sj, s.lens, s.lm, 0, sp));
         AMP_RC(wait_before_last(wait, sj));
-        return rb_run(q.c1, q.c2, nd, sp > 0 ? b.R : s.U, B, t, kLreluSlope, b.XS, mode_last, nk, sj, s.lens, s.lm, sp, -1);
+        const bool fold = s.next_up && s.u_next && mode_last == 2 && rb_fold_supported(q.c1, q.c2, nd, sp, mode_last, s.next_up);
+        float* u_out = !fold ? nullptr : (sp > 0 ? const_cast<float*>(s.U) : b.R);
+        AMP_RC(rb_run(q.c1, q.c2, nd, sp > 0 ? b.R : s.U, B, t, kLreluSlope, b.XS, mode_last, nk, sj, s.lens, s.lm, sp, -1, fold ? s.next_up : nullptr, u_out));
+        if (fold) *s.u_next = u_out;
+        return AMP_OK;
     }
     const float* cur = s.U;
     for (int p = 0; p < nd; ++p) {
@@ -728,8 +734,19 @@
     const bool horizontal = conc && (long long)B * T <= kRbHorizontalMaxFrames && d.resblock_type == 1 && !big && d.n_kernels == 3;
     int t = T;
     int lm = 1;
+    const bool may_fold = stage_fold_on() && !conc && !big && d.resblock_type == 1;
+    float* u_folded = nullptr;
     for (int i = 0; i < d.n_stages; ++i) {
-        AMP_RC(conv_run(g->ups[i].get(), X, B, t, big ? 1.f : kLreluSlope, nullptr, 1.f, U, 0, 1.f, st, 0, lens, lm));
+        if (!u_folded) {
+            AMP_RC(conv_run(g->ups[i].get(), X, B, t, big ? 1.f : kLreluSlope, nullptr, 1.f, U, 0, 1.f, st, 0, lens, lm));
+        } else if (u_folded != U) {
+            s.R = U;
+            U = u_folded;
+            s.U = U;
+        }
+        u_folded = nullptr;
+        s.next_up = (may_fold && i + 1 < d.n_stages) ? g->ups[i + 1].get() : nullptr;
+        s.u_next = &u_folded;
         t *= d.upsample_rates[i];
         lm *= d.upsample_rates[i];
         if (ev_mrf) AMP_HIP(hipEventRecord(ev_mrf[2 * i], st));
diff --git a/amphion_amd/csrc/rb_f16x3.hip b/amphion_amd/csrc/rb_f16x3.hip
--- a/amphion_amd/csrc/rb_f16x3.hip
+++ b/amphion_amd/csrc/rb_f16x3.hip
@@ -6,208 +6,16 @@
 
 namespace amp {
 
-
-template <int KT, int WM, int WN, int NI, int RING = 0, int RB_G = 32>
-__global__ __launch_bounds__(64 * WM * WN, 2) void rb_f16x3_kernel(const RbArgs a) {
-    static_assert(RING == 0 || RING < KT, "a ring shorter than one chunk");
-    constexpr int NTHR = 64 * WM * WN;
-    constexpr int W = 32 * NI * WN;
-    constexpr int WL = W + 2 * RB_G;
-    constexpr int H2 = (KT - 1) / 2;
-    constexpr int NCH = 2 * WM;
-    constexpr int CHS = 4 * WL;
-    constexpr int C = 32 * WM;
-    static_assert(NI % 2 == 0, "B fragments are read in halves");
-    extern __shared__ __attribute__((aligned(16))) uint4 smem4[];
-
-    const int tid = threadIdx.x;
-    const int lane = tid & 63;
-    const int wave = __builtin_amdgcn_readfirstlane(tid >> 6);
-    const int wm = wave / WN, wn = wave % WN;
-    const int hi = lane >> 5, l31 = lane & 31;
-    const int nbx = gridDim.x;
-    int bx = tile_order(blockIdx.x, nbx, a.lens != nullptr, a.rev);
-    const int item = bx / a.tiles_per_item;
-    const int tile = bx - item * a.tiles_per_item;
-    const int T = a.T;
-    const int RH = a.rh;
-    const int NT = W - 2 * RH;
-    const int O0 = tile * NT;
-    int Tv = T;
-    if (a.lens) { const int l = a.lens[item] * a.len_mul; Tv = l < Tv ? l : Tv; }
-    if (O0 >= Tv) return;
-    const int q0 = O0 - RH;
-
-    for (int i = tid; i < NCH * 4 * 2 * RB_G; i += NTHR) {
-        const int row = i / (2 * RB_G), g = i - row * (2 * RB_G);
-        smem4[row * WL + (g < RB_G ? g : W + g)] = make_uint4(0u, 0u, 0u, 0u);
-    }
-
-    const int colw = wn * (32 * NI) + l31;
-    int qcl[NI];
-    bool qok[NI];
-#pragma unroll
-    for (int t = 0; t < NI; ++t) {
-        const int q = q0 + colw + 32 * t;
-        qok[t] = (q >= 0) && (q < Tv);
-        qcl[t] = q < 0 ? 0 : (q < T ? q : T - 1);
-    }
-    const float* xr = a.x + (size_t)item * C * T + (size_t)(32 * wm + 16 * hi) * T;
-    f32x16 rv[NI];
-#pragma unroll
-    for (int t = 0; t < NI; ++t)
-#pragma unroll
-        for (int r = 0; r < 16; ++r) rv[t][r] = xr[(size_t)r * T + qcl[t]];
-
-    constexpr size_t MBS = (size_t)NCH * (KT * 128);
-    constexpr int NA = RING > 0 ? RING : KT;
-    Frag a_h[NA], a_l[NA];
-    const int wlane = (lane & 32) | (16 * ((lane >> 2) & 1) + 4 * ((lane >> 3) & 3) + (lane & 3));
-    {
-        const uint4* w0 = static_cast<const uint4*>(a.wp1[0]) + (size_t)wm * MBS + wlane;
-#pragma unroll
-        for (int g = 0; g < NA; ++g) {
-            a_h[g].u = w0[g * 128];
-            a_l[g].u = w0[g * 128 + 64];
-        }
-    }
-    AMP_PIN_VMEM();
-
-    float range_max = 0.f;
-    const float kpos = 16.f, kneg = 16.f * a.slope;
-    auto stage_x = [&]() __attribute__((always_inline)) {
-#pragma unroll
-        for (int t = 0; t < NI; ++t) {
-            const int col = RB_G + colw + 32 * t;
-            const bool ok = qok[t];
-            const int o4 = (2 * wm + hi) * CHS + col;
-#pragma unroll
-            for (int o = 0; o < 2; ++o) {
-                struct { uint2 u; } fh0, fl0, fh1, fl1;
-                stage4_f16(ok ? rv[t][8 * o + 0] : 0.f, ok ? rv[t][8 * o + 1] : 0.f, ok ? rv[t][8 * o + 2] : 0.f,
-                           ok ? rv[t][8 * o + 3] : 0.f, kpos, kneg, range_max, fh0.u, fl0.u);
-                stage4_f16(ok ? rv[t][8 * o + 4] : 0.f, ok ? rv[t][8 * o + 5] : 0.f, ok ? rv[t][8 * o + 6] : 0.f,
-                           ok ? rv[t][8 * o + 7] : 0.f, kpos, kneg, range_max, fh1.u, fl1.u);
-                smem4[o4 + o * WL] = make_uint4(fh0.u.x, fh0.u.y, fh1.u.x, fh1.u.y);
-                smem4[o4 + o * WL + 2 * WL] = make_uint4(fl0.u.x, fl0.u.y, fl1.u.x, fl1.u.y);
-            }
-        }
-    };
-
-    f32x16 acc[NI];
-    auto conv = [&](const void* wp, const float* bias, float sc, int d, const void* wp_next) __attribute__((always_inline)) {
-#pragma unroll
-        for (int r = 0; r < 16; ++r) {
-            const float bv = bias[32 * wm + 16 * hi + r] * sc;
-#pragma unroll
-            for (int t = 0; t < NI; ++t) acc[t][r] = bv;
-        }
-        const uint4* wa = static_cast<const uint4*>(wp) + (size_t)wm * MBS + wlane;
-        const uint4* wn0 = static_cast<const uint4*>(wp_next) + (size_t)wm * MBS + wlane;
-        const int rd = hi * WL + RB_G + colw - H2 * d;
-#pragma unroll 1
-        for (int c = 0; c < NCH; ++c) {
-            const uint4* wcur = wa + (size_t)c * (KT * 128);
-            const uint4* wan = (c + 1) < NCH ? wa + (size_t)(c + 1) * (KT * 128) : wn0;
-            const uint4* base = smem4 + c * CHS + rd;
-#pragma unroll
-            for (int g = 0; g < KT; ++g) {
-                const int v = RING > 0 ? g % NA : g;
-                const uint4* bg = base + g * d;
-                constexpr int NB = NI / 2;
-#pragma unroll
-                for (int th = 0; th < 2; ++th) {
-                    Frag bh[NB], bl[NB];
-#pragma unroll
-                    for (int t = 0; t < NB; ++t) {
-                        bh[t].u = bg[32 * (th * NB + t)];
-                        bl[t].u = bg[2 * WL + 32 * (th * NB + t)];
-                    }
-                    mfma3<NB>(acc + th * NB, a_h[v], a_l[v], bh, bl);
-                }
-                {
-                    const bool same = RING > 0 && g + RING < KT;
-                    const uint4* src = same ? wcur + (size_t)(g + RING) * 128 : wan + (size_t)v * 128;
-                    a_h[v].u = src[0];
-                    a_l[v].u = src[64];
-                }
-                AMP_PIN_VMEM();
-            }
-        }
-    };
-
-    stage_x();
-    __syncthreads();
-
-    const int np = a.np;
-#pragma unroll 1
-    for (int p = 0; p < AMP_RB_MAX_PAIRS; ++p) {
-        if (p < np) {
-            const bool last = (p + 1 == np);
-            conv(a.wp1[p], a.bias1[p], a.sc1[p], a.dil[p], a.wp2[p]);
-            __syncthreads();
-            {
-                const float i1 = a.isc1[p];
-                const float slope = a.slope;
-#pragma unroll
-                for (int t = 0; t < NI; ++t) {
-                    const int o4 = (2 * wm + hi) * CHS + RB_G + colw + 32 * t;
-#pragma unroll
-                    for (int o = 0; o < 2; ++o) {
-                        struct { uint2 u; } fh0, fl0, fh1, fl1;
-                        seam4_f16(acc[t][8 * o + 0], acc[t][8 * o + 1], acc[t][8 * o + 2], acc[t][8 * o + 3], i1, slope, qok[t], range_max, fh0.u, fl0.u);
-                        seam4_f16(acc[t][8 * o + 4], acc[t][8 * o + 5], acc[t][8 * o + 6], acc[t][8 * o + 7], i1, slope, qok[t], range_max, fh1.u, fl1.u);
-                        smem4[o4 + o * WL] = make_uint4(fh0.u.x, fh0.u.y, fh1.u.x, fh1.u.y);
-                        smem4[o4 + o * WL + 2 * WL] = make_uint4(fl0.u.x, fl0.u.y, fl1.u.x, fl1.u.y);
-                    }
-                }
-            }
-            __syncthreads();
-            conv(a.wp2[p], a.bias2[p], a.sc2[p], 1, last ? a.wp2[p] : a.wp1[p + 1 < AMP_RB_MAX_PAIRS ? p + 1 : p]);
-            {
-                const float i2 = a.isc2[p];
-#pragma unroll
-                for (int t = 0; t < NI; ++t)
-#pragma unroll
-                    for (int r = 0; r < 16; ++r) rv[t][r] = __builtin_fmaf(acc[t][r], i2, rv[t][r]);
-            }
-            if (!last) {
-                __syncthreads();
-                stage_x();
-                __syncthreads();
-            }
-        }
-    }
-
-    {
-        const int mode = a.mode;
-        float* yr = a.y + (size_t)item * C * T + (size_t)(32 * wm + 16 * hi) * T;
-        if (mode != 0) {
-#pragma unroll
-            for (int t = 0; t < NI; ++t)
-#pragma unroll
-                for (int r = 0; r < 16; ++r) acc[t][r] = yr[(size_t)r * T + qcl[t]];
-#pragma unroll
-            for (int t = 0; t < NI; ++t) rv[t] += acc[t];
-            if (mode == 2) {
-#pragma unroll
-                for (int t = 0; t < NI; ++t)
-#pragma unroll
-                    for (int r = 0; r < 16; ++r) rv[t][r] = rv[t][r] / a.div;
-            }
-        }
-#pragma unroll
-        for (int t = 0; t < NI; ++t) {
-            const int col = colw + 32 * t;
-            const int q = q0 + col;
-            if (col >= RH && col < W - RH && q < T) {
-#pragma unroll
-                for (int r = 0; r < 16; ++r) yr[(size_t)r * T + qcl[t]] = rv[t][r];
-            }
-        }
-    }
-    if (a.range_flag && __any(range_max > 65504.f) && lane == 0) atomicOr(a.range_flag, 1u);
-}
+#define AMP_RB_KERNEL rb_f16x3_kernel
+#define AMP_RB_FOLD 0
+#include "rb_f16x3_body.h"
+#undef AMP_RB_KERNEL
+#undef AMP_RB_FOLD
+#define AMP_RB_KERNEL rb_up_f16x3_kernel
+#define AMP_RB_FOLD 1
+#include "rb_f16x3_body.h"
+#undef AMP_RB_KERNEL
+#undef AMP_RB_FOLD
 
 template <int KT, int WM, int WN, int NI, int RING = 0, int RB_G = 32>
 static hipError_t launch_rb_one(const RbArgs& a, hipStream_t stream) {
@@ -219,6 +27,21 @@
     note_work(grid.x, a.np * 2 * 2.0 * a.C * a.C * KT * (double)a.T * a.B / 1e9, 4.0 * a.B * (double)a.C * a.T * (2 + (a.mode ? 1 : 0)) / 1e6,
               "whole ResBlock C=%d k=%d T=%d B=%d: %d convs%s", a.C, KT, a.T, a.B, 2 * a.np, a.mode ? " +sum" : "");
     hipLaunchKernelGGL((rb_f16x3_kernel<KT, WM, WN, NI, RING, RB_G>), grid, dim3(64 * WM * WN), lds, stream, a);
+    return hipGetLastError();
+}
+
+template <int KT, int WM, int WN, int NI, int RING = 0, int RB_G = 32>
+static hipError_t launch_rb_up_one(const RbArgs& a, hipStream_t stream) {
+    constexpr int W = 32 * NI * WN;
+    const size_t lds = (size_t)2 * WM * 4 * (W + 2 * RB_G) * sizeof(uint4);
+    if (hipError_t e = ensure_dynamic_lds<&rb_up_f16x3_kernel<KT, WM, WN, NI, RING, RB_G>>(lds); e != hipSuccess) return e;
+    dim3 grid((unsigned)(a.B * a.tiles_per_item));
+    note_kernel("rb_up_f16x3_kernel", KT, WM, WN, NI, RING, RB_G);
+    note_work(grid.x, (a.np * 2 * 2.0 * a.C * a.C * KT * (double)a.T + 2.0 * a.C * a.C * 2 * (double)(a.T + 1)) * a.B / 1e9,
+              4.0 * a.B * (double)a.C * a.T * (2 + (a.mode ? 1 : 0)) / 1e6,
+              "whole ResBlock C=%d k=%d T=%d B=%d: %d convs%s +ConvT %d->%d k=4 T=%d->%d", a.C, KT, a.T, a.B, 2 * a.np, a.mode ? " +sum" : "", a.C,
+              a.C / 2, a.T, 2 * a.T);
+    hipLaunchKernelGGL((rb_up_f16x3_kernel<KT, WM, WN, NI, RING, RB_G>), grid, dim3(64 * WM * WN), lds, stream, a);
     return hipGetLastError();
 }
 
@@ -235,6 +58,12 @@
 template <int KT>
 hipError_t launch_rb(const RbArgs& a, int wide, hipStream_t stream) {
     constexpr int RING = KT >= 7 ? 4 : 0;
+    if (a.up_wp) {
+        if constexpr (KT == 11) {
+            if (a.C == 64 && wide) return launch_rb_up_one<KT, 2, 4, 4, RING>(a, stream);
+        }
+        return hipErrorInvalidValue;
+    }
     if (a.C == 32) return wide ? launch_rb_one<KT, 1, 8, 4, RING>(a, stream) : launch_rb_one<KT, 1, 4, 4, RING>(a, stream);
     if (a.C == 64 && wide) return launch_rb_one<KT, 2, 4, 4, RING>(a, stream);
     if constexpr (KT <= 5) {
@@ -247,7 +76,11 @@
     return hipErrorInvalidValue;
 }
 
+template <int KT>
+bool rb_has_up(int C, int wide) { return KT == 11 && C == 64 && wide == 1; }
+
 template int rb_tile<AMP_KT>(int, int, int);
+template bool rb_has_up<AMP_KT>(int, int);
 template hipError_t launch_rb<AMP_KT>(const RbArgs&, int, hipStream_t);
 
 }
diff --git a/amphion_amd/csrc/rb_f16x3_body.h b/amphion_amd/csrc/rb_f16x3_body.h
--- /dev/null
+++ b/amphion_amd/csrc/rb_f16x3_body.h
@@ -0,0 +1,276 @@
+#if !defined(AMP_RB_KERNEL) || !defined(AMP_RB_FOLD)
+#error "define AMP_RB_KERNEL and AMP_RB_FOLD before including rb_f16x3_body.h"
+#endif
+
+
+template <int KT, int WM, int WN, int NI, int RING = 0, int RB_G = 32>
+__global__ __launch_bounds__(64 * WM * WN, 2) void AMP_RB_KERNEL(const RbArgs a) {
+    constexpr bool FOLD = AMP_RB_FOLD != 0;
+    static_assert(RING == 0 || RING < KT, "a ring shorter than one chunk");
+    static_assert(!FOLD || RING == 4, "the closing phase walks its 2 * NCH fragments through a ring of four");
+    constexpr int NTHR = 64 * WM * WN;
+    constexpr int W = 32 * NI * WN;
+    constexpr int WL = W + 2 * RB_G;
+    constexpr int H2 = (KT - 1) / 2;
+    constexpr int NCH = 2 * WM;
+    constexpr int CHS = 4 * WL;
+    constexpr int C = 32 * WM;
+    static_assert(NI % 2 == 0, "B fragments are read in halves");
+    extern __shared__ __attribute__((aligned(16))) uint4 smem4[];
+
+    const int tid = threadIdx.x;
+    const int lane = tid & 63;
+    const int wave = __builtin_amdgcn_readfirstlane(tid >> 6);
+    const int wm = wave / WN, wn = wave % WN;
+    const int hi = lane >> 5, l31 = lane & 31;
+    const int nbx = gridDim.x;
+    int bx = tile_order(blockIdx.x, nbx, a.lens != nullptr, a.rev);
+    const int item = bx / a.tiles_per_item;
+    const int tile = bx - item * a.tiles_per_item;
+    const int T = a.T;
+    const int RH = a.rh;
+    constexpr int FC = FOLD ? 1 : 0;
+    const int NT = W - 2 * RH - FC;
+    const int O0 = tile * NT;
+    int Tv = T;
+    if (a.lens) { const int l = a.lens[item] * a.len_mul; Tv = l < Tv ? l : Tv; }
+    if (O0 >= Tv + FC) return;
+    const int q0 = O0 - RH - FC;
+
+    for (int i = tid; i < NCH * 4 * 2 * RB_G; i += NTHR) {
+        const int row = i / (2 * RB_G), g = i - row * (2 * RB_G);
+        smem4[row * WL + (g < RB_G ? g : W + g)] = make_uint4(0u, 0u, 0u, 0u);
+    }
+
+    const int colw = wn * (32 * NI) + l31;
+    int qcl[NI];
+    bool qok[NI];
+#pragma unroll
+    for (int t = 0; t < NI; ++t) {
+        const int q = q0 + colw + 32 * t;
+        qok[t] = (q >= 0) && (q < Tv);
+        qcl[t] = q < 0 ? 0 : (q < T ? q : T - 1);
+    }
+    const float* xr = a.x + (size_t)item * C * T + (size_t)(32 * wm + 16 * hi) * T;
+    f32x16 rv[NI];
+#pragma unroll
+    for (int t = 0; t < NI; ++t)
+#pragma unroll
+        for (int r = 0; r < 16; ++r) rv[t][r] = xr[(size_t)r * T + qcl[t]];
+
+    constexpr size_t MBS = (size_t)NCH * (KT * 128);
+    constexpr int NA = RING > 0 ? RING : KT;
+    constexpr size_t MBS_UP = (size_t)NCH * (2 * 128);
+    Frag a_h[NA], a_l[NA];
+    const int wlane = (lane & 32) | (16 * ((lane >> 2) & 1) + 4 * ((lane >> 3) & 3) + (lane & 3));
+    {
+        const uint4* w0 = static_cast<const uint4*>(a.wp1[0]) + (size_t)wm * MBS + wlane;
+#pragma unroll
+        for (int g = 0; g < NA; ++g) {
+            a_h[g].u = w0[g * 128];
+            a_l[g].u = w0[g * 128 + 64];
+        }
+    }
+    AMP_PIN_VMEM();
+
+    float range_max = 0.f;
+    const float kpos = 16.f, kneg = 16.f * a.slope;
+    auto stage_x = [&]() __attribute__((always_inline)) {
+#pragma unroll
+        for (int t = 0; t < NI; ++t) {
+            const int col = RB_G + colw + 32 * t;
+            const bool ok = qok[t];
+            const int o4 = (2 * wm + hi) * CHS + col;
+#pragma unroll
+            for (int o = 0; o < 2; ++o) {
+                struct { uint2 u; } fh0, fl0, fh1, fl1;
+                stage4_f16(ok ? rv[t][8 * o + 0] : 0.f, ok ? rv[t][8 * o + 1] : 0.f, ok ? rv[t][8 * o + 2] : 0.f,
+                           ok ? rv[t][8 * o + 3] : 0.f, kpos, kneg, range_max, fh0.u, fl0.u);
+                stage4_f16(ok ? rv[t][8 * o + 4] : 0.f, ok ? rv[t][8 * o + 5] : 0.f, ok ? rv[t][8 * o + 6] : 0.f,
+                           ok ? rv[t][8 * o + 7] : 0.f, kpos, kneg, range_max, fh1.u, fl1.u);
+                smem4[o4 + o * WL] = make_uint4(fh0.u.x, fh0.u.y, fh1.u.x, fh1.u.y);
+                smem4[o4 + o * WL + 2 * WL] = make_uint4(fl0.u.x, fl0.u.y, fl1.u.x, fl1.u.y);
+            }
+        }
+    };
+
+    f32x16 acc[NI];
+    auto conv = [&](const void* wp, const float* bias, float sc, int d, const void* wp_next, size_t mbs_next) __attribute__((always_inline)) {
+#pragma unroll
+        for (int r = 0; r < 16; ++r) {
+            const float bv = bias[32 * wm + 16 * hi + r] * sc;
+#pragma unroll
+            for (int t = 0; t < NI; ++t) acc[t][r] = bv;
+        }
+        const uint4* wa = static_cast<const uint4*>(wp) + (size_t)wm * MBS + wlane;
+        const uint4* wn0 = static_cast<const uint4*>(wp_next) + (size_t)wm * (FOLD ? mbs_next : MBS) + wlane;
+        const int rd = hi * WL + RB_G + colw - H2 * d;
+#pragma unroll 1
+        for (int c = 0; c < NCH; ++c) {
+            const uint4* wcur = wa + (size_t)c * (KT * 128);
+            const uint4* wan = (c + 1) < NCH ? wa + (size_t)(c + 1) * (KT * 128) : wn0;
+            const uint4* base = smem4 + c * CHS + rd;
+#pragma unroll
+            for (int g = 0; g < KT; ++g) {
+                const int v = RING > 0 ? g % NA : g;
+                const uint4* bg = base + g * d;
+                constexpr int NB = NI / 2;
+#pragma unroll
+                for (int th = 0; th < 2; ++th) {
+                    Frag bh[NB], bl[NB];
+#pragma unroll
+                    for (int t = 0; t < NB; ++t) {
+                        bh[t].u = bg[32 * (th * NB + t)];
+                        bl[t].u = bg[2 * WL + 32 * (th * NB + t)];
+                    }
+                    mfma3<NB>(acc + th * NB, a_h[v], a_l[v], bh, bl);
+                }
+                {
+                    const bool same = RING > 0 && g + RING < KT;
+                    const uint4* src = same ? wcur + (size_t)(g + RING) * 128 : wan + (size_t)v * 128;
+                    a_h[v].u = src[0];
+                    a_l[v].u = src[64];
+                }
+                AMP_PIN_VMEM();
+            }
+        }
+    };
+
+    stage_x();
+    __syncthreads();
+
+    const int np = a.np;
+#pragma unroll 1
+    for (int p = 0; p < AMP_RB_MAX_PAIRS; ++p) {
+        if (p < np) {
+            const bool last = (p + 1 == np);
+            conv(a.wp1[p], a.bias1[p], a.sc1[p], a.dil[p], a.wp2[p], MBS);
+            __syncthreads();
+            {
+                const float i1 = a.isc1[p];
+                const float slope = a.slope;
+#pragma unroll
+                for (int t = 0; t < NI; ++t) {
+                    const int o4 = (2 * wm + hi) * CHS + RB_G + colw + 32 * t;
+#pragma unroll
+                    for (int o = 0; o < 2; ++o) {
+                        struct { uint2 u; } fh0, fl0, fh1, fl1;
+                        seam4_f16(acc[t][8 * o + 0], acc[t][8 * o + 1], acc[t][8 * o + 2], acc[t][8 * o + 3], i1, slope, qok[t], range_max, fh0.u, fl0.u);
+                        seam4_f16(acc[t][8 * o + 4], acc[t][8 * o + 5], acc[t][8 * o + 6], acc[t][8 * o + 7], i1, slope, qok[t], range_max, fh1.u, fl1.u);
+                        smem4[o4 + o * WL] = make_uint4(fh0.u.x, fh0.u.y, fh1.u.x, fh1.u.y);
+                        smem4[o4 + o * WL + 2 * WL] = make_uint4(fl0.u.x, fl0.u.y, fl1.u.x, fl1.u.y);
+                    }
+                }
+            }
+            __syncthreads();
+            if constexpr (FOLD) {
+                conv(a.wp2[p], a.bias2[p], a.sc2[p], 1, last ? a.up_wp : a.wp1[p + 1 < AMP_RB_MAX_PAIRS ? p + 1 : p], last ? MBS_UP : MBS);
+            } else {
+                conv(a.wp2[p], a.bias2[p], a.sc2[p], 1, last ? a.wp2[p] : a.wp1[p + 1 < AMP_RB_MAX_PAIRS ? p + 1 : p], MBS);
+            }
+            {
+                const float i2 = a.isc2[p];
+#pragma unroll
+                for (int t = 0; t < NI; ++t)
+#pragma unroll
+                    for (int r = 0; r < 16; ++r) rv[t][r] = __builtin_fmaf(acc[t][r], i2, rv[t][r]);
+            }
+            if (!last) {
+                __syncthreads();
+                stage_x();
+                __syncthreads();
+            }
+        }
+    }
+
+    {
+        const int mode = a.mode;
+        float* yr = a.y + (size_t)item * C * T + (size_t)(32 * wm + 16 * hi) * T;
+        if (mode != 0) {
+#pragma unroll
+            for (int t = 0; t < NI; ++t)
+#pragma unroll
+                for (int r = 0; r < 16; ++r) acc[t][r] = yr[(size_t)r * T + qcl[t]];
+#pragma unroll
+            for (int t = 0; t < NI; ++t) rv[t] += acc[t];
+            if (mode == 2) {
+#pragma unroll
+                for (int t = 0; t < NI; ++t)
+#pragma unroll
+                    for (int r = 0; r < 16; ++r) rv[t][r] = rv[t][r] / a.div;
+            }
+        }
+        if constexpr (!FOLD) {
+#pragma unroll
+        for (int t = 0; t < NI; ++t) {
+            const int col = colw + 32 * t;
+            const int q = q0 + col;
+            if (col >= RH && col < W - RH && q < T) {
+#pragma unroll
+                for (int r = 0; r < 16; ++r) yr[(size_t)r * T + qcl[t]] = rv[t][r];
+            }
+        }
+        }
+    }
+    if constexpr (FOLD) {
+        __syncthreads();
+        stage_x();
+        __syncthreads();
+#pragma unroll
+        for (int r = 0; r < 16; ++r) {
+            const float bv = a.up_bias[(32 * wm + 16 * hi + r) >> 1] * a.up_sc;
+#pragma unroll
+            for (int t = 0; t < NI; ++t) acc[t][r] = bv;
+        }
+        {
+            const uint4* wu = static_cast<const uint4*>(a.up_wp) + (size_t)wm * MBS_UP + wlane;
+            const int rd = hi * WL + RB_G + colw;
+#pragma unroll
+            for (int f = 0; f < 2 * NCH; ++f) {
+                const int v = f % NA;
+                const uint4* bg = smem4 + (f >> 1) * CHS + rd - (f & 1);
+                constexpr int NB = NI / 2;
+#pragma unroll
+                for (int th = 0; th < 2; ++th) {
+                    Frag bh[NB], bl[NB];
+#pragma unroll
+                    for (int t = 0; t < NB; ++t) {
+                        bh[t].u = bg[32 * (th * NB + t)];
+                        bl[t].u = bg[2 * WL + 32 * (th * NB + t)];
+                    }
+                    mfma3<NB>(acc + th * NB, a_h[v], a_l[v], bh, bl);
+                }
+                if (f + NA < 2 * NCH) {
+                    a_h[v].u = wu[(f + NA) * 128];
+                    a_l[v].u = wu[(f + NA) * 128 + 64];
+                }
+                AMP_PIN_VMEM();
+            }
+        }
+        struct __attribute__((packed, aligned(4))) F2 { float a, b; };
+        const int Tout = 2 * T;
+        float* ur = a.up_out + ((size_t)item * (C / 2) + (size_t)(16 * wm + 8 * hi)) * Tout;
+        const float iu = a.up_isc;
+#pragma unroll
+        for (int t = 0; t < NI; ++t) {
+            const int col = colw + 32 * t;
+            const int q = q0 + col;
+            if (col > RH && col < W - RH && q <= T) {
+                const int n0 = 2 * q - 1;
+#pragma unroll
+                for (int j = 0; j < 8; ++j) {
+                    const float v0 = acc[t][2 * j] * iu, v1 = acc[t][2 * j + 1] * iu;
+                    float* urow = ur + (size_t)j * Tout;
+                    if (n0 >= 0 && n0 + 1 < Tout) {
+                        F2 v{v0, v1};
+                        *reinterpret_cast<F2*>(urow + n0) = v;
+                    } else {
+                        if (n0 >= 0) urow[n0] = v0;
+                        if (n0 + 1 < Tout) urow[n0 + 1] = v1;
+                    }
+                }
+            }
+        }
+    }
+    if (a.range_flag && __any(range_max > 65504.f) && lane == 0) atomicOr(a.range_flag, 1u);
+}
diff --git a/amphion_amd/csrc/runtime.hip b/amphion_amd/csrc/runtime.hip
--- a/amphion_amd/csrc/runtime.hip
+++ b/amphion_amd/csrc/runtime.hip
@@ -140,6 +140,7 @@
     rb_fusion = num("AMP_RB_FUSION", 0, 3, 1);
     ampb_fusion = num("AMP_AMPB_FUSION", 0, 3, 1);
     rb_streams = num("AMP_RB_STREAMS", -1, 1, -1);
+    stage_fold = num("AMP_STAGE_FOLD", -1, 1, -1);
     static const char* const kRemoved[][2] = {
         {"AMP_GROUP_MB", "amp_set_group_mb(megabytes)"}, {"AMP_PAIR_STRIP", "amp_set_pair_strips(mode)"}, {"AMP_CONV_BLK", "amp_set_conv_blk(mode)"},
         {"AMP_FUSE_PAIRS", "nothing (the fused pairs are the only form)"}, {"AMP_RB_SUM_FRAMES", "nothing"},
@@ -170,7 +171,7 @@
 
 extern "C" {
 
-int amp_version(void) { return 150; }
+int amp_version(void) { return 151; }
 const char* amp_last_error(void) { return g_err; }
 
 int amp_set_precision(int precision) {
@@ -241,6 +242,12 @@
     return AMP_OK;
 }
 
+int amp_set_stage_fold(int mode) {
+    if (mode < -1 || mode > 1) { set_error("amp_set_stage_fold: mode=%d (-1 policy, 0 off, 1 wherever built)", mode); return AMP_ERR_INVALID; }
+    cfg().stage_fold = mode;
+    return AMP_OK;
+}
+
 int amp_set_ampblock_fusion(int mode) {
     if (mode < -1 || mode > 3) { set_error("amp_set_ampblock_fusion: mode=%d", mode); return AMP_ERR_INVALID; }
     cfg().ampb_fusion = mode < 0 ? 1 : mode;
diff --git a/include/amphion_hip.h b/include/amphion_hip.h
--- a/include/amphion_hip.h
+++ b/include/amphion_hip.h
@@ -178,6 +178,9 @@
 int amp_resblock_forward(const amp_conv* const* c1, const amp_conv* const* c2, int n_pairs, const float* x_dev, int B, int T,
                          float slope, float* y_dev, void* stream);
 int amp_set_resblock_fusion(int mode);
+int amp_resblock_upsample_forward(const amp_conv* const* c1, const amp_conv* const* c2, int n_pairs, const float* x_dev, int B, int T,
+                                  float slope, float* y_dev, int mode, float div, const amp_conv* up, float* u_dev, void* stream);
+int amp_set_stage_fold(int mode);
 int amp_set_resblock_streams(int mode);
 int amp_gen_prepare_streams(amp_gen* g);
 
```

Result: no change. 146.7 million (median of 6 runs) (+0.5%).
